# muzishen/IMAGDressing

Measured on AMD Instinct MI355X. Metric: 512x512 50-step images/sec (whole node), higher is better.
Workload: dtype bf16

## Files before the change

imagdressing_amd/_lib.py:

```python
from __future__ import annotations

import ctypes as C
import os

_HERE = os.path.dirname(os.path.abspath(__file__))
LIB_PATH = os.environ.get("IMD_LIB_PATH") or os.path.join(_HERE, "libimagdressing_hip.so")

ABI_VERSION = 9

u16p = C.POINTER(C.c_uint16)
f32p = C.POINTER(C.c_float)


class _Sized(C.Structure):

    def __init__(self, *args, **kw):
        super().__init__(*args, **kw)
        self.struct_bytes = C.sizeof(self)


class HeadsDest(C.Structure):
    _fields_ = [("ptr", C.c_void_p), ("kind", C.c_int), ("DP", C.c_int), ("L", C.c_int), ("scale", C.c_float)]


class ConvGemmParams(_Sized):
    _fields_ = [("struct_bytes", C.c_uint32), 
        ("x", C.c_void_p), ("w", C.c_void_p), ("out", C.c_void_p),
        ("M", C.c_int), ("N", C.c_int), ("K", C.c_int),
        ("Cin", C.c_int), ("taps", C.c_int), ("Hin", C.c_int), ("Win", C.c_int), ("Hout", C.c_int),
        ("Wout", C.c_int), ("stride", C.c_int), ("ups", C.c_int),
        ("x_pix_stride", C.c_int), ("out_ld", C.c_int), ("res_ld", C.c_int),
        ("bias", C.c_void_p), ("rowvec", C.c_void_p), ("rowvec_stride", C.c_int),
        ("res", C.c_void_p), ("out_scale", C.c_float), ("act", C.c_int), ("out_f32", C.c_int),
        ("mode", C.c_int), ("hC", C.c_int), ("hH", C.c_int), ("hD", C.c_int),
        ("hd", HeadsDest * 3), ("dtype", C.c_int), ("split_k", C.c_int), ("splitk_ws", C.c_void_p),
        ("x_bytes", C.c_uint32), ("w_bytes", C.c_uint32), ("flags", C.c_int),
        ("gn_a", C.c_void_p), ("gn_b", C.c_void_p), ("gn_silu", C.c_int), ("pad_br_only", C.c_int),
        ("splitk_counters", C.c_void_p),
        ("gn_stats_out", C.c_void_p), ("gn_stats_groups", C.c_int),
        ("gn_in_partial", C.c_void_p), ("gn_in_gamma", C.c_void_p), ("gn_in_beta", C.c_void_p),
        ("gn_in_nparts", C.c_int), ("gn_in_groups", C.c_int), ("gn_in_silu", C.c_int), ("gn_in_eps", C.c_float),
        ("gn_out_gamma", C.c_void_p), ("gn_out_beta", C.c_void_p), ("gn_out_eps", C.c_float), ("gn_out_silu", C.c_int), ("gn_out_groups", C.c_int), ("res_rows", C.c_int),
    ]


class FfParams(_Sized):
    _fields_ = [("struct_bytes", C.c_uint32), ("x", C.c_void_p), ("w1", C.c_void_p), ("b1", C.c_void_p), ("w2", C.c_void_p), ("b2", C.c_void_p), ("out", C.c_void_p),
                ("M", C.c_int), ("C", C.c_int), ("inner", C.c_int), ("x_ld", C.c_int), ("out_ld", C.c_int), ("ln", C.c_int),
                ("ln_eps", C.c_float), ("dtype", C.c_int)]


class XattnParams(_Sized):
    _fields_ = [("struct_bytes", C.c_uint32), ("x", C.c_void_p), ("w", C.c_void_p), ("bq", C.c_void_p), ("bo", C.c_void_p), ("kv", C.c_void_p),
                ("out", C.c_void_p), ("M", C.c_int), ("C", C.c_int), ("heads", C.c_int), ("L", C.c_int), ("rows_per_image", C.c_int),
                ("kv_bdiv", C.c_int), ("text_rows", C.c_int), ("x_ld", C.c_int), ("out_ld", C.c_int), ("q_scale", C.c_float),
                ("ln_eps", C.c_float), ("dtype", C.c_int)]


class AttnParams(_Sized):
    _fields_ = [("struct_bytes", C.c_uint32), 
        ("q", C.c_void_p), ("k1", C.c_void_p), ("v1t", C.c_void_p), ("k2", C.c_void_p), ("v2t", C.c_void_p),
        ("scale2", C.c_void_p), ("out", C.c_void_p),
        ("B", C.c_int), ("H", C.c_int), ("N", C.c_int), ("D", C.c_int),
        ("L1", C.c_int), ("L1P", C.c_int), ("kv1_bdiv", C.c_int),
        ("L2", C.c_int), ("L2P", C.c_int), ("kv2_bdiv", C.c_int),
        ("out_ld", C.c_int), ("dtype", C.c_int), ("flags", C.c_int), ("causal", C.c_int), ("k_pad_one", C.c_int),
        ("proj_w", C.c_void_p), ("proj_b", C.c_void_p), ("proj_res", C.c_void_p), ("proj_out", C.c_void_p),
        ("proj_res_ld", C.c_int), ("proj_out_ld", C.c_int), ("proj_counters", C.c_void_p),
        ("out_dup", C.c_void_p), ("phase2_out", C.c_void_p), ("phase2_rows", C.c_int),
    ]


class GroupNormParams(_Sized):
    _fields_ = [("struct_bytes", C.c_uint32), 
        ("x", C.c_void_p), ("y", C.c_void_p), ("gamma", C.c_void_p), ("beta", C.c_void_p), ("partial", C.c_void_p),
        ("B", C.c_int), ("HW", C.c_int), ("C", C.c_int), ("G", C.c_int), ("x_ld", C.c_int), ("y_ld", C.c_int),
        ("eps", C.c_float), ("silu", C.c_int), ("dtype", C.c_int), ("nparts", C.c_int),
    ]


class LayerNormParams(_Sized):
    _fields_ = [("struct_bytes", C.c_uint32), 
        ("x", C.c_void_p), ("y", C.c_void_p), ("gamma", C.c_void_p), ("beta", C.c_void_p),
        ("rows", C.c_int), ("C", C.c_int), ("x_ld", C.c_int), ("y_ld", C.c_int), ("eps", C.c_float), ("dtype", C.c_int),
    ]


class DdimParams(_Sized):
    _fields_ = [("struct_bytes", C.c_uint32), 
        ("z", C.c_void_p), ("eps", C.c_void_p), ("x_next", C.c_void_p),
        ("B", C.c_int), ("HW", C.c_int),
        ("guidance", C.c_float), ("sqrt_a_t", C.c_float), ("sqrt_1m_a_t", C.c_float),
        ("sqrt_a_prev", C.c_float), ("sqrt_1m_a_prev", C.c_float),
        ("mask", C.c_void_p), ("z_img", C.c_void_p), ("noise", C.c_void_p),
        ("sqrt_a_next", C.c_float), ("sqrt_1m_a_next", C.c_float), ("dtype", C.c_int),
        ("coefs", C.c_void_p), ("var_noise", C.c_void_p), ("sigma", C.c_float),
    ]


class SamplerParams(_Sized):
    _fields_ = [("struct_bytes", C.c_uint32),
        ("z", C.c_void_p), ("eps", C.c_void_p), ("x_next", C.c_void_p), ("hist", C.c_void_p),
        ("B", C.c_int), ("HW", C.c_int), ("K", C.c_int), ("dtype", C.c_int),
        ("guidance", C.c_float), ("guidance_rows", C.c_void_p),
        ("m_x", C.c_float), ("m_e", C.c_float), ("z_x", C.c_float), ("z_m", C.c_float),
        ("z_h", C.c_float * 4),
        ("z_n", C.c_float), ("b_img", C.c_float), ("b_noise", C.c_float), ("in_scale", C.c_float),
        ("store", C.c_int),
        ("noise", C.c_void_p), ("mask", C.c_void_p), ("z_img", C.c_void_p), ("blend_noise", C.c_void_p),
        ("coefs", C.c_void_p),
    ]


class ImageResampleParams(_Sized):
    _fields_ = [("struct_bytes", C.c_uint32),
        ("src", C.c_void_p), ("src_row_stride", C.c_int64), ("src_img_stride", C.c_int64), ("out", C.c_void_p), ("tmp", C.c_void_p),
        ("B", C.c_int), ("Hin", C.c_int), ("Win", C.c_int), ("C", C.c_int), ("Hres", C.c_int), ("Wres", C.c_int),
        ("h_xmin", C.c_void_p), ("h_count", C.c_void_p), ("h_k", C.c_void_p), ("h_kmax", C.c_int), ("h_taps", C.c_int),
        ("v_xmin", C.c_void_p), ("v_count", C.c_void_p), ("v_k", C.c_void_p), ("v_kmax", C.c_int), ("v_taps", C.c_int),
        ("v_tile_rows", C.c_int), ("top", C.c_int), ("left", C.c_int), ("crop_h", C.c_int), ("crop_w", C.c_int),
        ("kind", C.c_int), ("dtype", C.c_int), ("binarize", C.c_int), ("flags", C.c_int),
        ("a", C.c_float * 3), ("b", C.c_float * 3),
    ]


class ImagePackParams(_Sized):
    _fields_ = [("struct_bytes", C.c_uint32), ("src", C.c_void_p), ("out", C.c_void_p),
                ("B", C.c_int), ("H", C.c_int), ("W", C.c_int), ("ld", C.c_int), ("dtype", C.c_int)]


class ImageOverlayParams(_Sized):
    _fields_ = [("struct_bytes", C.c_uint32), ("orig", C.c_void_p), ("mask", C.c_void_p), ("gen", C.c_void_p), ("out", C.c_void_p),
                ("B", C.c_int), ("Bo", C.c_int), ("H0", C.c_int), ("W0", C.c_int),
                ("x1", C.c_int), ("y1", C.c_int), ("cw", C.c_int), ("ch", C.c_int)]


class ImageInpaintConditionParams(_Sized):
    _fields_ = [("struct_bytes", C.c_uint32), ("image", C.c_void_p), ("mask", C.c_void_p), ("out", C.c_void_p),
                ("B", C.c_int), ("H", C.c_int), ("W", C.c_int), ("dtype", C.c_int)]


SYMBOLS = {
    "imd_abi_version": (C.c_int, []),
    "imd_last_error": (C.c_char_p, []),
    "imd_device_check": (C.c_int, [C.c_int]),
    "imd_conv_gemm": (C.c_int, [C.POINTER(ConvGemmParams), C.c_int, C.c_void_p]),
    "imd_conv_gemm_auto_cfg": (C.c_int, [C.c_int, C.c_int]),
    "imd_conv_gemm_auto_split": (C.c_int, [C.c_int, C.c_int, C.c_int, C.c_int]),
    "imd_attention": (C.c_int, [C.POINTER(AttnParams), C.c_void_p]),
    "imd_attention_dup_supported": (C.c_int, [C.c_int, C.c_int, C.c_int]),
    "imd_attention_phase_split_supported": (C.c_int, [C.c_int]),
    "imd_attention_fp8": (C.c_int, [C.POINTER(AttnParams), C.c_int, C.c_int, C.c_int, C.c_void_p]),
    "imd_attn_quantize_fp8": (C.c_int, [C.c_void_p, C.c_void_p, C.c_int, C.c_long, C.c_int, C.c_int, C.c_float, C.c_int, C.c_void_p]),
    "imd_set_tuning": (C.c_int, [C.c_int, C.c_int]),
    "imd_get_tuning": (C.c_int, [C.c_int]),
    "imd_attn_padded_dims": (C.c_int, [C.c_int, C.POINTER(C.c_int), C.POINTER(C.c_int)]),
    "imd_groupnorm": (C.c_int, [C.POINTER(GroupNormParams), C.c_void_p]),
    "imd_groupnorm_coeffs": (C.c_int, [C.POINTER(GroupNormParams), C.c_void_p, C.c_void_p, C.c_void_p]),
    "imd_conv_patch_supported": (C.c_int, [C.POINTER(ConvGemmParams)]),
    "imd_conv_patch2_supported": (C.c_int, [C.POINTER(ConvGemmParams)]),
    "imd_conv_patch3_supported": (C.c_int, [C.POINTER(ConvGemmParams)]),
    "imd_conv_patch4_supported": (C.c_int, [C.POINTER(ConvGemmParams)]),
    "imd_conv_img_supported": (C.c_int, [C.POINTER(ConvGemmParams)]),
    "imd_conv_patch_stats_parts": (C.c_int, [C.POINTER(ConvGemmParams)]),
    "imd_conv_gemm_stats_parts": (C.c_int, [C.POINTER(ConvGemmParams), C.c_int]),
    "imd_conv_gemm_gn_out_supported": (C.c_int, [C.POINTER(ConvGemmParams)]),
    "imd_row_linear_gn_in_supported": (C.c_int, [C.POINTER(ConvGemmParams), C.c_int]),
    "imd_gemm_dma_supported": (C.c_int, [C.POINTER(ConvGemmParams)]),
    "imd_row_linear": (C.c_int, [C.POINTER(ConvGemmParams), C.c_int, C.c_float, C.c_void_p]),
    "imd_row_linear_supported": (C.c_int, [C.POINTER(ConvGemmParams)]),
    "imd_ff_geglu": (C.c_int, [C.POINTER(FfParams), C.c_void_p]),
    "imd_text_xattn320": (C.c_int, [C.POINTER(XattnParams), C.c_void_p]),
    "imd_text_xattn320_supported": (C.c_int, [C.POINTER(XattnParams)]),
    "imd_conv_ups_phase": (C.c_int, [C.POINTER(ConvGemmParams), C.c_void_p]),
    "imd_conv_ups_phase_supported": (C.c_int, [C.POINTER(ConvGemmParams)]),
    "imd_groupnorm_workspace_floats": (C.c_int, [C.c_int, C.c_int, C.c_int, C.c_int]),
    "imd_layernorm": (C.c_int, [C.POINTER(LayerNormParams), C.c_void_p]),
    "imd_softmax_rows": (C.c_int, [C.c_void_p, C.c_int, C.c_void_p, C.c_int, C.c_int, C.c_int, C.c_int, C.c_void_p]),
    "imd_ddim_cfg_step": (C.c_int, [C.POINTER(DdimParams), C.c_void_p]),
    "imd_ddim_cfg_step_rows": (C.c_int, [C.POINTER(DdimParams), C.c_void_p, C.c_void_p]),
    "imd_sampler_step": (C.c_int, [C.POINTER(SamplerParams), C.c_void_p]),
    "imd_sampler_step_rows": (C.c_int, [C.POINTER(SamplerParams), C.c_void_p, C.c_void_p]),
    "imd_image_resample": (C.c_int, [C.POINTER(ImageResampleParams), C.c_void_p]),
    "imd_image_resample_form": (C.c_int, [C.POINTER(ImageResampleParams)]),
    "imd_image_pack_u8": (C.c_int, [C.POINTER(ImagePackParams), C.c_void_p]),
    "imd_image_overlay": (C.c_int, [C.POINTER(ImageOverlayParams), C.c_void_p]),
    "imd_image_inpaint_condition": (C.c_int, [C.POINTER(ImageInpaintConditionParams), C.c_void_p]),
    "imd_timestep_embedding": (C.c_int, [C.c_void_p, C.c_void_p, C.c_int, C.c_int, C.c_void_p]),
    "imd_add": (C.c_int, [C.c_void_p, C.c_int, C.c_void_p, C.c_int, C.c_void_p, C.c_int, C.c_long, C.c_int, C.c_float, C.c_int, C.c_void_p]),
    "imd_embed_tokens": (C.c_int, [C.c_void_p, C.c_int, C.c_void_p, C.c_int, C.c_void_p, C.c_void_p, C.c_long, C.c_int, C.c_int, C.c_void_p]),
    "imd_vit_assemble": (C.c_int, [C.c_void_p, C.c_void_p, C.c_void_p, C.c_void_p, C.c_int, C.c_int, C.c_int, C.c_int, C.c_void_p]),
    "imd_lincomb": (C.c_int, [C.POINTER(C.c_void_p), C.POINTER(C.c_float), C.c_int, C.c_void_p, C.c_long, C.c_void_p]),
    "imd_copy2d": (C.c_int, [C.c_void_p, C.c_int, C.c_void_p, C.c_int, C.c_long, C.c_int, C.c_void_p]),
    "imd_concat2": (C.c_int, [C.c_void_p, C.c_int, C.c_void_p, C.c_int, C.c_void_p, C.c_void_p, C.c_long, C.c_long, C.c_int, C.c_void_p]),
    "imd_concat2_gn_stats": (C.c_int, [C.c_void_p, C.c_int, C.c_void_p, C.c_int, C.c_void_p, C.c_void_p, C.c_int, C.c_int, C.c_int, C.c_int,
                                       C.c_void_p, C.c_int, C.c_void_p]),
    "imd_groupnorm_parts": (C.c_int, [C.c_int, C.c_int, C.c_int]),
    "imd_f32_to_16": (C.c_int, [C.c_void_p, C.c_void_p, C.c_long, C.c_int, C.c_void_p]),
}

_lib = None


class ImdError(RuntimeError):
    pass


def load():
    global _lib
    if _lib is None:
        if not os.path.isfile(LIB_PATH):
            raise ImdError(
                f"{LIB_PATH} not found: build it with `python -c 'import __graft_entry__ as g; g.build()'` "
                "(or imagdressing_amd/csrc/build.sh).  imagdressing_amd has no CPU / torch fallback.")
        lib = C.CDLL(LIB_PATH)
        for name, (res, args) in SYMBOLS.items():
            fn = getattr(lib, name)
            fn.restype, fn.argtypes = res, args
        if lib.imd_abi_version() != ABI_VERSION:
            raise ImdError(f"ABI version mismatch: library reports {lib.imd_abi_version()}, binding expects {ABI_VERSION}")
        _lib = lib
    return _lib


def check(rc: int):
    if rc != 0:
        raise ImdError(load().imd_last_error().decode("utf-8", "replace"))
```

imagdressing_amd/adapter/attention_processor.py:

```python
from __future__ import annotations

import math
from typing import Dict, Optional, Tuple

import torch
import torch.nn as nn

from .. import ops

bf16 = torch.bfloat16
LOG2E = math.log2(math.e)


class LoRALinearLayer(nn.Module):

    def __init__(self, in_features, out_features, rank=4, network_alpha=None):
        super().__init__()
        self.down = nn.Linear(in_features, rank, bias=False)
        self.up = nn.Linear(rank, out_features, bias=False)
        self.network_alpha = network_alpha
        self.rank = rank
        nn.init.normal_(self.down.weight, std=1 / rank)
        nn.init.zeros_(self.up.weight)

    def delta(self) -> torch.Tensor:
        d = self.up.weight.float() @ self.down.weight.float()
        if self.network_alpha is not None:
            d = d * (self.network_alpha / self.rank)
        return d


def _version_key(*tensors) -> Tuple:
    return tuple((t.data_ptr(), t._version, t.device, t.dtype) for t in tensors)


class _TensorCache:

    def __init__(self, capacity: int = 4):
        self._entries = []
        self._cap = capacity

    def get(self, srcs, extra=()):
        key = (_version_key(*srcs), extra)
        for i, (s, k, v) in enumerate(self._entries):
            if k == key and len(s) == len(srcs) and all(a is b for a, b in zip(s, srcs)):
                if i != len(self._entries) - 1:
                    self._entries.append(self._entries.pop(i))
                return v
        return None

    def put(self, srcs, value, extra=()):
        self._entries.append((tuple(srcs), (_version_key(*srcs), extra), value))
        if len(self._entries) > self._cap:
            self._entries.pop(0)
        return value


_W_PARTS = {"qkv": ("to_q", "to_k", "to_v"), "kv": ("to_k", "to_v"), "q": ("to_q",), "o": ("to_out",), "bo": ("to_out",)}
_16BIT = (torch.bfloat16, torch.float16)


def _compute_dtype(attn, hidden_states: torch.Tensor, attention_mask=None):
    if attention_mask is not None:
        raise NotImplementedError("attention_mask is always None on the IMAGDressing path (SURVEY appendix 3); masks are not implemented")
    if getattr(attn, "spatial_norm", None) is not None or getattr(attn, "group_norm", None) is not None \
            or getattr(attn, "norm_cross", None):
        raise NotImplementedError("attn.spatial_norm / group_norm / norm_cross are None for every SD1.5 attention layer; "
                                  "modules that set them are not supported by the fused processors")
    wd = attn.to_q.weight.dtype
    if wd in _16BIT:
        return wd
    return hidden_states.dtype if hidden_states.dtype in _16BIT else torch.float16


def _layer_weights(attn, which: str, dtype, device) -> torch.Tensor:
    mods = [attn.to_out[0] if n == "to_out" else getattr(attn, n) for n in _W_PARTS[which]]
    srcs = [m.bias if which == "bo" else m.weight for m in mods]
    if srcs[0] is None:
        return None
    want = torch.float32 if which == "bo" else dtype
    if len(srcs) == 1 and srcs[0].dtype == want and srcs[0].device == device and srcs[0].is_contiguous():
        return srcs[0].detach()
    cache = attn.__dict__.setdefault("_imd_wcache", {})
    key = (_version_key(*srcs), want, str(device))
    ent = cache.get(which)
    if ent is None or ent[0] != key or not all(a is b for a, b in zip(ent[1], srcs)):
        t = torch.cat([t.detach().to(device=device, dtype=want) for t in srcs], 0).contiguous()
        ent = cache[which] = (key, tuple(srcs), t)
    return ent[2]


def _ln_folded_q(attn, gamma: torch.Tensor, beta: torch.Tensor, dtype, device, which: str = "q"):
    mods = [getattr(attn, n) for n in _W_PARTS[which]]
    srcs = tuple(m.weight for m in mods) + (gamma, beta)
    cache = attn.__dict__.setdefault("_imd_wcache", {})
    key = (_version_key(*srcs), dtype, str(device))
    ent = cache.get(which + "_ln")
    if ent is None or ent[0] != key or not all(a is b for a, b in zip(ent[1], srcs)):
        w = torch.cat([m.weight.detach().to(device=device, dtype=dtype) for m in mods], 0)
        ent = cache[which + "_ln"] = (key, srcs, ops.fold_layernorm_affine(w, None, gamma.to(device), beta.to(device)))
    return ent[2]


def _qkv_ln_ok(x: torch.Tensor) -> bool:
    return x.shape[-1] == 320 and x.shape[1] % 128 == 0 and ops.FUSED_LN


FUSED_LN_CHANNELS = (320, 640, 1280)


def _as_tokens(hidden_states: torch.Tensor, dtype):
    shape4 = None
    if hidden_states.dim() == 4:
        b, c, h, w = hidden_states.shape
        shape4 = (b, c, h, w)
        hidden_states = hidden_states.view(b, c, h * w).transpose(1, 2)
    if not hidden_states.is_cuda:
        from .._lib import ImdError
        raise ImdError("imagdressing_amd processors run on MI355X only: hidden_states is on " + str(hidden_states.device))
    return hidden_states.to(dtype).contiguous(), shape4


def _restore(out, shape4, like):
    if shape4 is not None:
        b, c, h, w = shape4
        out = out.transpose(-1, -2).reshape(b, c, h, w)
    return out


def _project_kv(tokens: torch.Tensor, wkv: torch.Tensor, heads: int):
    Bk, Lk, Kd = tokens.shape
    Cc = wkv.shape[0] // 2
    D = Cc // heads
    dpk, dpv = ops.attn_padded_dims(D)
    LP = ops.pad64(Lk)
    k = ops.k_buffer((Bk, heads, Lk, dpk), D, wkv.dtype, tokens.device)
    vt = torch.zeros(Bk, heads, dpv, LP, dtype=wkv.dtype, device=tokens.device)
    ops.conv_gemm(tokens.view(Bk * Lk, Kd), wkv, M=Bk * Lk, N=2 * Cc, Cin=Kd, Hin=Lk, Win=1, Hout=Lk, Wout=1,
                  heads=dict(C=Cc, H=heads, D=D, dests=[(k, 0, dpk, Lk, 1.0), (vt, 1, dpv, LP, 1.0)]))
    return k, vt, Lk, LP


_FP8_KV: Dict[int, tuple] = {}
ops._clear_hooks.append(_FP8_KV.clear)


def _fp8_kv(kv, cache: bool):
    k, vt = kv[0], kv[1]
    e = ops.FP8_EXPS
    if cache:
        hit = _FP8_KV.get(id(k))
        if hit is not None and hit[0] is k and hit[1] == (e["q"], e["k"], e["v"]):
            return hit[2], hit[3]
    k8 = ops.quantize_fp8_rows(k, e["k"], pad_val=float(2 ** (e["q"] + e["k"])))
    v8 = ops.quantize_fp8_vt(vt, e["v"])
    if cache:
        if len(_FP8_KV) > 64:
            _FP8_KV.clear()
        _FP8_KV[id(k)] = (k, (e["q"], e["k"], e["v"]), k8, v8)
    return k8, v8


def _fused_attention(x: torch.Tensor, heads: int, *, wq_or_qkv: torch.Tensor, self_attn: bool,
                     kv1=None, kv1_bdiv: int = 1, kv2=None, kv2_bdiv: int = 1, scale2: Optional[torch.Tensor] = None,
                     wo: torch.Tensor, bo: Optional[torch.Tensor], residual: Optional[torch.Tensor],
                     q_ln: Optional[tuple] = None, pair_half: bool = False, phase2_rows: int = 0) -> torch.Tensor:
    B, N, Cc = x.shape
    D = Cc // heads
    dpk, dpv = ops.attn_padded_dims(D)
    dev, dt = x.device, x.dtype
    qscale = D ** -0.5 * LOG2E
    if (ops.FUSED_XATTN and not self_attn and q_ln is not None and kv1 is not None and kv2 is None and not pair_half
            and ops.text_xattn_supported(Cc, heads, N, kv1[2]) and not ops.ATTN_FP8 and not ops.FUSED_OUT_PROJ
            and residual is not None and residual.data_ptr() == x.data_ptr() and residual.shape == x.shape
            and residual.dtype == dt and residual.is_contiguous()):
        return ops.text_xattn(x, ops.pack_text_xattn(q_ln[0], q_ln[1], wo, bo), ops.pack_text_kv(kv1[0], kv1[1], kv1[2]),
                              Lk=kv1[2], kv_bdiv=kv1_bdiv, ln_eps=q_ln[2], q_scale=qscale)
    q = ops.workspace("attn_q", (B, heads, N, dpk), dt, dev)
    x2 = x.view(B * N, Cc)
    if self_attn:
        LP = ops.pad64(N)
        k = ops.k_buffer((B, heads, N, dpk), D, dt, dev, tag="attn_k")
        vt = ops.workspace("attn_vt", (B, heads, dpv, LP), dt, dev)
        dests = dict(C=Cc, H=heads, D=D, dests=[(q, 0, dpk, N, qscale), (k, 0, dpk, N, 1.0), (vt, 1, dpv, LP, 1.0)])
        if q_ln is not None:
            ops.conv_gemm(x2, q_ln[0], M=B * N, N=3 * Cc, Cin=Cc, Hin=N, Win=1, Hout=N, Wout=1, bias=q_ln[1], ln_eps=q_ln[2], heads=dests)
        else:
            ops.conv_gemm(x2, wq_or_qkv, M=B * N, N=3 * Cc, Cin=Cc, Hin=N, Win=1, Hout=N, Wout=1, heads=dests)
        kv1, kv1_bdiv = (k, vt, N, LP), 1
    elif q_ln is not None:
        ops.conv_gemm(x2, q_ln[0], M=B * N, N=Cc, Cin=Cc, Hin=N, Win=1, Hout=N, Wout=1, bias=q_ln[1], ln_eps=q_ln[2],
                      heads=dict(C=Cc, H=heads, D=D, dests=[(q, 0, dpk, N, qscale)]))
    else:
        ops.conv_gemm(x2, wq_or_qkv, M=B * N, N=Cc, Cin=Cc, Hin=N, Win=1, Hout=N, Wout=1,
                      heads=dict(C=Cc, H=heads, D=D, dests=[(q, 0, dpk, N, qscale)]))
    o = torch.empty(B, N, Cc, dtype=dt, device=dev)
    if ops.ATTN_FP8 and D == 40:
        e = ops.FP8_EXPS
        q8 = ops.quantize_fp8_rows(q, e["q"])
        k18, v18 = _fp8_kv(kv1, cache=not self_attn)
        kw = {}
        if kv2 is not None and scale2 is not None:
            k28, v28 = _fp8_kv(kv2, cache=True)
            kw = dict(k2=k28, v2t=v28, L2=kv2[2], L2P=kv2[3], kv2_bdiv=kv2_bdiv, scale2=scale2)
        ops.attention_fp8(q8, k18, v18, o, B=B, H=heads, N=N, L1=kv1[2], L1P=kv1[3], kv1_bdiv=kv1_bdiv, **kw)
        res2 = None if residual is None else residual.view(B * N, Cc)
        return ops.linear(o.view(B * N, Cc), wo, bo, res=res2).view(B, N, Cc)
    kw = {}
    if kv2 is not None and scale2 is not None:
        kw = dict(k2=kv2[0], v2t=kv2[1], L2=kv2[2], L2P=kv2[3], kv2_bdiv=kv2_bdiv, scale2=scale2)
    if ops.FUSED_OUT_PROJ and ops.attention_proj_supported(heads, N, D):
        out = torch.empty(B, N, Cc, dtype=dt, device=dev)
        return ops.attention(q, kv1[0], kv1[1], o, B=B, H=heads, N=N, D=D, L1=kv1[2], L1P=kv1[3], kv1_bdiv=kv1_bdiv, k_pad_one=True,
                             proj=(wo, bo, residual, out), **kw)
    if pair_half:
        o = torch.empty(2 * B, N, Cc, dtype=dt, device=dev)
        ops.attention(q, kv1[0], kv1[1], o[:B], B=B, H=heads, N=N, D=D, L1=kv1[2], L1P=kv1[3], kv1_bdiv=kv1_bdiv, k_pad_one=True,
                      out_dup=o[B:], **kw)
        res2 = None if residual is None else residual.reshape(-1, Cc)
        return ops.linear(o.view(2 * B * N, Cc), wo, bo, res=res2).view(2 * B, N, Cc)
    ops.attention(q, kv1[0], kv1[1], o, B=B, H=heads, N=N, D=D, L1=kv1[2], L1P=kv1[3], kv1_bdiv=kv1_bdiv, k_pad_one=True, phase2_rows=phase2_rows if kw else 0, **kw)
    res2 = None if residual is None else residual.view(B * N, Cc)
    return ops.linear(o.view(B * N, Cc), wo, bo, res=res2).view(B, N, Cc)


class _FusedBase:
    fused_residual = True

    @staticmethod
    def _ehs_bdiv(B: int, ehs: torch.Tensor) -> int:
        Be = ehs.shape[0]
        if B % Be:
            raise ValueError(f"encoder_hidden_states batch {Be} does not divide hidden_states batch {B}")
        return B // Be

    @staticmethod
    def _finish(attn, out, residual_given, like, shape4, ln_fused=False):
        if getattr(attn, "residual_connection", False) and not residual_given:
            if ln_fused:
                raise NotImplementedError("attn.residual_connection together with the engine's fused LayerNorm (imd_layernorm)")
            out = ops.add(out, _as_tokens(like, out.dtype)[0])
        if getattr(attn, "rescale_output_factor", 1.0) != 1.0:
            raise NotImplementedError("rescale_output_factor != 1 is not used by SD1.5")
        out = _restore(out, shape4, like)
        return out if out.dtype == like.dtype else out.to(like.dtype)


class AttnProcessor2_0(_FusedBase):

    fused_layernorm = True

    def __init__(self, cache_entries: int = 256):
        self._text = _TensorCache(capacity=cache_entries)

    def __call__(self, attn, hidden_states, encoder_hidden_states=None, attention_mask=None, temb=None, scale=1.0,
                 imd_residual=None, imd_layernorm=None, **kwargs):
        dt = _compute_dtype(attn, hidden_states, attention_mask)
        x, shape4 = _as_tokens(hidden_states, dt)
        dev = x.device
        wo, bo = _layer_weights(attn, "o", dt, dev), _layer_weights(attn, "bo", dt, dev)
        q_ln = None
        if imd_layernorm is not None:
            g, be, eps = imd_layernorm
            if encoder_hidden_states is not None and x.shape[-1] in FUSED_LN_CHANNELS:
                q_ln = _ln_folded_q(attn, g, be, dt, dev) + (eps,)
            elif encoder_hidden_states is None and _qkv_ln_ok(x):
                q_ln = _ln_folded_q(attn, g, be, dt, dev, "qkv") + (eps,)
            else:
                x = ops.layer_norm(x, g, be, eps)
        if encoder_hidden_states is None:
            out = _fused_attention(x, attn.heads, wq_or_qkv=_layer_weights(attn, "qkv", dt, dev), self_attn=True, wo=wo, bo=bo,
                                   residual=imd_residual, q_ln=q_ln)
        else:
            srcs = (encoder_hidden_states, attn.to_k.weight, attn.to_v.weight)
            kv = self._text.get(srcs, extra=(dt,))
            if kv is None:
                e = encoder_hidden_states.to(device=dev, dtype=dt).contiguous()
                kv = self._text.put(srcs, _project_kv(e, _layer_weights(attn, "kv", dt, dev), attn.heads), extra=(dt,))
            out = _fused_attention(x, attn.heads, wq_or_qkv=_layer_weights(attn, "q", dt, dev), self_attn=False, kv1=kv,
                                   kv1_bdiv=self._ehs_bdiv(x.shape[0], encoder_hidden_states), wo=wo, bo=bo,
                                   residual=imd_residual, q_ln=q_ln)
        return self._finish(attn, out, imd_residual is not None, hidden_states, shape4, ln_fused=imd_layernorm is not None)


class CacheAttnProcessor2_0(AttnProcessor2_0):
    fused_layernorm = False

    def __init__(self):
        super().__init__()
        self.cache = {}

    def __call__(self, attn, hidden_states, encoder_hidden_states=None, attention_mask=None, temb=None, scale=1.0,
                 **kwargs):
        self.cache["hidden_states"] = hidden_states
        return super().__call__(attn, hidden_states, encoder_hidden_states=encoder_hidden_states, **kwargs)


class _RefMixin:

    def _init_ref(self, name, hidden_size, cross_attention_dim, scale):
        self.name = name
        self.hidden_size = hidden_size
        self.cross_attention_dim = cross_attention_dim
        self.to_k_ref = nn.Linear(cross_attention_dim or hidden_size, hidden_size, bias=False)
        self.to_v_ref = nn.Linear(cross_attention_dim or hidden_size, hidden_size, bias=False)
        self.scale = scale
        self._wref = _TensorCache()
        self._garment = _TensorCache()
        self._scale2 = _TensorCache()
        self._scale2_plain: Dict = {}

    def _garment_kv(self, ref: torch.Tensor, heads: int, device, dtype):
        wsrc = (self.to_k_ref.weight, self.to_v_ref.weight)
        kv = self._garment.get((ref,) + wsrc, extra=(dtype,))
        if kv is None:
            w = self._wref.get(wsrc, extra=(dtype,))
            if w is None:
                w = self._wref.put(wsrc, torch.cat([t.detach().to(device=device, dtype=dtype) for t in wsrc], 0).contiguous(),
                                   extra=(dtype,))
            r = ref.detach().to(device=device, dtype=dtype).contiguous()
            if r.dim() != 3:
                raise ValueError(f"sa_hidden_states[{self.name!r}] must be [Bg, M, C], got {tuple(ref.shape)}")
            kv = self._garment.put((ref,) + wsrc, _project_kv(r, w, heads), extra=(dtype,))
        return kv

    def _garment_bdiv(self, B: int, ref: torch.Tensor) -> int:
        Bg = ref.shape[0]
        if Bg < 1 or B % Bg:
            raise ValueError(f"sa_hidden_states[{self.name!r}] has batch {Bg}, which does not divide hidden_states batch {B}")
        return B // Bg

    def _branch_weights(self, B: int, mask: Optional[torch.Tensor], device) -> torch.Tensor:
        s = float(self.scale)
        if mask is None:
            t = self._scale2_plain.get((B, s, str(device)))
            if t is None:
                t = torch.full((B,), s, dtype=torch.float32, device=device)
                self._scale2_plain = {(B, s, str(device)): t}
            return t
        t = self._scale2.get((mask,), extra=(s,))
        if t is None:
            t = self._scale2.put((mask,), (mask.to(device=device, dtype=torch.float32) * s).contiguous(), extra=(s,))
        return t


class RefSAttnProcessor2_0(nn.Module, _FusedBase, _RefMixin):
    fused_layernorm = True
    fused_pair_half = True

    def __init__(self, name, hidden_size, cross_attention_dim=None, scale=1.0):
        super().__init__()
        self._init_ref(name, hidden_size, cross_attention_dim, scale)

    def _weights(self, attn, dt, dev):
        return _layer_weights(attn, "qkv", dt, dev), _layer_weights(attn, "o", dt, dev), _layer_weights(attn, "bo", dt, dev)

    def __call__(self, attn, hidden_states, encoder_hidden_states=None, attention_mask=None, temb=None, scale=1.0,
                 num_images_per_prompt=1, cond_hidden_states=None, sa_hidden_states=None, sa_batch_mask=None,
                 imd_residual=None, imd_layernorm=None, imd_pair_half=False, **kwargs):
        if encoder_hidden_states is not None:
            raise NotImplementedError(f"{type(self).__name__} is a self-attention (attn1) processor")
        dt = _compute_dtype(attn, hidden_states, attention_mask)
        x, shape4 = _as_tokens(hidden_states, dt)
        wqkv, wo, bo = self._weights(attn, dt, x.device)
        q_ln = None
        if imd_layernorm is not None:
            g, be, eps = imd_layernorm
            if _qkv_ln_ok(x):
                q_ln = _ln_folded_q(attn, g, be, dt, x.device, "qkv") + (eps,)
            else:
                x = ops.layer_norm(x, g, be, eps)
        kv2 = s2 = None
        bdiv2 = 1
        if sa_hidden_states is not None:
            ref = sa_hidden_states[self.name]
            kv2 = self._garment_kv(ref, attn.heads, x.device, x.dtype)
            cond_rows = x.shape[0] // 2 if (kwargs.get("sa_pair_layout") and not imd_pair_half and x.shape[0] % 2 == 0) else x.shape[0]
            bdiv2 = self._garment_bdiv(cond_rows, ref)
            s2 = self._branch_weights(x.shape[0] * (2 if imd_pair_half else 1), sa_batch_mask, x.device)
        if imd_pair_half and (kv2 is None or imd_residual is None or shape4 is not None):
            raise ValueError("imd_pair_half needs sa_hidden_states, the block residual and token-major hidden states (engine-internal)")
        pr = x.shape[0] // 2 if (kwargs.get("sa_pair_layout") and sa_batch_mask is not None and kv2 is not None and not imd_pair_half and x.shape[0] % 2 == 0) else 0
        out = _fused_attention(x, attn.heads, wq_or_qkv=wqkv, self_attn=True, kv2=kv2, kv2_bdiv=bdiv2,
                               scale2=s2, wo=wo, bo=bo, residual=imd_residual, q_ln=q_ln, pair_half=bool(imd_pair_half), phase2_rows=pr)
        return self._finish(attn, out, imd_residual is not None, hidden_states, shape4, ln_fused=imd_layernorm is not None)


class _LoraFold:

    def _init_lora(self, hidden_size, kdim, rank, network_alpha, lora_scale):
        self.rank = rank
        self.lora_scale = lora_scale
        self.to_q_lora = LoRALinearLayer(hidden_size, hidden_size, rank, network_alpha)
        self.to_k_lora = LoRALinearLayer(kdim, hidden_size, rank, network_alpha)
        self.to_v_lora = LoRALinearLayer(kdim, hidden_size, rank, network_alpha)
        self.to_out_lora = LoRALinearLayer(hidden_size, hidden_size, rank, network_alpha)
        self._folded = _TensorCache()

    def _fold(self, attn, device, dtype):
        ls = float(self.lora_scale)
        srcs = tuple(l.weight for lo in (self.to_q_lora, self.to_k_lora, self.to_v_lora, self.to_out_lora)
                     for l in (lo.down, lo.up)) + (attn.to_q.weight, attn.to_k.weight, attn.to_v.weight, attn.to_out[0].weight)
        w = self._folded.get(srcs, extra=(ls, dtype, str(device)))
        if w is None:
            def eff(base, lora):
                base = base.detach().to(device)
                if ls == 0.0:
                    return base.to(dtype).contiguous()
                return (base.float() + ls * lora.delta().to(device)).to(dtype).contiguous()
            wq, wk, wv = eff(attn.to_q.weight, self.to_q_lora), eff(attn.to_k.weight, self.to_k_lora), eff(attn.to_v.weight, self.to_v_lora)
            wo = eff(attn.to_out[0].weight, self.to_out_lora)
            w = self._folded.put(srcs, dict(q=wq, kv=torch.cat([wk, wv], 0).contiguous(),
                                            qkv=(torch.cat([wq, wk, wv], 0).contiguous() if wk.shape[1] == wq.shape[1] else None),
                                            o=wo), extra=(ls, dtype, str(device)))
        return w


class _LoraRefSBase(nn.Module, _FusedBase, _RefMixin, _LoraFold):

    def __init__(self, name, hidden_size, cross_attention_dim=None, scale=1.0, rank=128, network_alpha=None, lora_scale=1.0):
        super().__init__()
        self._init_ref(name, hidden_size, cross_attention_dim, scale)
        self._init_lora(hidden_size, cross_attention_dim or hidden_size, rank, network_alpha, lora_scale)

    def _weights(self, attn, dt, dev):
        w = self._fold(attn, dev, dt)
        return w["qkv"], w["o"], _layer_weights(attn, "bo", dt, dev)

    __call__ = RefSAttnProcessor2_0.__call__
    fused_pair_half = True


class LoraRefSAttnProcessor2_0(_LoraRefSBase):
    """attention_processor.py:391-511 (used by inference_IMAGdressing_ipa_controlnetpose.py:88-94)."""


class RefLoraSAttnProcessor2_0(_LoraRefSBase):
    """Same arithmetic under the name ``app.py:90`` uses (attention_processor.py:1006-1128).  As in the
    reference, ``pipe.set_scale`` does not match this class (it checks LoraRefSAttnProcessor2_0)."""


class CAttnProcessor2_0(nn.Module, _FusedBase):

    def __init__(self, name, hidden_size, cross_attention_dim=None):
        super().__init__()
        self.name = name
        self.hidden_size = hidden_size
        self.cross_attention_dim = cross_attention_dim
        self._plain = AttnProcessor2_0(cache_entries=4)

    fused_layernorm = True

    def __call__(self, attn, hidden_states, encoder_hidden_states=None, attention_mask=None, temb=None, scale=1.0,
                 cond_hidden_states=None, sa_hidden_states=None, imd_residual=None, imd_layernorm=None, **kwargs):
        return self._plain(attn, hidden_states, encoder_hidden_states=encoder_hidden_states, imd_residual=imd_residual,
                           imd_layernorm=imd_layernorm)


class _IPBase(nn.Module, _FusedBase, _LoraFold):

    def __init__(self, hidden_size, cross_attention_dim=None, rank=4, network_alpha=None, lora_scale=1.0, scale=1.0,
                 num_tokens=4):
        super().__init__()
        self.num_tokens = num_tokens
        self.hidden_size = hidden_size
        self.cross_attention_dim = cross_attention_dim
        self.scale = scale
        self._init_lora(hidden_size, cross_attention_dim or hidden_size, rank, network_alpha, lora_scale)
        self.to_k_ip = nn.Linear(cross_attention_dim or hidden_size, hidden_size, bias=False)
        self.to_v_ip = nn.Linear(cross_attention_dim or hidden_size, hidden_size, bias=False)
        self._kv = _TensorCache()
        self._wip = _TensorCache()
        self._s2: Dict = {}

    def _weights(self, attn, dt, dev):
        w = self._fold(attn, dev, dt)
        return w["q"], w["kv"], w["o"]

    def __call__(self, attn, hidden_states, encoder_hidden_states=None, attention_mask=None, scale=1.0, temb=None,
                 *args, imd_residual=None, **kwargs):
        if encoder_hidden_states is None:
            raise NotImplementedError(f"{type(self).__name__} is a cross-attention (attn2) processor")
        dt = _compute_dtype(attn, hidden_states, attention_mask)
        x, shape4 = _as_tokens(hidden_states, dt)
        wq, wkv, wo = self._weights(attn, dt, x.device)
        wsrc = (self.to_k_ip.weight, self.to_v_ip.weight)
        ls = float(getattr(self, "lora_scale", 0.0))
        ksrc = (encoder_hidden_states, attn.to_k.weight, attn.to_v.weight) + wsrc
        kvs = self._kv.get(ksrc, extra=(ls, x.dtype))
        if kvs is None:
            wip = self._wip.get(wsrc, extra=(x.dtype,))
            if wip is None:
                wip = self._wip.put(wsrc, torch.cat([t.detach().to(device=x.device, dtype=x.dtype) for t in wsrc], 0).contiguous(),
                                    extra=(x.dtype,))
            e = encoder_hidden_states.to(device=x.device, dtype=x.dtype)
            end = e.shape[1] - self.num_tokens
            kvs = self._kv.put(ksrc,
                               (_project_kv(e[:, :end].contiguous(), wkv, attn.heads),
                                _project_kv(e[:, end:].contiguous(), wip, attn.heads)), extra=(ls, x.dtype))
        B = x.shape[0]
        key = (B, float(self.scale), str(x.device))
        s2 = self._s2.get(key)
        if s2 is None:
            s2 = torch.full((B,), float(self.scale), dtype=torch.float32, device=x.device)
            self._s2 = {key: s2}
        bdiv = self._ehs_bdiv(B, encoder_hidden_states)
        out = _fused_attention(x, attn.heads, wq_or_qkv=wq, self_attn=False, kv1=kvs[0], kv1_bdiv=bdiv, kv2=kvs[1],
                               kv2_bdiv=bdiv, scale2=s2, wo=wo, bo=_layer_weights(attn, "bo", dt, x.device), residual=imd_residual)
        return self._finish(attn, out, imd_residual is not None, hidden_states, shape4)


class LoRAIPAttnProcessor2_0(_IPBase):
    """attention_processor.py:746-871."""


class IPAttnProcessor2_0(_IPBase):

    def __init__(self, hidden_size, cross_attention_dim=None, scale=1.0, num_tokens=4):
        nn.Module.__init__(self)
        self.num_tokens = num_tokens
        self.hidden_size = hidden_size
        self.cross_attention_dim = cross_attention_dim
        self.scale = scale
        self.to_k_ip = nn.Linear(cross_attention_dim or hidden_size, hidden_size, bias=False)
        self.to_v_ip = nn.Linear(cross_attention_dim or hidden_size, hidden_size, bias=False)
        self._kv = _TensorCache()
        self._wip = _TensorCache()
        self._s2 = {}

    def _weights(self, attn, dt, dev):
        return _layer_weights(attn, "q", dt, dev), _layer_weights(attn, "kv", dt, dev), _layer_weights(attn, "o", dt, dev)


class BaseSAttnProcessor2_0(nn.Module, _FusedBase):

    def __init__(self, name, cross_attention_dim=None):
        super().__init__()
        self.name, self.cross_attention_dim = name, cross_attention_dim
        self._plain = AttnProcessor2_0(cache_entries=4)

    def __call__(self, attn, hidden_states, encoder_hidden_states=None, attention_mask=None, temb=None, scale=1.0,
                 imd_residual=None, **kwargs):
        return self._plain(attn, hidden_states, encoder_hidden_states=encoder_hidden_states, imd_residual=imd_residual)


class SAttnProcessor2_0(nn.Module, _FusedBase):

    def __init__(self, name, hidden_size, cross_attention_dim=None):
        super().__init__()
        self.name, self.hidden_size, self.cross_attention_dim = name, hidden_size, cross_attention_dim
        self._plain = AttnProcessor2_0(cache_entries=4)
        self._garment = _TensorCache()

    def __call__(self, attn, hidden_states, encoder_hidden_states=None, attention_mask=None, temb=None, scale=1.0,
                 cond_hidden_states=None, sa_hidden_states=None, imd_residual=None, **kwargs):
        if sa_hidden_states is None or encoder_hidden_states is not None:
            return self._plain(attn, hidden_states, encoder_hidden_states=encoder_hidden_states, imd_residual=imd_residual)
        dt = _compute_dtype(attn, hidden_states, attention_mask)
        x, shape4 = _as_tokens(hidden_states, dt)
        dev, heads = x.device, attn.heads
        B, N, Cc = x.shape
        D = Cc // heads
        ref = sa_hidden_states[self.name]
        if ref.dim() != 3 or B % ref.shape[0]:
            raise ValueError(f"sa_hidden_states[{self.name!r}] must be [Bg, M, C] with Bg dividing the batch {B}, got {tuple(ref.shape)}")
        wkv = _layer_weights(attn, "kv", dt, dev)
        srcs = (ref, attn.to_k.weight, attn.to_v.weight)
        kvr = self._garment.get(srcs, extra=(dt,))
        if kvr is None:
            kvr = self._garment.put(srcs, _project_kv(ref.detach().to(device=dev, dtype=dt).contiguous(), wkv, heads), extra=(dt,))
        kx, vtx, _, _ = _project_kv(x, wkv, heads)
        M = kvr[2]
        L, LP = N + M, ops.pad64(N + M)
        dpk, dpv = ops.attn_padded_dims(D)
        k = ops.k_buffer((B, heads, L, dpk), D, dt, dev)
        vt = torch.zeros(B, heads, dpv, LP, dtype=dt, device=dev)
        rep = B // ref.shape[0]
        k[:, :, :N] = kx
        k[:, :, N:] = kvr[0].repeat_interleave(rep, 0) if rep > 1 else kvr[0]
        vt[..., :N] = vtx[..., :N]
        vt[..., N:L] = (kvr[1].repeat_interleave(rep, 0) if rep > 1 else kvr[1])[..., :M]
        out = _fused_attention(x, heads, wq_or_qkv=_layer_weights(attn, "q", dt, dev), self_attn=False, kv1=(k, vt, L, LP), kv1_bdiv=1,
                               wo=_layer_weights(attn, "o", dt, dev), bo=_layer_weights(attn, "bo", dt, dev), residual=imd_residual)
        return self._finish(attn, out, imd_residual is not None, hidden_states, shape4)


class RefCAttnProcessor2_0(nn.Module, _FusedBase, _RefMixin):

    def __init__(self, name, hidden_size, cross_attention_dim=None, scale=1.0):
        super().__init__()
        self._init_ref(name, hidden_size, None, scale)
        self.cross_attention_dim = cross_attention_dim
        self._plain = AttnProcessor2_0(cache_entries=4)
        self._text = _TensorCache()

    def __call__(self, attn, hidden_states, encoder_hidden_states=None, attention_mask=None, temb=None, scale=1.0,
                 cond_hidden_states=None, sa_hidden_states=None, sa_batch_mask=None, imd_residual=None, **kwargs):
        if sa_hidden_states is None:
            return self._plain(attn, hidden_states, encoder_hidden_states=encoder_hidden_states, imd_residual=imd_residual)
        dt = _compute_dtype(attn, hidden_states, attention_mask)
        x, shape4 = _as_tokens(hidden_states, dt)
        dev, heads = x.device, attn.heads
        ref = sa_hidden_states[self.name]
        kv2 = self._garment_kv(ref, heads, dev, dt)
        bdiv2 = self._garment_bdiv(x.shape[0], ref)
        s2 = self._branch_weights(x.shape[0], sa_batch_mask, dev)
        wo, bo = _layer_weights(attn, "o", dt, dev), _layer_weights(attn, "bo", dt, dev)
        if encoder_hidden_states is None:
            out = _fused_attention(x, heads, wq_or_qkv=_layer_weights(attn, "qkv", dt, dev), self_attn=True, kv2=kv2, kv2_bdiv=bdiv2,
                                   scale2=s2, wo=wo, bo=bo, residual=imd_residual)
        else:
            srcs = (encoder_hidden_states, attn.to_k.weight, attn.to_v.weight)
            kv = self._text.get(srcs, extra=(dt,))
            if kv is None:
                e = encoder_hidden_states.to(device=dev, dtype=dt).contiguous()
                kv = self._text.put(srcs, _project_kv(e, _layer_weights(attn, "kv", dt, dev), heads), extra=(dt,))
            out = _fused_attention(x, heads, wq_or_qkv=_layer_weights(attn, "q", dt, dev), self_attn=False, kv1=kv,
                                   kv1_bdiv=self._ehs_bdiv(x.shape[0], encoder_hidden_states), kv2=kv2, kv2_bdiv=bdiv2, scale2=s2,
                                   wo=wo, bo=bo, residual=imd_residual)
        return self._finish(attn, out, imd_residual is not None, hidden_states, shape4)
```

imagdressing_amd/csrc/capi.cpp:

```cpp
#include <atomic>
#include <mutex>
#include <stdarg.h>
#include <stdio.h>
#include <string.h>

#include "imd_kernels.h"

namespace {
thread_local char g_err[512] = "";
}

int imd_set_error(const char* fmt, ...) {
    va_list ap;
    va_start(ap, fmt);
    vsnprintf(g_err, sizeof(g_err), fmt, ap);
    va_end(ap);
    return 1;
}

int imd_check_launch(const char* what) {
    hipError_t e = hipGetLastError();
    if (e != hipSuccess) return imd_set_error("%s: launch failed: %s", what, hipGetErrorString(e));
    return 0;
}

#define IMD_REQUIRE(cond, ...) do { if (!(cond)) return imd_set_error(__VA_ARGS__); } while (0)
#define IMD_REQUIRE_SIZE(p, what) IMD_REQUIRE((p)->struct_bytes == sizeof(*(p)), \
    "%s: parameter block is %u bytes in the caller's view, this library (ABI v%d) expects %zu: the binding mirrors another version of include/imagdressing_hip.h (set struct_bytes = sizeof(struct) after zero-initialising it)", \
    what, (unsigned)(p)->struct_bytes, IMD_ABI_VERSION, sizeof(*(p)))

namespace {
struct LdsAttrEnt { const void* kern; int dev; };
constexpr int kMaxLdsAttr = 512;
LdsAttrEnt g_lds_attr[kMaxLdsAttr];
std::atomic<int> g_lds_attr_n{0};
std::mutex g_lds_attr_mu;
int g_cu8[64] = {};
}

int imd_lds_attr(const void* kern, int bytes, const char* what) {
    int dev = 0;
    if (hipGetDevice(&dev) != hipSuccess) return imd_set_error("%s: cannot identify the current device", what);
    const int n = g_lds_attr_n.load(std::memory_order_acquire);
    for (int i = 0; i < n; ++i)
        if (g_lds_attr[i].kern == kern && g_lds_attr[i].dev == dev) return 0;
    std::lock_guard<std::mutex> lock(g_lds_attr_mu);
    hipError_t e = hipFuncSetAttribute(kern, hipFuncAttributeMaxDynamicSharedMemorySize, bytes);
    if (e != hipSuccess) return imd_set_error("%s: hipFuncSetAttribute failed: %s", what, hipGetErrorString(e));
    const int m = g_lds_attr_n.load(std::memory_order_relaxed);
    if (m < kMaxLdsAttr) {
        g_lds_attr[m] = LdsAttrEnt{kern, dev};
        g_lds_attr_n.store(m + 1, std::memory_order_release);
    }
    return 0;
}

int imd_cu_count8() {
    int dev = 0;
    if (hipGetDevice(&dev) != hipSuccess || dev < 0 || dev >= 64) return -1;
    if (g_cu8[dev] == 0) {
        int cus = 0;
        if (hipDeviceGetAttribute(&cus, hipDeviceAttributeMultiprocessorCount, dev) != hipSuccess) return -1;
        g_cu8[dev] = cus / 8 * 8 < 8 ? 8 : cus / 8 * 8;
    }
    return g_cu8[dev];
}

extern "C" {

int imd_abi_version(void) { return IMD_ABI_VERSION; }
const char* imd_last_error(void) { return g_err; }

int imd_device_check(int device) {
    hipDeviceProp_t prop;
    hipError_t e = hipGetDeviceProperties(&prop, device);
    if (e != hipSuccess) return imd_set_error("device_check: hipGetDeviceProperties(%d) failed: %s", device, hipGetErrorString(e));
    if (strncmp(prop.gcnArchName, "gfx950", 6) != 0)
        return imd_set_error("device_check: device %d is %s; this library is built for gfx950 (MI355X) only", device, prop.gcnArchName);
    return 0;
}

int imd_conv_gemm(const imd_conv_gemm_params* p, int cfg, void* stream) {
    IMD_REQUIRE(p != nullptr, "conv_gemm: null params");
    IMD_REQUIRE_SIZE(p, "conv_gemm");
    IMD_REQUIRE(p->x && p->w, "conv_gemm: null input/weight pointer");
    IMD_REQUIRE(p->mode == IMD_OUT_HEADS || p->out != nullptr, "conv_gemm: null output pointer");
    IMD_REQUIRE(p->Hout > 0 && p->Wout > 0 && p->Hin > 0 && p->Win > 0, "conv_gemm: bad geometry");
    IMD_REQUIRE(p->stride == 1 || p->stride == 2, "conv_gemm: stride must be 1 or 2");
    IMD_REQUIRE(p->M % (p->Hout * p->Wout) == 0, "conv_gemm: M (%d) is not a multiple of Hout*Wout (%d)", p->M, p->Hout * p->Wout);
    if (p->mode == IMD_OUT_HEADS) {
        IMD_REQUIRE(p->hC > 0 && p->hH > 0 && p->hD > 0 && p->hC == p->hH * p->hD, "conv_gemm: bad head split C=%d H=%d D=%d", p->hC, p->hH, p->hD);
        IMD_REQUIRE(p->N % p->hC == 0 && p->N / p->hC <= 3, "conv_gemm: N (%d) must be 1..3 splits of %d channels", p->N, p->hC);
        IMD_REQUIRE(p->hD % 8 == 0, "conv_gemm: head dim must be a multiple of 8");
        IMD_REQUIRE(p->act != IMD_ACT_GEGLU && !p->out_f32, "conv_gemm: head-split output excludes GEGLU / fp32 output");
    }
    if (p->act == IMD_ACT_GEGLU) IMD_REQUIRE(!p->out_f32 && !p->res, "conv_gemm: GEGLU excludes fp32 output and residual");
    return imd_launch_conv_gemm(*p, cfg, (hipStream_t)stream);
}

int imd_conv_gemm_auto_cfg(int M, int N) { return imd_conv_gemm_choose_cfg(M, N); }
int imd_conv_gemm_auto_split(int M, int N, int K, int cfg) { return imd_conv_gemm_choose_split(M, N, K, cfg < 0 ? imd_conv_gemm_choose_cfg(M, N) : cfg); }

int imd_attention(const imd_attn_params* p, void* stream) {
    IMD_REQUIRE(p != nullptr, "attention: null params");
    IMD_REQUIRE_SIZE(p, "attention");
    IMD_REQUIRE(p->q && p->k1 && p->v1t && p->out, "attention: null q/k/v/out pointer");
    IMD_REQUIRE((p->k2 == nullptr) == (p->v2t == nullptr), "attention: k2 and v2t must be given together");
    IMD_REQUIRE(p->out_ld >= p->H * p->D && p->out_ld % 4 == 0, "attention: bad out_ld %d", p->out_ld);
    return imd_launch_attention(*p, (hipStream_t)stream);
}

int imd_attention_fp8(const imd_attn_params* p, int eq, int ek, int ev, void* stream) {
    IMD_REQUIRE(p != nullptr, "attention_fp8: null params");
    IMD_REQUIRE_SIZE(p, "attention_fp8");
    IMD_REQUIRE(p->q && p->k1 && p->v1t && p->out, "attention_fp8: null q/k/v/out pointer");
    IMD_REQUIRE((p->k2 == nullptr) == (p->v2t == nullptr), "attention_fp8: k2 and v2t must be given together");
    IMD_REQUIRE(p->out_ld >= p->H * p->D && p->out_ld % 4 == 0, "attention_fp8: bad out_ld %d", p->out_ld);
    IMD_REQUIRE(p->dtype == IMD_DTYPE_BF16 || p->dtype == IMD_DTYPE_F16, "attention_fp8: unknown output dtype %d", p->dtype);
    return imd_launch_attention_fp8(*p, eq, ek, ev, (hipStream_t)stream);
}

int imd_attn_quantize_fp8(const uint16_t* src, uint8_t* dst, int kind, long count, int LP, int exp2_scale, float pad_val, int dtype,
                          void* stream) {
    IMD_REQUIRE(src && dst && count > 0, "attn_quantize_fp8: null pointer / empty");
    IMD_REQUIRE(kind == 0 || kind == 1, "attn_quantize_fp8: kind must be 0 (Q / K rows) or 1 (V^T)");
    IMD_REQUIRE(exp2_scale >= -16 && exp2_scale <= 16, "attn_quantize_fp8: exponent out of range");
    return imd_launch_attn_quantize_fp8(src, dst, kind, count, LP, exp2_scale, pad_val, dtype, (hipStream_t)stream);
}

int imd_set_tuning(int knob, int value) {
    switch (knob) {
        case 0:
#ifdef IMD_ABLATIONS
            IMD_REQUIRE(value >= 1 && value <= 54, "set_tuning: attention variant for head dim 40 must be 1..54 (20..49: timing ablations, WRONG results; 50..54: correct but no faster)");
#else
            IMD_REQUIRE(value >= 1 && value <= 13, "set_tuning: attention variant for head dim 40 must be 1..13 (the timing ablations 20..49 and the measured no-gain variants 50..54 exist only in -DIMD_ABLATIONS builds)");
#endif
            g_attn_qw40 = value; return 0;
        case 1: g_attn_xcd = value ? 1 : 0; return 0;
        case 2:
#ifndef IMD_ABLATIONS
            IMD_REQUIRE((value & 224) == 0, "set_tuning: bits 5..7 of knob 2 are the timing ablations of gemm_dma256.hip (WRONG results); they exist only in -DIMD_ABLATIONS builds");
#endif
            IMD_REQUIRE((value & ~2047) == 0, "set_tuning: knob 2 has bits 0..10 only (got %d)", value);
            g_gemm_flags = value; return 0;
#ifdef IMD_ATTN_SWEEP
        case 3: g_attn_v80 = value; return 0;
        case 4: g_attn_v160 = value; return 0;
#endif
        default: return imd_set_error("set_tuning: unknown knob %d", knob);
    }
}

int imd_get_tuning(int knob) { return knob == 0 ? g_attn_qw40 : knob == 1 ? g_attn_xcd : knob == 2 ? g_gemm_flags : -1; }

int imd_attn_padded_dims(int D, int* dpk, int* dpv) {
    IMD_REQUIRE(D == 40 || D == 64 || D == 80 || D == 160, "attn_padded_dims: unsupported head dim %d", D);
    if (dpk) *dpk = imd_attn_dpk(D);
    if (dpv) *dpv = imd_attn_dpv(D);
    return 0;
}

int imd_groupnorm(const imd_groupnorm_params* p, void* stream) {
    IMD_REQUIRE(p != nullptr, "groupnorm: null params");
    IMD_REQUIRE_SIZE(p, "groupnorm");
    IMD_REQUIRE(p->x && p->y && p->gamma && p->beta && p->partial, "groupnorm: null pointer");
    return imd_launch_groupnorm(*p, (hipStream_t)stream);
}

int imd_groupnorm_coeffs(const imd_groupnorm_params* p, float* coef_a, float* coef_b, void* stream) {
    IMD_REQUIRE(p != nullptr, "groupnorm_coeffs: null params");
    IMD_REQUIRE_SIZE(p, "groupnorm_coeffs");
    IMD_REQUIRE(p->x && p->gamma && p->beta && p->partial && coef_a && coef_b, "groupnorm_coeffs: null pointer");
    return imd_launch_groupnorm_coeffs(*p, coef_a, coef_b, (hipStream_t)stream);
}

static bool sized(const imd_conv_gemm_params* p) { return p && p->struct_bytes == sizeof(*p); }
static int query(const imd_conv_gemm_params* p, bool (*pred)(const imd_conv_gemm_params&)) {
    if (!sized(p)) return 0;
    imd_conv_gemm_params q = *p;
    if (!imd_conv_gemm_fill_extents(q)) return 0;
    return pred(q) ? 1 : 0;
}
int imd_conv_patch_supported(const imd_conv_gemm_params* p) { return query(p, static_cast<bool (*)(const imd_conv_gemm_params&)>(imd_conv_patch_supported)); }
int imd_conv_patch2_supported(const imd_conv_gemm_params* p) { return query(p, static_cast<bool (*)(const imd_conv_gemm_params&)>(imd_conv_patch2_supported)); }
int imd_conv_patch3_supported(const imd_conv_gemm_params* p) { return query(p, static_cast<bool (*)(const imd_conv_gemm_params&)>(imd_conv_patch3_supported)); }
int imd_conv_patch4_supported(const imd_conv_gemm_params* p) { return query(p, static_cast<bool (*)(const imd_conv_gemm_params&)>(imd_conv_patch4_supported)); }
int imd_conv_img_supported(const imd_conv_gemm_params* p) { return query(p, static_cast<bool (*)(const imd_conv_gemm_params&)>(imd_conv_img_supported)); }
int imd_conv_patch_stats_parts(const imd_conv_gemm_params* p) { return sized(p) ? imd_conv_patch_stats_parts_of(*p) : 0; }
int imd_conv_gemm_stats_parts(const imd_conv_gemm_params* p, int cfg) { return sized(p) ? imd_conv_gemm_stats_parts_of(*p, cfg) : 0; }
int imd_row_linear_gn_in_supported(const imd_conv_gemm_params* p, int cfg) { return (sized(p) && p->gn_in_partial != nullptr && imd_row_linear_gn_in_supported_of(*p, cfg)) ? 1 : 0; }
int imd_conv_gemm_gn_out_supported(const imd_conv_gemm_params* p) { return (sized(p) && imd_conv_gemm_gn_out_supported_of(*p, -1)) ? 1 : 0; }
int imd_gemm_dma_supported(const imd_conv_gemm_params* p) { return query(p, static_cast<bool (*)(const imd_conv_gemm_params&)>(imd_gemm_dma_supported)); }

int imd_row_linear_supported(const imd_conv_gemm_params* p) { return (sized(p) && (imd_row_linear_supported(*p) || imd_row_linear_k640_supported(*p) || imd_row_linear_k1280_supported(*p) || imd_row_qkv_supported(*p))) ? 1 : 0; }

int imd_row_linear(const imd_conv_gemm_params* p, int ln, float ln_eps, void* stream) {
    IMD_REQUIRE(p != nullptr, "row_linear: null params");
    IMD_REQUIRE_SIZE(p, "row_linear");
    IMD_REQUIRE(p->x && p->w, "row_linear: null input/weight pointer");
    IMD_REQUIRE(p->mode == IMD_OUT_HEADS || p->out != nullptr, "row_linear: null output pointer");
    IMD_REQUIRE(p->Hout > 0 && p->Wout > 0 && p->M > 0 && p->M % (p->Hout * p->Wout) == 0, "row_linear: bad geometry");
    if (p->mode == IMD_OUT_HEADS) {
        IMD_REQUIRE(p->hC > 0 && p->hH > 0 && p->hD > 0 && p->hC == p->hH * p->hD && p->N % p->hC == 0 && p->N / p->hC <= 3 && p->hD % 8 == 0,
                    "row_linear: bad head split C=%d H=%d D=%d", p->hC, p->hH, p->hD);
        IMD_REQUIRE(!p->out_f32, "row_linear: head-split output excludes fp32 output");
    }
    IMD_REQUIRE(!ln || ln_eps > 0.f, "row_linear: LayerNorm needs eps > 0");
    if (p->K == 320 && p->N == 960 && p->mode == IMD_OUT_HEADS) {
        IMD_REQUIRE(p->gn_in_partial == nullptr, "row_linear: the fused q / k / v projection has no GroupNorm prologue (gn_in_*)");
        return imd_launch_row_qkv(*p, ln, ln_eps, (hipStream_t)stream);
    }
    if (p->K == 640) return imd_launch_row_linear_k640(*p, ln, ln_eps, (hipStream_t)stream);
    if (p->K == 1280) return imd_launch_row_linear_k1280(*p, ln, ln_eps, (hipStream_t)stream);
    return imd_launch_row_linear(*p, ln, ln_eps, (hipStream_t)stream);
}

int imd_ff_geglu(const imd_ff_params* p, void* stream) {
    IMD_REQUIRE(p != nullptr, "ff_geglu: null params");
    IMD_REQUIRE_SIZE(p, "ff_geglu");
    IMD_REQUIRE(p->x && p->w1 && p->b1 && p->w2 && p->b2 && p->out, "ff_geglu: null pointer");
    IMD_REQUIRE(!p->ln || p->ln_eps > 0.f, "ff_geglu: LayerNorm needs eps > 0");
    return imd_launch_ff_geglu(*p, (hipStream_t)stream);
}

int imd_text_xattn320_supported(const imd_xattn_params* p) {
    return (p && p->struct_bytes == sizeof(*p) && imd_text_xattn320_supported_of(*p)) ? 1 : 0;
}

int imd_text_xattn320(const imd_xattn_params* p, void* stream) {
    IMD_REQUIRE(p != nullptr, "text_xattn320: null params");
    IMD_REQUIRE_SIZE(p, "text_xattn320");
    IMD_REQUIRE(p->x && p->w && p->bq && p->bo && p->kv && p->out, "text_xattn320: null pointer");
    return imd_launch_text_xattn320(*p, (hipStream_t)stream);
}

int imd_conv_ups_phase_supported(const imd_conv_gemm_params* p) { return (sized(p) && imd_conv_ups_phase_supported_of(*p)) ? 1 : 0; }

int imd_conv_ups_phase(const imd_conv_gemm_params* p, void* stream) {
    IMD_REQUIRE(p != nullptr, "conv_ups_phase: null params");
    IMD_REQUIRE_SIZE(p, "conv_ups_phase");
    IMD_REQUIRE(p->x && p->w && p->out, "conv_ups_phase: null input / weight / output pointer");
    return imd_launch_conv_ups_phase(*p, (hipStream_t)stream);
}

int imd_layernorm(const imd_layernorm_params* p, void* stream) {
    IMD_REQUIRE(p != nullptr, "layernorm: null params");
    IMD_REQUIRE_SIZE(p, "layernorm");
    IMD_REQUIRE(p->x && p->y && p->gamma && p->beta, "layernorm: null pointer");
    return imd_launch_layernorm(*p, (hipStream_t)stream);
}

int imd_embed_tokens(const uint16_t* table, int vocab, const uint16_t* pos, int T, const int64_t* ids, uint16_t* out, long rows, int C,
                     int dtype, void* stream) {
    IMD_REQUIRE(table && pos && ids && out, "embed_tokens: null pointer");
    return imd_launch_embed_tokens(table, vocab, pos, T, ids, out, rows, C, dtype, (hipStream_t)stream);
}

int imd_vit_assemble(const uint16_t* patches, const uint16_t* cls, const uint16_t* pos, uint16_t* out, int B, int P, int C, int dtype,
                     void* stream) {
    IMD_REQUIRE(patches && cls && pos && out, "vit_assemble: null pointer");
    return imd_launch_vit_assemble(patches, cls, pos, out, B, P, C, dtype, (hipStream_t)stream);
}

int imd_lincomb(const float* const* xs, const float* coefs, int n, float* out, long numel, void* stream) {
    IMD_REQUIRE(xs && coefs && out, "lincomb: null pointer");
    return imd_launch_lincomb(xs, coefs, n, out, numel, (hipStream_t)stream);
}

int imd_softmax_rows(const float* s, int s_ld, uint16_t* p, int p_ld, int rows, int cols, int dtype, void* stream) {
    IMD_REQUIRE(s && p, "softmax_rows: null pointer");
    return imd_launch_softmax_rows(s, s_ld, p, p_ld, rows, cols, dtype, (hipStream_t)stream);
}

int imd_ddim_cfg_step(const imd_ddim_params* p, void* stream) {
    IMD_REQUIRE(p != nullptr, "ddim_cfg_step: null params");
    IMD_REQUIRE_SIZE(p, "ddim_cfg_step");
    IMD_REQUIRE(p->z && p->eps, "ddim_cfg_step: null pointer");
    IMD_REQUIRE(p->coefs != nullptr || p->sqrt_a_t > 0.f, "ddim_cfg_step: sqrt(alpha_t) must be positive");
    return imd_launch_ddim_cfg_step(*p, (hipStream_t)stream);
}

int imd_sampler_step(const imd_sampler_params* p, void* stream) {
    IMD_REQUIRE(p != nullptr, "sampler_step: null params");
    IMD_REQUIRE_SIZE(p, "sampler_step");
    IMD_REQUIRE(p->z && p->eps, "sampler_step: null pointer");
    return imd_launch_sampler_step(*p, (hipStream_t)stream);
}

int imd_sampler_step_rows(const imd_sampler_params* p, const float* coef_rows, void* stream) {
    IMD_REQUIRE(p != nullptr, "sampler_step_rows: null params");
    IMD_REQUIRE_SIZE(p, "sampler_step_rows");
    IMD_REQUIRE(p->z && p->eps, "sampler_step_rows: null pointer");
    return imd_launch_sampler_step_rows(*p, coef_rows, (hipStream_t)stream);
}

int imd_image_resample(const imd_image_resample_params* p, void* stream) {
    IMD_REQUIRE(p != nullptr, "image_resample: null params");
    IMD_REQUIRE_SIZE(p, "image_resample");
    return imd_launch_image_resample(*p, (hipStream_t)stream);
}

int imd_image_resample_form(const imd_image_resample_params* p) {
    if (!p || p->struct_bytes != sizeof(*p)) return 0;
    return imd_image_resample_form_of(*p);
}

int imd_image_pack_u8(const imd_image_pack_params* p, void* stream) {
    IMD_REQUIRE(p != nullptr, "image_pack_u8: null params");
    IMD_REQUIRE_SIZE(p, "image_pack_u8");
    return imd_launch_image_pack_u8(*p, (hipStream_t)stream);
}

int imd_image_overlay(const imd_image_overlay_params* p, void* stream) {
    IMD_REQUIRE(p != nullptr, "image_overlay: null params");
    IMD_REQUIRE_SIZE(p, "image_overlay");
    return imd_launch_image_overlay(*p, (hipStream_t)stream);
}

int imd_image_inpaint_condition(const imd_image_inpaint_condition_params* p, void* stream) {
    IMD_REQUIRE(p != nullptr, "image_inpaint_condition: null params");
    IMD_REQUIRE_SIZE(p, "image_inpaint_condition");
    return imd_launch_image_inpaint_condition(*p, (hipStream_t)stream);
}

int imd_ddim_cfg_step_rows(const imd_ddim_params* p, const float* guidance, void* stream) {
    IMD_REQUIRE(p != nullptr, "ddim_cfg_step_rows: null params");
    IMD_REQUIRE_SIZE(p, "ddim_cfg_step_rows");
    IMD_REQUIRE(p->z && p->eps && guidance, "ddim_cfg_step_rows: null pointer");
    IMD_REQUIRE(p->coefs != nullptr || p->sqrt_a_t > 0.f, "ddim_cfg_step_rows: sqrt(alpha_t) must be positive");
    return imd_launch_ddim_cfg_step_rows(*p, guidance, (hipStream_t)stream);
}

int imd_timestep_embedding(const float* t, float* out, int B, int dim, void* stream) {
    IMD_REQUIRE(t && out, "timestep_embedding: null pointer");
    return imd_launch_timestep_embedding(t, out, B, dim, (hipStream_t)stream);
}

int imd_add(const uint16_t* a, int a_ld, const uint16_t* b, int b_ld, uint16_t* out, int out_ld, long rows, int C, float b_scale, int dtype, void* stream) {
    IMD_REQUIRE(a && b && out, "add: null pointer");
    return imd_launch_add(a, a_ld, b, b_ld, out, out_ld, rows, C, b_scale, dtype, (hipStream_t)stream);
}

int imd_copy2d(const uint16_t* a, int a_ld, uint16_t* out, int out_ld, long rows, int C, void* stream) {
    IMD_REQUIRE(a && out, "copy2d: null pointer");
    return imd_launch_copy2d(a, a_ld, out, out_ld, rows, C, (hipStream_t)stream);
}

int imd_concat2(const uint16_t* a, int Ca, const uint16_t* b, int Cb, const uint16_t* b_add, uint16_t* out, long rows, long b_rows, int dtype, void* stream) {
    IMD_REQUIRE(a && b && out, "concat2: null pointer");
    return imd_launch_concat2(a, Ca, b, Cb, b_add, out, rows, b_rows, dtype, (hipStream_t)stream);
}

int imd_groupnorm_parts(int B, int HW, int C) { return imd_groupnorm_parts_of(B, HW, C); }

int imd_concat2_gn_stats(const uint16_t* a, int Ca, const uint16_t* b, int Cb, const uint16_t* b_add, uint16_t* out, int B, int HW, int b_B, int G,
                         float* partial, int dtype, void* stream) {
    IMD_REQUIRE(a && b && out && partial, "concat2 + statistics: null pointer");
    return imd_launch_concat2_gn_stats(a, Ca, b, Cb, b_add, out, B, HW, b_B, G, partial, dtype, (hipStream_t)stream);
}

int imd_f32_to_16(const float* a, uint16_t* out, long n, int dtype, void* stream) {
    IMD_REQUIRE(a && out, "f32_to_16: null pointer");
    return imd_launch_f32_to_16(a, out, n, dtype, (hipStream_t)stream);
}

}
```

imagdressing_amd/csrc/imd_kernels.h:

```cpp
#pragma once
#include <hip/hip_runtime.h>
#include <stdint.h>

#include "../../include/imagdressing_hip.h"

typedef uint16_t bf16_t;
typedef imd_heads_dest HeadsDest;
typedef imd_conv_gemm_params ConvGemmParams;
typedef imd_attn_params AttnParams;
typedef imd_groupnorm_params GroupNormParams;
typedef imd_layernorm_params LayerNormParams;
typedef imd_ddim_params DdimParams;
typedef imd_sampler_params SamplerParams;
typedef imd_image_resample_params ImageResampleParams;
typedef imd_image_pack_params ImagePackParams;
typedef imd_image_overlay_params ImageOverlayParams;
typedef imd_image_inpaint_condition_params ImageInpaintConditionParams;

enum { ACT_NONE = IMD_ACT_NONE, ACT_SILU = IMD_ACT_SILU, ACT_GEGLU = IMD_ACT_GEGLU, ACT_GELU = IMD_ACT_GELU, ACT_QUICK_GELU = IMD_ACT_QUICK_GELU };
enum { OUT_ROWMAJOR = IMD_OUT_ROWMAJOR, OUT_HEADS = IMD_OUT_HEADS };

int imd_set_error(const char* fmt, ...);
int imd_check_launch(const char* what);
int imd_lds_attr(const void* kern, int bytes, const char* what);
int imd_cu_count8();

int imd_conv_gemm_choose_cfg(int M, int N);
int imd_conv_gemm_choose_split(int M, int N, int K, int cfg);
int imd_launch_conv_gemm(const ConvGemmParams& p, int cfg, hipStream_t s);
bool imd_conv_gemm_fill_extents(ConvGemmParams& p);
bool imd_conv_patch_supported(const ConvGemmParams& p);
bool imd_conv_patch2_supported(const ConvGemmParams& p);
int imd_launch_conv_patch2(const ConvGemmParams& p, hipStream_t s);
bool imd_conv_patch3_supported(const ConvGemmParams& p);
int imd_launch_conv_patch3(const ConvGemmParams& p, hipStream_t s);
bool imd_conv_patch4_supported(const ConvGemmParams& p);
int imd_launch_conv_patch4(const ConvGemmParams& p, hipStream_t s);
int imd_conv_patch3_stats_parts_of(const ConvGemmParams& p, int nw);
bool imd_conv_patch64_supported(const ConvGemmParams& p);
int imd_launch_conv_patch64(const ConvGemmParams& p, hipStream_t s);
bool imd_conv_ups_phase_supported_of(const ConvGemmParams& p);
int imd_launch_conv_ups_phase(const ConvGemmParams& p, hipStream_t s);
bool imd_conv_img_supported(const ConvGemmParams& p);
int imd_launch_conv_img(const ConvGemmParams& p, hipStream_t s);
int imd_conv_patch_stats_parts_of(const ConvGemmParams& p);
int imd_conv_gemm_stats_parts_of(const ConvGemmParams& p, int cfg);
bool imd_conv_gemm_gn_out_supported_of(const ConvGemmParams& p, int cfg);
bool imd_row_linear_gn_in_supported_of(const ConvGemmParams& p, int cfg);
int imd_launch_conv_patch(const ConvGemmParams& p, hipStream_t s);
bool imd_row_linear_supported(const ConvGemmParams& p);
int imd_launch_row_linear(const ConvGemmParams& p, int ln, float ln_eps, hipStream_t s);
bool imd_row_linear_k640_supported(const ConvGemmParams& p);
int imd_launch_row_linear_k640(const ConvGemmParams& p, int ln, float ln_eps, hipStream_t s);
bool imd_row_linear_k1280_supported(const ConvGemmParams& p);
int imd_launch_row_linear_k1280(const ConvGemmParams& p, int ln, float ln_eps, hipStream_t s);
bool imd_row_qkv_supported(const ConvGemmParams& p);
int imd_launch_row_qkv(const ConvGemmParams& p, int ln, float ln_eps, hipStream_t s);
bool imd_gemm_dma_supported(const ConvGemmParams& p);
int imd_launch_gemm_dma(const ConvGemmParams& p, hipStream_t s);
int imd_launch_gemm_dma128(const ConvGemmParams& p, int stages, int bk, hipStream_t s);
int imd_launch_gemm_dma256(const ConvGemmParams& p, int form, hipStream_t s);
bool imd_conv_dma_supported(const ConvGemmParams& p);
int imd_launch_ff_geglu(const imd_ff_params& p, hipStream_t s);
bool imd_text_xattn320_supported_of(const imd_xattn_params& p);
int imd_launch_text_xattn320(const imd_xattn_params& p, hipStream_t s);
int imd_launch_attention(const AttnParams& p, hipStream_t s);
int imd_launch_attention_d40(const AttnParams& p, int variant, hipStream_t s);
int imd_launch_attention_fp8(const AttnParams& p, int eq, int ek, int ev, hipStream_t s);
int imd_launch_attn_quantize_fp8(const bf16_t* src, unsigned char* dst, int kind, long rows_or_groups, int LP, int exp2_scale,
                                 float pad_val, int dtype, hipStream_t s);
extern int g_attn_qw40;
extern int g_attn_xcd;
#ifdef IMD_ATTN_SWEEP
extern int g_attn_v80, g_attn_v160;
#endif
extern int g_gemm_flags;
int imd_attn_dpk(int D);
int imd_attn_dpv(int D);
int imd_launch_groupnorm(const GroupNormParams& p, hipStream_t s);
int imd_launch_groupnorm_coeffs(const GroupNormParams& p, float* ca, float* cb, hipStream_t s);
int imd_groupnorm_parts_of(int B, int HW, int C);
int imd_launch_concat2_gn_stats(const bf16_t* a, int Ca, const bf16_t* b, int Cb, const bf16_t* b_add, bf16_t* out, int B, int HW, int b_B, int G,
                                float* partial, int dtype, hipStream_t s);
int imd_launch_layernorm(const LayerNormParams& p, hipStream_t s);
int imd_launch_softmax_rows(const float* s_in, int s_ld, bf16_t* p_out, int p_ld, int rows, int cols, int dtype, hipStream_t s);
int imd_launch_ddim_cfg_step(const DdimParams& p, hipStream_t s);
int imd_launch_ddim_cfg_step_rows(const DdimParams& p, const float* guidance, hipStream_t s);
int imd_launch_sampler_step(const SamplerParams& p, hipStream_t s);
int imd_launch_sampler_step_rows(const SamplerParams& p, const float* coef_rows, hipStream_t s);
int imd_launch_image_resample(const ImageResampleParams& p, hipStream_t s);
int imd_image_resample_form_of(const ImageResampleParams& p);
int imd_launch_image_pack_u8(const ImagePackParams& p, hipStream_t s);
int imd_launch_image_overlay(const ImageOverlayParams& p, hipStream_t s);
int imd_launch_image_inpaint_condition(const ImageInpaintConditionParams& p, hipStream_t s);
int imd_launch_timestep_embedding(const float* t, float* out, int B, int dim, hipStream_t s);
int imd_launch_add(const bf16_t* a, int a_ld, const bf16_t* b, int b_ld, bf16_t* out, int out_ld, long rows, int C, float b_scale, int dtype, hipStream_t s);
int imd_launch_embed_tokens(const bf16_t* table, int vocab, const bf16_t* pos, int T, const int64_t* ids, bf16_t* out, long rows, int C, int dtype, hipStream_t s);
int imd_launch_vit_assemble(const bf16_t* patches, const bf16_t* cls, const bf16_t* pos, bf16_t* out, int B, int P, int C, int dtype, hipStream_t s);
int imd_launch_lincomb(const float* const* xs, const float* coefs, int n, float* out, long numel, hipStream_t s);
int imd_launch_copy2d(const bf16_t* a, int a_ld, bf16_t* out, int out_ld, long rows, int C, hipStream_t s);
int imd_launch_concat2(const bf16_t* a, int Ca, const bf16_t* b, int Cb, const bf16_t* b_add, bf16_t* out, long rows, long b_rows, int dtype, hipStream_t s);
int imd_launch_f32_to_16(const float* a, bf16_t* out, long n, int dtype, hipStream_t s);
```

imagdressing_amd/csrc/row_xattn.hip:

```cpp
#include "row_common.h"

namespace {

constexpr int XA_C = 320;
constexpr int XA_STEPS = XA_C / 16;
constexpr int XA_ROWB = XA_C * 2;
constexpr int XA_CHUNK = 64 * XA_ROWB;
constexpr int XA_PIECES = ROW_PIECES;
constexpr int XA_RING = ROW_RING;
constexpr int XA_BM = 128;
constexpr int XA_NQ = 6, XA_NKV = 4, XA_NO = 5;
constexpr int XA_NCHUNK = XA_NQ + XA_NKV + XA_NO;
constexpr int XA_LMAX = 96;
constexpr int XA_KROW = 96;
constexpr int XA_VROW = 208;
constexpr int XA_KBYTES = XA_LMAX * XA_KROW;
constexpr int XA_HEADB = XA_KBYTES + 48 * XA_VROW;
constexpr int XA_XB = 8 * 5 * 512;
constexpr int XA_OFF_X = XA_RING * XA_CHUNK;
constexpr int XA_LDS = XA_OFF_X + 2 * XA_XB;
static_assert(XA_CHUNK == ROW_CHUNK, "the ring of the family: 40 KB chunks in five pieces per wave");
static_assert(2 * XA_HEADB <= XA_CHUNK && XA_LDS <= 160 * 1024, "LDS budget");
static_assert(64 * XA_NQ * 4 <= XA_XB && XA_C * 4 <= XA_XB, "bias tables live in the exchange area");

template <bool F16>
__global__ __launch_bounds__(512, 1) void text_xattn320_kernel(const imd_xattn_params p) {
    using E = El<F16>;
    extern __shared__ __attribute__((aligned(16))) char smem[];
    const int tid = threadIdx.x;
    const int lane = tid & 63;
    const int wave = __builtin_amdgcn_readfirstlane(tid >> 6);
    const int hi = lane >> 5, col = lane & 31;
    const int rb = wave & 3;
    const int chh = wave >> 2;
    const int m0 = blockIdx.x * XA_BM;

    const uint32_t x_bytes = (uint32_t)(((size_t)(p.M - 1) * p.x_ld + XA_C) * 2);
    const __amdgpu_buffer_rsrc_t rs_x = __builtin_amdgcn_make_buffer_rsrc(const_cast<uint16_t*>(p.x), 0, x_bytes, 0x00020000);
    const int m = m0 + rb * 32 + col;
    const uint32_t xoff = (uint32_t)m * (uint32_t)(p.x_ld * 2) + hi * 16;
    uint4 xf[XA_STEPS];
    load_rows(xf, rs_x, m < p.M, xoff, 32);
    float bq_v = 0.f, bo_v = 0.f;
    if (tid < 64 * XA_NQ) bq_v = p.bq[tid];
    if (tid < XA_C) bo_v = p.bo[tid];

    const int tb = (m0 / p.rows_per_image) / p.kv_bdiv;
    const v4i_t ds_w = raw_rsrc(p.w, (uint32_t)((XA_NQ + XA_NO) * XA_CHUNK));
    const v4i_t ds_kv = raw_rsrc(reinterpret_cast<const char*>(p.kv) + (size_t)tb * XA_NKV * XA_CHUNK, (uint32_t)(XA_NKV * XA_CHUNK));
    const uint32_t loff = (uint32_t)wave * 1024u + (uint32_t)lane * 16u;
    const uint32_t lds0 = (uint32_t)(uintptr_t)smem;
    auto stage = [&](int c) {
        const uint32_t base = lds0 + (uint32_t)((c % XA_RING) * XA_CHUNK) + (uint32_t)wave * 1024u;
        const bool kvc = c >= XA_NQ && c < XA_NQ + XA_NKV;
        const uint32_t src = loff + (uint32_t)((kvc ? c - XA_NQ : c < XA_NQ ? c : c - XA_NKV) * XA_CHUNK);
#pragma unroll
        for (int j = 0; j < XA_PIECES; ++j) dma16(kvc ? ds_kv : ds_w, base + j * 8192u, src + j * 8192u);
    };
    stage(0);
    stage(1);
    pin_rows(xf);
    float* bias_s = reinterpret_cast<float*>(smem + XA_OFF_X);
    if (tid < 64 * XA_NQ) bias_s[tid] = bq_v;

    ln_rows_inplace<F16, XA_C>(xf, p.ln_eps);

    const f32x16 zero16 = {0.f, 0.f, 0.f, 0.f, 0.f, 0.f, 0.f, 0.f, 0.f, 0.f, 0.f, 0.f, 0.f, 0.f, 0.f, 0.f};
    const int wrow = chh * 32 + col;
    const uint32_t a16 = (uint32_t)((hi ^ ((wrow >> 1) & 7)) << 4);
    const char* wlane = smem + wrow * XA_ROWB;

    uint4 qf[2 * XA_NQ];
#pragma unroll
    for (int c = 0; c < XA_NQ; ++c) {
        dma_wait_keep_n<XA_PIECES>();
        __syncthreads();
        stage(c + 2);
        const char* Ws = wlane + (c % XA_RING) * XA_CHUNK;
        f32x16 acc = zero16;
#pragma unroll
        for (int s = 0; s < XA_STEPS; ++s) {
            const uint4 wf = *reinterpret_cast<const uint4*>(Ws + ((uint32_t)(s * 32) ^ a16));
            acc = E::mfma(wf, xf[s], acc);
        }
        v2u pk[4];
#pragma unroll
        for (int j = 0; j < 4; ++j) {
            const float4 bb = *reinterpret_cast<const float4*>(bias_s + c * 64 + chh * 32 + 8 * j + 4 * hi);
            pk[j] = v2u{E::pack2((acc[4 * j] + bb.x) * p.q_scale, (acc[4 * j + 1] + bb.y) * p.q_scale),
                        E::pack2((acc[4 * j + 2] + bb.z) * p.q_scale, (acc[4 * j + 3] + bb.w) * p.q_scale)};
        }
#pragma unroll
        for (int t = 0; t < 2; ++t) {
            const v4u w = quads_to_wide(pk[2 * t], pk[2 * t + 1]);
            qf[2 * c + t] = make_uint4(w[0], w[1], w[2], w[3]);
        }
    }
    {
        const uint32_t one = (uint32_t)E::fromf(1.0f);
#pragma unroll
        for (int hl = 0; hl < 4; ++hl)
            if (hi == 1) qf[3 * hl + 2].x = (qf[3 * hl + 2].x & 0xffff0000u) | one;
    }

    uint2 og[4][5], pg[4][5];
    const int krot = 3 * ((col >> 3) & 1);
    const char* xown = smem + XA_OFF_X + wave * (5 * 512) + lane * 8;
    const char* xpar = smem + XA_OFF_X + (wave ^ 4) * (5 * 512) + lane * 8;
#pragma unroll
    for (int hl = 0; hl < XA_NKV; ++hl) {
        const int c = XA_NQ + hl;
        dma_wait_keep_n<XA_PIECES>();
        __syncthreads();
        stage(c + 2);
        if (hl > 0) {
#pragma unroll
            for (int j = 0; j < 5; ++j) pg[hl - 1][j] = *reinterpret_cast<const uint2*>(xpar + ((hl - 1) & 1) * XA_XB + j * 512);
        }
        const char* Ks = smem + (c % XA_RING) * XA_CHUNK + chh * XA_HEADB;
        const char* Vs = Ks + XA_KBYTES;
        f32x16 sc[3];
#pragma unroll
        for (int kb = 0; kb < 3; ++kb) {
            sc[kb] = zero16;
#pragma unroll
            for (int t = 0; t < 3; ++t) {
                const uint4 kf = *reinterpret_cast<const uint4*>(Ks + (kb * 32 + col) * XA_KROW + ((2 * t + hi + krot) % 6) * 16);
                sc[kb] = E::mfma(kf, qf[3 * hl + t], sc[kb]);
            }
        }
        float mx = sc[0][0];
#pragma unroll
        for (int kb = 0; kb < 3; ++kb)
#pragma unroll
            for (int r = 0; r < 16; ++r) mx = fmaxf(mx, sc[kb][r]);
        mx = fmaxf(mx, __shfl_xor(mx, 32));
        f32x16 o0 = zero16, o1 = zero16;
#pragma unroll
        for (int kb = 0; kb < 3; ++kb)
#pragma unroll
            for (int g = 0; g < 2; ++g) {
                uint4 pf;
                pf.x = E::pack2(__builtin_amdgcn_exp2f(sc[kb][8 * g + 0] - mx), __builtin_amdgcn_exp2f(sc[kb][8 * g + 1] - mx));
                pf.y = E::pack2(__builtin_amdgcn_exp2f(sc[kb][8 * g + 2] - mx), __builtin_amdgcn_exp2f(sc[kb][8 * g + 3] - mx));
                pf.z = E::pack2(__builtin_amdgcn_exp2f(sc[kb][8 * g + 4] - mx), __builtin_amdgcn_exp2f(sc[kb][8 * g + 5] - mx));
                pf.w = E::pack2(__builtin_amdgcn_exp2f(sc[kb][8 * g + 6] - mx), __builtin_amdgcn_exp2f(sc[kb][8 * g + 7] - mx));
                const int pc = (2 * (2 * kb + g) + hi) * 16;
                const uint4 v0 = *reinterpret_cast<const uint4*>(Vs + col * XA_VROW + pc);
                const uint4 v1 = *reinterpret_cast<const uint4*>(Vs + (32 + (col & 15)) * XA_VROW + pc);
                o0 = E::mfma(v0, pf, o0);
                o1 = E::mfma(v1, pf, o1);
            }
        const float inv = 1.0f / __shfl(o1[4], col);
#pragma unroll
        for (int j = 0; j < 4; ++j)
            og[hl][j] = make_uint2(E::pack2(o0[4 * j] * inv, o0[4 * j + 1] * inv), E::pack2(o0[4 * j + 2] * inv, o0[4 * j + 3] * inv));
        og[hl][4] = make_uint2(E::pack2(o1[0] * inv, o1[1] * inv), E::pack2(o1[2] * inv, o1[3] * inv));
#pragma unroll
        for (int j = 0; j < 5; ++j) *reinterpret_cast<uint2*>(const_cast<char*>(xown) + (hl & 1) * XA_XB + j * 512) = og[hl][j];
    }

    const __amdgpu_buffer_rsrc_t rs_o = __builtin_amdgcn_make_buffer_rsrc(p.out, 0, 0x80000000u, 0x00020000);
    const uint32_t obase = m < p.M ? (uint32_t)m * (uint32_t)(p.out_ld * 2) : OOB;
    const uint32_t roff = (uint32_t)m * (uint32_t)(p.x_ld * 2) + (uint32_t)(chh * 64);
    uint4 rraw[2][2];
    auto load_res = [&](int c) {
#pragma unroll
        for (int t = 0; t < 2; ++t) rraw[c & 1][t] = buf_load16(rs_x, m < p.M ? roff + (uint32_t)(c * 128 + t * 32 + hi * 16) : OOB);
    };
    f32x16 acc[XA_NO];
    auto emit = [&](int c) {
        uint2 rres[4];
#pragma unroll
        for (int t = 0; t < 2; ++t) {
            const uint4 r = wide_to_quads(rraw[c & 1][t]);
            rres[2 * t] = make_uint2(r.x, r.y); rres[2 * t + 1] = make_uint2(r.z, r.w);
        }
        v2u pk[4];
#pragma unroll
        for (int j = 0; j < 4; ++j) {
            const float4 bb = *reinterpret_cast<const float4*>(bias_s + c * 64 + chh * 32 + 8 * j + 4 * hi);
            const float v0 = acc[c][4 * j] + bb.x + E::lo(rres[j].x), v1 = acc[c][4 * j + 1] + bb.y + E::hi(rres[j].x);
            const float v2 = acc[c][4 * j + 2] + bb.z + E::lo(rres[j].y), v3 = acc[c][4 * j + 3] + bb.w + E::hi(rres[j].y);
            pk[j] = v2u{E::pack2(v0, v1), E::pack2(v2, v3)};
        }
#pragma unroll
        for (int t = 0; t < 2; ++t) {
            const v4u w = quads_to_wide(pk[2 * t], pk[2 * t + 1]);
            const uint32_t off = (uint32_t)((c * 64 + chh * 32 + 16 * t + 8 * hi) * 2);
            __builtin_amdgcn_raw_buffer_store_b128(w, rs_o, (int)(obase == OOB ? OOB : obase + off), 0, 0);
        }
    };
    uint4 of[XA_STEPS];
#pragma unroll
    for (int co = 0; co < XA_NO; ++co) {
        const int c = XA_NQ + XA_NKV + co;
        dma_wait();
        __syncthreads();
        if (co == 0) {
#pragma unroll
            for (int j = 0; j < 5; ++j) pg[3][j] = *reinterpret_cast<const uint2*>(xpar + XA_XB + j * 512);
            if (tid < XA_C) bias_s[tid] = bo_v;
#pragma unroll
            for (int s = 0; s < XA_STEPS; ++s) {
                uint2 g2[2];
#pragma unroll
                for (int e = 0; e < 2; ++e) {
                    const int G = 2 * s + e, h = G / 5, j = G % 5;
                    const uint2 mine = og[h & 3][j], theirs = pg[h & 3][j];
                    const bool own = (h >> 2) == chh;
                    g2[e] = make_uint2(own ? mine.x : theirs.x, own ? mine.y : theirs.y);
                }
                of[s] = make_uint4(g2[0].x, g2[0].y, g2[1].x, g2[1].y);
            }
        }
        if (co > 0) emit(co - 1);
        if (c + 2 < XA_NCHUNK) stage(c + 2);
        load_res(co);
        const char* Ws = wlane + (c % XA_RING) * XA_CHUNK;
        acc[co] = zero16;
#pragma unroll
        for (int s = 0; s < XA_STEPS; ++s) {
            const uint4 wf = *reinterpret_cast<const uint4*>(Ws + ((uint32_t)(s * 32) ^ a16));
            acc[co] = E::mfma(wf, of[s], acc[co]);
        }
    }
    emit(XA_NO - 1);
}

}

bool imd_text_xattn320_supported_of(const imd_xattn_params& p) {
    return p.C == XA_C && p.heads == 8 && p.L >= 1 && p.L <= XA_LMAX && p.M > 0 && p.rows_per_image > 0 && (p.rows_per_image % XA_BM) == 0 &&
           (p.M % p.rows_per_image) == 0 && p.kv_bdiv >= 1 && p.text_rows >= 1 && (p.M / p.rows_per_image) == p.text_rows * p.kv_bdiv &&
           p.x_ld >= XA_C && (p.x_ld % 8) == 0 && p.out_ld >= XA_C && (p.out_ld % 8) == 0 &&
           (p.dtype == IMD_DTYPE_BF16 || p.dtype == IMD_DTYPE_F16);
}

int imd_launch_text_xattn320(const imd_xattn_params& p, hipStream_t s) {
    if (!imd_text_xattn320_supported_of(p))
        return imd_set_error("text_xattn320: needs C = 320, 8 heads, 1..96 text keys, rows per image a multiple of 128 and M / rows_per_image == text_rows * kv_bdiv "
                             "(got C=%d heads=%d L=%d M=%d rows_per_image=%d text_rows=%d kv_bdiv=%d x_ld=%d out_ld=%d dtype=%d)",
                             p.C, p.heads, p.L, p.M, p.rows_per_image, p.text_rows, p.kv_bdiv, p.x_ld, p.out_ld, p.dtype);
    if (((size_t)(p.M - 1) * p.x_ld + XA_C) * 2 >= 0x80000000ull || ((size_t)(p.M - 1) * p.out_ld + XA_C) * 2 >= 0x80000000ull)
        return imd_set_error("text_xattn320: operand larger than 2 GiB");
    if (!(p.ln_eps > 0.f)) return imd_set_error("text_xattn320: LayerNorm needs eps > 0");
    const bool h = p.dtype == IMD_DTYPE_F16;
    const void* kern = h ? reinterpret_cast<const void*>(text_xattn320_kernel<true>) : reinterpret_cast<const void*>(text_xattn320_kernel<false>);
    if (int rc_attr = imd_lds_attr(kern, XA_LDS, "text_xattn320")) return rc_attr;
    const dim3 grid((unsigned)(p.M / XA_BM));
    if (h) hipLaunchKernelGGL(text_xattn320_kernel<true>, grid, dim3(512), XA_LDS, s, p);
    else hipLaunchKernelGGL(text_xattn320_kernel<false>, grid, dim3(512), XA_LDS, s, p);
    return imd_check_launch("text_xattn320");
}
```

imagdressing_amd/ops.py:

```python
from __future__ import annotations

import functools
import ctypes as C
from typing import Dict, Optional, Sequence, Tuple

import torch

from . import _lib as L

ACT_NONE, ACT_SILU, ACT_GEGLU, ACT_GELU, ACT_QUICK_GELU = 0, 1, 2, 3, 4
bf16 = torch.bfloat16
f16 = torch.float16
DTYPE_CODE = {torch.bfloat16: 0, torch.float16: 1}


def _code(t: torch.Tensor, name: str = "tensor") -> int:
    try:
        return DTYPE_CODE[t.dtype]
    except KeyError:
        raise L.ImdError(f"{name}: expected a bfloat16 or float16 tensor, got {t.dtype}") from None


try:
    _raw_stream, _cur_dev = torch._C._cuda_getCurrentRawStream, torch._C._cuda_getDevice
# ... 285 lines not shown
    gamma, beta, eps, silu, groups = gn_out
    if not (p.split_k > 1 and p.mode == 0 and not p.out_f32 and p.act == ACT_NONE and not p.res and out_scale == 1.0):
        return False
    p.gn_out_gamma, p.gn_out_beta = _dev(gamma, torch.float32, "gn_out gamma"), _dev(beta, torch.float32, "gn_out beta")
    p.gn_out_eps, p.gn_out_silu, p.gn_out_groups = float(eps), int(bool(silu)), int(groups)
    if lib.imd_conv_gemm_gn_out_supported(C.byref(p)):
        p.splitk_counters = None
        return True
    p.gn_out_gamma, p.gn_out_beta, p.gn_out_groups = None, None, 0
    return False


def _attach_stats(p, lib, cfg: int, split_k: int, groups: int, images: int, device):
    if not (cfg in STATS_EPILOGUE_CFGS or split_k > 1 or (GENERIC_GN_STATS and cfg in TILE_STATS_CFGS)):
        return None
    p.gn_stats_groups = groups
    nparts = lib.imd_conv_gemm_stats_parts(C.byref(p), cfg)
    if nparts <= 0:
        p.gn_stats_groups = 0
        return None
    part = torch.empty((images, nparts, groups, 2), dtype=torch.float32, device=device)
    p.gn_stats_out = part.data_ptr()
    return part, nparts, groups


def conv_gemm(
    x: torch.Tensor, w: torch.Tensor, *, M: int, N: int, Cin: int, taps: int = 1,
    Hin: int = 1, Win: int = 1, Hout: int = 1, Wout: int = 1, stride: int = 1, ups: bool = False,
    x_pix_stride: Optional[int] = None, out: Optional[torch.Tensor] = None, out_ld: Optional[int] = None,
    bias: Optional[torch.Tensor] = None, rowvec: Optional[torch.Tensor] = None, rowvec_stride: int = 0,
    rowvec_off: int = 0, res: Optional[torch.Tensor] = None, res_ld: Optional[int] = None, out_scale: float = 1.0,
    act: int = ACT_NONE, out_f32: bool = False, heads: Optional[dict] = None, cfg: int = -1, split_k: int = 0,
    gn: Optional[tuple] = None, pad_br_only: bool = False, ln_eps: Optional[float] = None, gn_stats_groups: int = 0,
    gn_out: Optional[tuple] = None, gn_in: Optional[tuple] = None,
) -> Optional[torch.Tensor]:
    ensure_device(x.device)
    K = taps * Cin
    p, out, res_rows = _marshal(x, w, M, N, K, Cin, taps, Hin, Win, Hout, Wout, stride, ups, x_pix_stride, out, out_ld, bias, rowvec, rowvec_stride, rowvec_off,
                                res, res_ld, out_scale, act, out_f32, heads, pad_br_only)
    _count("gemm_conv", 2.0 * M * N * K)
    lib = L.load()
    if gn is not None:
        p.gn_a, p.gn_b, p.gn_silu = _dev(gn[0], torch.float32, "gn_a"), _dev(gn[1], torch.float32, "gn_b"), int(gn[2])
        if cfg == -1:
            cfg = PATCH_CFG
    if ln_eps is not None:
        if res_rows:
            res = _periodic_residual(p, res, res_rows, K == 320)
        p.split_k = 1
        L.check(lib.imd_row_linear(C.byref(p), 1, float(ln_eps), _stream()))
        return out
    splittable = heads is None and act != ACT_GEGLU
    if GEMM_TRACE is not None:
        GEMM_TRACE.append(dict(M=M, N=N, K=K, Cin=Cin, taps=taps, Hin=Hin, Win=Win, Hout=Hout, Wout=Wout, stride=stride, ups=int(ups), splittable=splittable, dtype=str(x.dtype),
                               bias=bias is not None, rowvec=rowvec is not None, rowvec_stride=rowvec_stride, res=res is not None, res_rows=res_rows, act=act, out_f32=bool(out_f32),
                               heads=None if heads is None else dict(C=heads["C"], H=heads["H"], D=heads["D"],
                                                                     dests=[(t is not None, kind, DP, Ltok, scale) for t, kind, DP, Ltok, scale in heads["dests"]]),
                               gn_stats_groups=gn_stats_groups, x_pix_stride=p.x_pix_stride, out_scale=out_scale, pad_br_only=bool(pad_br_only),
                               out_ld=p.out_ld, res_ld=p.res_ld, gn=gn is not None, gn_in=gn_in is not None, gn_out=gn_out is not None))
    dkey = hit = None
    if cfg == -1 and split_k == 0 and GEMM_TRACE is None:
        hk = None if heads is None else (heads["C"], heads["H"], heads["D"], tuple((t is None, kind, DP, Ltok) for t, kind, DP, Ltok, _ in heads["dests"]))
        dkey = (M, N, K, Cin, taps, stride, int(ups), Hin, Win, Hout, Wout, p.x_pix_stride, p.res_ld, p.out_ld, act, int(out_f32), int(pad_br_only), p.dtype,
                rowvec is None, res is None, bias is None, hk, PATCH_CONV, id(_GEMM_TABLE))
        hit = _CFG_DECISIONS.get(dkey)
    cfg, split_k = hit or _choose_tile(p, lib, cfg, split_k, splittable)
    if hit is None and dkey is not None and len(_CFG_DECISIONS) < 4096:
        _CFG_DECISIONS[dkey] = (cfg, split_k)
    if res_rows:
        res = _periodic_residual(p, res, res_rows, cfg in PERIODIC_RES_CFGS)
    p.split_k = split_k
    xn = None if gn_in is None else _fuse_gn_in(p, lib, x, gn_in, cfg, M, Hout * Wout)
    if split_k > 1:
        p.splitk_ws = splitk_workspace(split_k * M * N, x.device).data_ptr()
        if SPLITK_IN_KERNEL:
            p.splitk_counters = splitk_counters(x.device).data_ptr()
    if gn_out is not None and FUSED_GN_FINISH and _fuse_gn_out(p, lib, gn_out, out_scale):
        L.check(lib.imd_conv_gemm(C.byref(p), cfg, _stream()))
        out._imd_gn_applied = True
        return out
    stats = None
    if gn_stats_groups and FUSED_GN_STATS and heads is None and not out_f32 and act != ACT_GEGLU:
        stats = _attach_stats(p, lib, cfg, split_k, gn_stats_groups, M // (Hout * Wout), x.device)
    if GEMM_EVENT_HOOK is not None:
        e0, e1 = torch.cuda.Event(enable_timing=True), torch.cuda.Event(enable_timing=True)
        e0.record()
        L.check(lib.imd_conv_gemm(C.byref(p), cfg, _stream()))
        e1.record()
        GEMM_EVENT_HOOK.setdefault((f"{M},{N},{K},{taps},{stride},{int(ups)}|{Hout}x{Wout}", cfg, split_k), []).append((e0, e1))
    else:
        L.check(lib.imd_conv_gemm(C.byref(p), cfg, _stream()))
    if stats is not None:
        out._imd_gn_stats = stats
    return out


_splitk_ws: Dict[Tuple, torch.Tensor] = {}
_splitk_cnt: Dict[Tuple, torch.Tensor] = {}


def splitk_counters(device) -> torch.Tensor:
    key = (str(device), _stream())
    t = _splitk_cnt.get(key)
    if t is None:
        t = torch.zeros(16384, dtype=torch.int32, device=device)
        _splitk_cnt[key] = t
    return t


def splitk_workspace(nfloats: int, device) -> torch.Tensor:
    key = (str(device), _stream())
    t = _splitk_ws.get(key)
    if t is None or t.numel() < nfloats:
        t = torch.empty(max(nfloats, 1 << 22), dtype=torch.float32, device=device)
        _splitk_ws[key] = t
    return t


def linear(x2d: torch.Tensor, w: torch.Tensor, bias=None, *, res=None, act=ACT_NONE, out_f32=False, out=None,
           out_ld=None, res_ld=None, cfg=-1, split_k=0, ln_eps=None) -> torch.Tensor:
    M, K = x2d.shape
    N = w.shape[0]
    return conv_gemm(x2d, w, M=M, N=N, Cin=K, bias=bias, res=res, act=act, out_f32=out_f32, out=out,
                     out_ld=out_ld, res_ld=res_ld, cfg=cfg, split_k=split_k, ln_eps=ln_eps)


def fold_layernorm_affine(w: torch.Tensor, bias: Optional[torch.Tensor], gamma: torch.Tensor, beta: torch.Tensor):
    wf = w.float()
    w2 = (wf * gamma.float()[None, :]).to(w.dtype).contiguous()
    b2 = wf @ beta.float()
    if bias is not None:
        b2 = b2 + bias.float()
    return w2, b2.contiguous()


def pack_ff_fused(w1: torch.Tensor, b1: torch.Tensor, w2: torch.Tensor, b2: torch.Tensor, gamma: Optional[torch.Tensor] = None,
                  beta: Optional[torch.Tensor] = None, dtype=None):
    dtype = dtype or w1.dtype
    inner, C = w2.shape[1], w2.shape[0]
    w1f, b1f = w1.float(), b1.float()
    if gamma is not None:
        b1f = b1f + w1f @ beta.float()
        w1f = w1f * gamma.float()[None, :]
    dev = w1.device
    i = torch.arange(32, device=dev)
    jj = (i & 7) + 8 * (i >> 4)
    gate = ((i >> 3) & 1).bool()
    blk = torch.arange(inner // 16, device=dev)
    src = 16 * blk[:, None] + jj[None, :] + torch.where(gate, inner, 0)[None, :]
    w1p = w1f[src.reshape(-1)].to(dtype).contiguous()
    b1p = b1f[src.reshape(-1)].contiguous()
    ks = torch.arange(16, device=dev)
    jk = torch.where(ks < 4, ks, torch.where(ks < 8, ks + 4, torch.where(ks < 12, ks - 4, ks)))
    cols = (16 * torch.arange(inner // 16, device=dev)[:, None] + jk[None, :]).reshape(inner // 32, 32)
    w2p = w2.float()[:, cols].permute(1, 0, 2).to(dtype).contiguous()
    return dict(w1=w1p, b1=b1p, w2=w2p, b2=b2.float().contiguous(), ln=gamma is not None, C=C, inner=inner)


def ff_geglu_fused(x2d: torch.Tensor, packed: dict, ln_eps: float = 1e-5, out: Optional[torch.Tensor] = None) -> torch.Tensor:
    ensure_device(x2d.device)
    M, C_ = x2d.shape
    dt = x2d.dtype
    if out is None:
        out = torch.empty((M, C_), dtype=dt, device=x2d.device)
    p = L.FfParams()
    p.x, p.w1, p.b1 = _dev(x2d, dt, "x"), _dev(packed["w1"], dt, "w1"), _dev(packed["b1"], torch.float32, "b1")
    p.w2, p.b2, p.out = _dev(packed["w2"], dt, "w2"), _dev(packed["b2"], torch.float32, "b2"), _dev(out, dt, "out")
    p.M, p.C, p.inner, p.x_ld, p.out_ld = M, packed["C"], packed["inner"], x2d.stride(0), out.stride(0)
    p.ln, p.ln_eps, p.dtype = int(packed["ln"]), float(ln_eps), _code(x2d, "x")
    _count("gemm_conv", 2.0 * M * packed["C"] * 2 * packed["inner"] + 2.0 * M * packed["inner"] * packed["C"])
    L.check(L.load().imd_ff_geglu(C.byref(p), _stream()))
    return out


FUSED_XATTN = _os.environ.get("IMD_FUSED_XATTN", "1") != "0"
XATTN_C, XATTN_HEADS, XATTN_D, XATTN_DP, XATTN_LMAX = 320, 8, 40, 48, 96
XATTN_CHUNK = 64 * 320
XATTN_VROW = 104
XATTN_HEAD = XATTN_LMAX * XATTN_DP + XATTN_DP * XATTN_VROW
XATTN_PAD_KEY = -30000.0
_XATTN_W: Dict[Tuple, tuple] = {}
_XATTN_KV: Dict[int, tuple] = {}
_clear_hooks.append(_XATTN_W.clear)
_clear_hooks.append(_XATTN_KV.clear)


def xattn_q_rows(device=None):
    i = torch.arange(6 * 64, device=device)
    r = i % 64
    R = 32 * (i // 64) + r % 32
    head, dim = 4 * (r // 32) + R // 48, R % 48
    return head * XATTN_D + dim.clamp(max=XATTN_D - 1), dim < XATTN_D


def xattn_o_cols(device=None):
    k = torch.arange(XATTN_C, device=device)
    s, hi, e = k // 16, (k % 16) // 8, k % 8
    G = 2 * s + e // 4
    return (G // 5) * XATTN_D + 8 * (G % 5) + 4 * hi + e % 4


def xattn_swizzle_rows(w2d: torch.Tensor) -> torch.Tensor:
    R = w2d.shape[0]
    r = torch.arange(R, device=w2d.device) % 64
    pos = torch.arange(40, device=w2d.device)[None, :] ^ ((r >> 1) & 7)[:, None]
    return w2d.reshape(R, 40, 8).gather(1, pos[:, :, None].expand(R, 40, 8)).reshape(R, XATTN_C).contiguous()


def xattn_key_cols(device=None):
    c = torch.arange(XATTN_LMAX, device=device)
    c16 = c % 16
    return (c // 16) * 16 + (c16 & 3) + 8 * ((c16 >> 2) & 1) + 4 * (c16 >> 3)


def xattn_k_pieces(device=None):
    r = torch.arange(XATTN_LMAX, device=device)
    return (torch.arange(6, device=device)[None, :] - 3 * ((r >> 3) & 1)[:, None]) % 6


def _pack_text_xattn(wq, bq, wo, bo):
    dev, dt = wq.device, wq.dtype
    src, valid = xattn_q_rows(dev)
    wq_p = torch.where(valid[:, None], wq[src], torch.zeros((), dtype=dt, device=dev))
    bq_p = torch.where(valid, bq.float()[src], torch.zeros((), dtype=torch.float32, device=dev)).contiguous()
    wo_p = wo[:, xattn_o_cols(dev)]
    w = torch.cat([xattn_swizzle_rows(wq_p), xattn_swizzle_rows(wo_p)], 0).contiguous()
    bo_p = torch.zeros(XATTN_C, dtype=torch.float32, device=dev) if bo is None else bo.float().contiguous()
    return dict(w=w, bq=bq_p, bo=bo_p)


def pack_text_xattn(wq: torch.Tensor, bq: torch.Tensor, wo: torch.Tensor, bo: Optional[torch.Tensor]):
    if tuple(wq.shape) != (XATTN_C, XATTN_C) or tuple(wo.shape) != (XATTN_C, XATTN_C) or wq.dtype != wo.dtype:
        raise L.ImdError(f"pack_text_xattn: expected two [320, 320] matrices of one dtype, got {tuple(wq.shape)} {wq.dtype}, {tuple(wo.shape)} {wo.dtype}")
    srcs = (wq, bq, wo, bo)
    key = tuple(None if t is None else (t.data_ptr(), t._version, t.dtype, str(t.device)) for t in srcs)
    ent = _XATTN_W.get(key)
    if ent is None:
        if len(_XATTN_W) > 64:
            _XATTN_W.clear()
        ent = _XATTN_W[key] = (srcs, _pack_text_xattn(wq, bq, wo, bo))
    return ent[1]


def _pack_text_kv(k, vt, Lk):
    Bt, dev, dt = k.shape[0], k.device, k.dtype
    H, D, DP, LM = XATTN_HEADS, XATTN_D, XATTN_DP, XATTN_LMAX
    kf = torch.zeros(Bt, H, LM, DP, dtype=dt, device=dev)
    kf[:, :, :Lk, :D] = k[:, :, :Lk, :D]
    kf[:, :, Lk:, D] = XATTN_PAD_KEY
    kimg = kf.view(Bt, H, LM, 6, 8).gather(3, xattn_k_pieces(dev)[None, None, :, :, None].expand(Bt, H, LM, 6, 8))
    vf = torch.zeros(Bt, H, DP, LM, dtype=dt, device=dev)
    vf[:, :, :D, :Lk] = vt[:, :, :D, :Lk]
    vf[:, :, D, :] = 1.0
    vimg = torch.zeros(Bt, H, DP, XATTN_VROW, dtype=dt, device=dev)
    vimg[..., :LM] = vf[..., xattn_key_cols(dev)]
    head = torch.cat([kimg.reshape(Bt, H, LM * DP), vimg.reshape(Bt, H, DP * XATTN_VROW)], -1)
    img = torch.zeros(Bt, 4, XATTN_CHUNK, dtype=dt, device=dev)
    img[:, :, :XATTN_HEAD] = head[:, :4]
    img[:, :, XATTN_HEAD:2 * XATTN_HEAD] = head[:, 4:]
    return img


def pack_text_kv(k: torch.Tensor, vt: torch.Tensor, Lk: int) -> torch.Tensor:
    if k.dim() != 4 or k.shape[1] != XATTN_HEADS or k.shape[3] != XATTN_DP or not (1 <= Lk <= XATTN_LMAX) or k.shape[2] < Lk \
            or vt.shape[:2] != k.shape[:2] or vt.shape[2] < XATTN_D or vt.shape[3] < Lk:
        raise L.ImdError(f"pack_text_kv: expected K [Bt, 8, L, 48] / V^T [Bt, 8, >= 40, >= L] with L <= 96, got {tuple(k.shape)} / {tuple(vt.shape)}, L = {Lk}")
    hit = _XATTN_KV.get(id(k))
    if hit is not None and hit[0] is k and hit[1] is vt and hit[2] == Lk:
        return hit[3]
    if len(_XATTN_KV) > 64:
        _XATTN_KV.clear()
    img = _pack_text_kv(k, vt, Lk)
    _XATTN_KV[id(k)] = (k, vt, Lk, img)
    return img


def text_xattn_supported(C_: int, heads: int, N: int, Lk: int) -> bool:
    return C_ == XATTN_C and heads == XATTN_HEADS and N % 128 == 0 and 1 <= Lk <= XATTN_LMAX


def text_xattn(x: torch.Tensor, packed: dict, kv_img: torch.Tensor, *, Lk: int, kv_bdiv: int = 1, ln_eps: float = 1e-5,
               q_scale: Optional[float] = None, out: Optional[torch.Tensor] = None) -> torch.Tensor:
    ensure_device(x.device)
    B, N, C_ = x.shape
    dt = x.dtype
    if out is None:
        out = torch.empty((B, N, C_), dtype=dt, device=x.device)
    if kv_img.dim() != 3 or tuple(kv_img.shape[1:]) != (4, XATTN_CHUNK):
        raise L.ImdError(f"text_xattn: kv_img must be [Bt, 4, {XATTN_CHUNK}], got {tuple(kv_img.shape)}")
    p = L.XattnParams()
    p.x, p.w, p.out = _dev(x, dt, "x"), _dev(packed["w"], dt, "w"), _dev(out, dt, "out")
    p.bq, p.bo, p.kv = _dev(packed["bq"], torch.float32, "bq"), _dev(packed["bo"], torch.float32, "bo"), _dev(kv_img, dt, "kv_img")
    p.M, p.C, p.heads, p.L = B * N, C_, XATTN_HEADS, int(Lk)
    p.rows_per_image, p.kv_bdiv, p.text_rows = N, int(kv_bdiv), kv_img.shape[0]
    p.x_ld = p.out_ld = C_
    p.q_scale = float(XATTN_D ** -0.5 * 1.4426950408889634 if q_scale is None else q_scale)
    p.ln_eps, p.dtype = float(ln_eps), _code(x, "x")
    _count("gemm_conv", 2 * 2.0 * B * N * C_ * C_)
    _count("attention", 4.0 * XATTN_HEADS * N * XATTN_D * B * Lk)
    L.check(L.load().imd_text_xattn320(C.byref(p), _stream()))
    return out


def conv2d_nhwc(x: torch.Tensor, w: torch.Tensor, bias=None, *, taps=9, stride=1, ups=False, rowvec=None,
                rowvec_stride=0, rowvec_off=0, res=None, out_scale=1.0, act=ACT_NONE, out_f32=False, cfg=-1, split_k=0, gn=None,
                pad_br_only=False, gn_stats_groups=0, gn_out=None, gn_in=None) -> torch.Tensor:
    B, H, W, Cin = x.shape
    Cout = w.shape[0]
    Hl, Wl = (2 * H, 2 * W) if ups else (H, W)
    Ho, Wo = ((Hl + stride - 1) // stride, (Wl + stride - 1) // stride)
    M = B * Ho * Wo
    out = conv_gemm(x, w, M=M, N=Cout, Cin=Cin, taps=taps, Hin=H, Win=W, Hout=Ho, Wout=Wo, stride=stride, ups=ups,
                    bias=bias, rowvec=rowvec, rowvec_stride=rowvec_stride, rowvec_off=rowvec_off, res=res, out_scale=out_scale, act=act,
                    out_f32=out_f32, cfg=cfg, split_k=split_k, gn=gn, pad_br_only=pad_br_only, gn_stats_groups=gn_stats_groups, gn_out=gn_out, gn_in=gn_in)
    r = out.view(B, Ho, Wo, -1)
    if getattr(out, "_imd_gn_applied", False):
        r._imd_gn_applied = True
    st = getattr(out, "_imd_gn_stats", None)
    if st is not None:
        r._imd_gn_stats = st
    return r


UPS_PHASE = _os.environ.get("IMD_UPS_PHASE", "1") != "0"
UPS_PHASE_TAPS = (((0,), (1, 2)), ((0, 1), (2,)))
UPS_PHASE_CFG = "ups_phase"
_UPS_W: Dict[Tuple, tuple] = {}
_UPS_OK: Dict[Tuple, bool] = {}
_clear_hooks.append(_UPS_W.clear)
_clear_hooks.append(_UPS_OK.clear)


def _pack_upsample_phase(w: torch.Tensor, dtype=None) -> torch.Tensor:
    N, Cp = w.shape[0], w.shape[1] // 9
    acc_dt = torch.float32 if w.dtype in DTYPE_CODE else w.dtype
    w9 = w.to(acc_dt).view(N, 3, 3, Cp)
    out = torch.zeros(4, N, 4, Cp, dtype=acc_dt, device=w.device)
    for py in range(2):
        for px in range(2):
            for dy in range(2):
                for dx in range(2):
                    for ky in UPS_PHASE_TAPS[py][dy]:
                        for kx in UPS_PHASE_TAPS[px][dx]:
                            out[2 * py + px, :, 2 * dy + dx] += w9[:, ky, kx]
    return out.to(w.dtype if dtype is None else dtype).contiguous()


def pack_upsample_phase(w: torch.Tensor, dtype=None) -> torch.Tensor:
    if w.dim() != 2 or w.shape[1] % 9:
        raise L.ImdError(f"pack_upsample_phase: expected a packed 3x3 weight [Cout, 9 * Cin], got {tuple(w.shape)}")
    key = (w.data_ptr(), w._version, w.dtype, str(w.device), tuple(w.shape), dtype)
    ent = _UPS_W.get(key)
    if ent is None:
        if len(_UPS_W) > 64:
            _UPS_W.clear()
        ent = _UPS_W[key] = (w, _pack_upsample_phase(w, dtype))
    return ent[1]


def _ups_phase_block(shape, N: int, dtype):
    B, H, W, Cin = shape
    p = L.ConvGemmParams()
    p.flags = _gemm_call_flags()
    p.dtype, p.M, p.N, p.K, p.Cin, p.taps = DTYPE_CODE[dtype], 4 * B * H * W, N, 9 * Cin, Cin, 9
    p.Hin, p.Win, p.Hout, p.Wout, p.stride, p.ups = H, W, 2 * H, 2 * W, 1, 1
    p.x_pix_stride, p.out_ld, p.res_ld, p.out_scale, p.split_k = Cin, N, N, 1.0, 1
    return p


def conv_ups_phase_supported(x: torch.Tensor, w: torch.Tensor, bias=None) -> bool:
    if x.dim() != 4 or w.dim() != 2 or w.shape[1] != 9 * x.shape[3] or x.dtype not in DTYPE_CODE or w.dtype != x.dtype or not x.is_contiguous():
        return False
    key = (tuple(x.shape), w.shape[0], x.dtype)
    ok = _UPS_OK.get(key)
    if ok is None:
        ok = bool(L.load().imd_conv_ups_phase_supported(C.byref(_ups_phase_block(x.shape, w.shape[0], x.dtype))))
        if len(_UPS_OK) < 4096:
            _UPS_OK[key] = ok
    return ok


def conv_ups_phase(x: torch.Tensor, w: torch.Tensor, bias=None, *, out: Optional[torch.Tensor] = None,
                   phase_weights: Optional[torch.Tensor] = None) -> torch.Tensor:
    ensure_device(x.device)
    B, H, W, Cin = x.shape
    N = w.shape[0]
    M, K = 4 * B * H * W, 9 * Cin
    dt = x.dtype
    if w.dim() != 2 or tuple(w.shape) != (N, K) or w.dtype != dt:
        raise L.ImdError(f"conv_ups_phase: expected a packed 3x3 weight [{N}, {K}] of {dt}, got {tuple(w.shape)} {w.dtype}")
    wp = pack_upsample_phase(w) if phase_weights is None else phase_weights
    if tuple(wp.shape) != (4, N, 4, Cin):
        raise L.ImdError(f"conv_ups_phase: phase weights must be [4, {N}, 4, {Cin}], got {tuple(wp.shape)}")
    if out is None:
        out = torch.empty((B, 2 * H, 2 * W, N), dtype=dt, device=x.device)
    elif out.numel() != M * N:
        raise L.ImdError(f"conv_ups_phase: out has {out.numel()} elements, expected {M * N}")
    p = _ups_phase_block(x.shape, N, dt)
    p.x, p.w, p.out = _dev(x, dt, "x"), _dev(wp, dt, "phase weights"), _dev(out, dt, "out")
    p.bias = None if bias is None else _dev(bias, torch.float32, "bias")
    _count("gemm_conv", 2.0 * M * N * K)
    if GEMM_TRACE is not None:
        GEMM_TRACE.append(dict(M=M, N=N, K=K, Cin=Cin, taps=9, Hin=H, Win=W, Hout=2 * H, Wout=2 * W, stride=1, ups=1, splittable=True, dtype=str(x.dtype),
                               bias=bias is not None, rowvec=False, rowvec_stride=0, res=False, res_rows=0, act=ACT_NONE, out_f32=False, heads=None,
                               gn_stats_groups=0, x_pix_stride=Cin, out_scale=1.0, pad_br_only=False, out_ld=N, res_ld=N, gn=False, gn_in=False, gn_out=False,
                               ups_phase=True))
    lib = L.load()
    if GEMM_EVENT_HOOK is not None:
        e0, e1 = torch.cuda.Event(enable_timing=True), torch.cuda.Event(enable_timing=True)
        e0.record()
        L.check(lib.imd_conv_ups_phase(C.byref(p), _stream()))
        e1.record()
        GEMM_EVENT_HOOK.setdefault((f"{M},{N},{K},9,1,1|{2 * H}x{2 * W}", UPS_PHASE_CFG, 1), []).append((e0, e1))
    else:
        L.check(lib.imd_conv_ups_phase(C.byref(p), _stream()))
    return out.view(B, 2 * H, 2 * W, N)


ATTN_EVENT_HOOK = None


FUSED_OUT_PROJ = _os.environ.get("IMD_FUSED_OUT_PROJ", "0") == "1"


def attention_proj_supported(H: int, N: int, D: int) -> bool:
    return D == 40 and H * D == 320 and N >= 512


_proj_cnt: Dict[Tuple, torch.Tensor] = {}


def proj_counters(n: int, device) -> torch.Tensor:
    key = (str(device), _stream())
    t = _proj_cnt.get(key)
    if t is None or t.numel() < n:
        t = torch.zeros(max(n, 4096), dtype=torch.int32, device=device)
        _proj_cnt[key] = t
    return t


def attention_dup_supported(H: int, N: int, D: int) -> bool:
    return bool(L.load().imd_attention_dup_supported(H, N, D))


ATTN_PHASE_SPLIT = _os.environ.get("IMD_ATTN_PHASE_SPLIT", "1") != "0"
ATTN_PHASE_SPLIT_MAX_N = int(_os.environ.get("IMD_ATTN_PHASE_SPLIT_MAX_N", "512"))


@functools.lru_cache(maxsize=None)
def attention_phase_split_supported(D: int) -> bool:
    return bool(L.load().imd_attention_phase_split_supported(D))


def attention(q, k1, v1t, out, *, B, H, N, D, L1, L1P, kv1_bdiv=1, k2=None, v2t=None, scale2=None,
              L2=0, L2P=0, kv2_bdiv=1, out_ld=None, causal=False, k_pad_one=False, proj=None, out_dup=None, phase2_rows=0):
    ensure_device(q.device)
    p = L.AttnParams()
    dt = q.dtype
    p.dtype = _code(q, "q")
    p.q, p.k1, p.v1t = _dev(q, dt, "q"), _dev(k1, dt, "k1"), _dev(v1t, dt, "v1t")
    p.k2, p.v2t = _opt(k2, dt, "k2"), _opt(v2t, dt, "v2t")
    p.scale2 = _opt(scale2, torch.float32, "scale2")
    p.out = _dev(out, dt, "out")
    p.B, p.H, p.N, p.D = B, H, N, D
    p.L1, p.L1P, p.kv1_bdiv = L1, L1P, kv1_bdiv
    p.L2, p.L2P, p.kv2_bdiv = L2, L2P, kv2_bdiv
    p.out_ld = H * D if out_ld is None else out_ld
    p.causal = int(causal)
    p.k_pad_one = int(bool(k_pad_one))
    p.flags = _attn_call_flags()
    if out_dup is not None:
        if out_dup.numel() != out.numel():
            raise L.ImdError("attention: out_dup must have the shape of out")
        p.out_dup = _dev(out_dup, dt, "out_dup")
    if phase2_rows and ATTN_PHASE_SPLIT and k2 is not None and scale2 is not None and proj is None and out_dup is None and not causal \
            and 0 < phase2_rows <= B and attention_phase_split_supported(D) and N <= ATTN_PHASE_SPLIT_MAX_N:
        p.phase2_rows = int(phase2_rows)
        p.phase2_out = workspace("attn_phase2", (phase2_rows * N * H * D,), torch.float32, q.device).data_ptr()
    ret = out
    if proj is not None:
        pw, pb, pres, pout = proj
        Cc = H * D
        if pw.numel() != Cc * Cc or pout.numel() != B * N * Cc or (pres is not None and pres.numel() != B * N * Cc):
            raise L.ImdError(f"attention: fused out-projection operands do not match B={B} N={N} C={Cc}")
        p.proj_w, p.proj_b = _dev(pw, dt, "proj_w"), _opt(pb, torch.float32, "proj_b")
        p.proj_res, p.proj_out = _opt(pres, dt, "proj_res"), _dev(pout, dt, "proj_out")
        p.proj_res_ld = p.proj_out_ld = Cc
        p.proj_counters = proj_counters(B * ((N + 255) // 256), q.device).data_ptr()
        ret = pout
        _count("gemm", 2.0 * B * N * Cc * Cc)
    if FLOP_COUNTER is not None:
        rows2 = 0 if (k2 is None or scale2 is None) else int((scale2 != 0).sum().item())
        _count("attention", 4.0 * H * N * D * (B * L1 * (0.5 if causal else 1.0) + rows2 * L2))
    hook = ATTN_EVENT_HOOK
    if hook is not None and hook["match"](B=B, H=H, N=N, D=D, L1=L1, L2=L2 if k2 is not None else 0):
        e0, e1 = torch.cuda.Event(enable_timing=True), torch.cuda.Event(enable_timing=True)
        e0.record()
        L.check(L.load().imd_attention(C.byref(p), _stream()))
        e1.record()
        hook["events"].append((e0, e1))
        return ret
    L.check(L.load().imd_attention(C.byref(p), _stream()))
    return ret


ATTN_FP8 = False
FP8_EXPS = dict(q=4, k=2, v=3)


def quantize_fp8_rows(x: torch.Tensor, exp: int, pad_val: float = 0.0) -> torch.Tensor:
    ensure_device(x.device)
    if x.shape[-1] != 48:
        raise L.ImdError(f"quantize_fp8_rows: expected head-dim-40 rows padded to 48, got {tuple(x.shape)}")
    rows = x.numel() // 48
    out = torch.empty(x.shape[:-1] + (64,), dtype=torch.uint8, device=x.device)
    L.check(L.load().imd_attn_quantize_fp8(_dev(x, x.dtype, "x"), out.data_ptr(), 0, rows, 0, exp, float(pad_val), _code(x, "x"), _stream()))
    return out


def quantize_fp8_vt(vt: torch.Tensor, exp: int) -> torch.Tensor:
    ensure_device(vt.device)
    if vt.shape[-2] != 64 or vt.shape[-1] % 64:
        raise L.ImdError(f"quantize_fp8_vt: expected [.., 64, LP] with LP % 64 == 0, got {tuple(vt.shape)}")
    LP = vt.shape[-1]
    groups = vt.numel() // (64 * LP)
    out = torch.zeros(vt.shape, dtype=torch.uint8, device=vt.device)
    L.check(L.load().imd_attn_quantize_fp8(_dev(vt, vt.dtype, "vt"), out.data_ptr(), 1, groups, LP, exp, 0.0, _code(vt, "vt"), _stream()))
    return out


def attention_fp8(q8, k1, v1t, out, *, B, H, N, L1, L1P, kv1_bdiv=1, k2=None, v2t=None, scale2=None, L2=0, L2P=0, kv2_bdiv=1,
                  out_ld=None, exps=None):
    ensure_device(out.device)
    e = dict(FP8_EXPS, **(exps or {}))
    u8 = torch.uint8
    p = L.AttnParams()
    p.dtype = _code(out, "out")
    p.q, p.k1, p.v1t = _dev(q8, u8, "q8"), _dev(k1, u8, "k1"), _dev(v1t, u8, "v1t")
    p.k2, p.v2t = _opt(k2, u8, "k2"), _opt(v2t, u8, "v2t")
    p.scale2 = _opt(scale2, torch.float32, "scale2")
    p.out = _dev(out, out.dtype, "out")
    p.B, p.H, p.N, p.D = B, H, N, 40
    p.L1, p.L1P, p.kv1_bdiv = L1, L1P, kv1_bdiv
    p.L2, p.L2P, p.kv2_bdiv = L2, L2P, kv2_bdiv
    p.out_ld = H * 40 if out_ld is None else out_ld
    L.check(L.load().imd_attention_fp8(C.byref(p), e["q"], e["k"], e["v"], _stream()))
    return out


def group_norm(x: torch.Tensor, gamma, beta, *, groups=32, eps=1e-5, silu=False, out=None) -> torch.Tensor:
    ensure_device(x.device)
    B, Cc = x.shape[0], x.shape[-1]
    HW = x.numel() // (B * Cc)
    if out is None:
        out = torch.empty_like(x)
    lib = L.load()
    nws = lib.imd_groupnorm_workspace_floats(B, HW, Cc, groups)
    part = workspace("gn_partial", (max(nws, 1),), torch.float32, x.device)
    p = L.GroupNormParams()
    p.dtype = _code(x, "x")
    p.x, p.y = _dev(x, x.dtype, "x"), _dev(out, x.dtype, "out")
    p.gamma, p.beta = _dev(gamma, torch.float32, "gamma"), _dev(beta, torch.float32, "beta")
    p.partial = part.data_ptr()
    p.B, p.HW, p.C, p.G, p.x_ld, p.y_ld = B, HW, Cc, groups, Cc, Cc
    p.eps, p.silu = eps, int(silu)
    st = getattr(x, "_imd_gn_stats", None)
    if st is not None and st[2] == groups and st[0].shape[0] == B and FUSED_GN_STATS:
        p.partial, p.nparts = st[0].data_ptr(), st[1]
    L.check(lib.imd_groupnorm(C.byref(p), _stream()))
    return out


def group_norm_coeffs(x: torch.Tensor, gamma, beta, *, groups=32, eps=1e-5):
    ensure_device(x.device)
    B, Cc = x.shape[0], x.shape[-1]
    HW = x.numel() // (B * Cc)
    lib = L.load()
    nws = lib.imd_groupnorm_workspace_floats(B, HW, Cc, groups)
    part = workspace("gn_partial", (max(nws, 1),), torch.float32, x.device)
    ab = torch.empty((2, B, Cc), dtype=torch.float32, device=x.device)
    p = L.GroupNormParams()
    p.dtype = _code(x, "x")
    p.x, p.y = _dev(x, x.dtype, "x"), None
    p.gamma, p.beta = _dev(gamma, torch.float32, "gamma"), _dev(beta, torch.float32, "beta")
    p.partial = part.data_ptr()
    p.B, p.HW, p.C, p.G, p.x_ld, p.y_ld = B, HW, Cc, groups, Cc, Cc
    p.eps, p.silu = eps, 0
    st = getattr(x, "_imd_gn_stats", None)
    if st is not None and st[2] == groups and st[0].shape[0] == B and FUSED_GN_STATS:
        p.partial, p.nparts = st[0].data_ptr(), st[1]
    L.check(lib.imd_groupnorm_coeffs(C.byref(p), ab[0].data_ptr(), ab[1].data_ptr(), _stream()))
    return ab[0], ab[1]


def lincomb(terms, out: Optional[torch.Tensor] = None) -> torch.Tensor:
    xs = [t for _, t in terms]
    ensure_device(xs[0].device)
    n, numel = len(terms), xs[0].numel()
    for t in xs:
        if t.numel() != numel:
            raise L.ImdError("lincomb: all tensors must have the same number of elements")
    if out is None:
        out = torch.empty_like(xs[0])
    ptrs = (C.c_void_p * n)(*[_dev(t, torch.float32, "lincomb input") for t in xs])
    coefs = (C.c_float * n)(*[float(c) for c, _ in terms])
    L.check(L.load().imd_lincomb(ptrs, coefs, n, _dev(out, torch.float32, "out"), numel, _stream()))
# ... 402 lines not shown
```

imagdressing_amd/unet.py:

```python
from __future__ import annotations

import math
from types import SimpleNamespace
from typing import Dict, List, Optional

import torch

from . import ops
from .hub import PretrainedMixin

FUSED_LN_CHANNELS = (320, 640, 1280)

bf16 = torch.bfloat16

SD15_CONFIG = dict(
    in_channels=4, out_channels=4, block_out_channels=(320, 640, 1280, 1280), layers_per_block=2,
    attention_head_dim=8, cross_attention_dim=768, norm_num_groups=32, sample_size=64,
    down_attn=(True, True, True, False), time_cond_proj_dim=None,
)


def _resnet_shapes(p, cin, cout, temb):
    s = {f"{p}.norm1.weight": (cin,), f"{p}.norm1.bias": (cin,),
         f"{p}.conv1.weight": (cout, cin, 3, 3), f"{p}.conv1.bias": (cout,),
         f"{p}.time_emb_proj.weight": (cout, temb), f"{p}.time_emb_proj.bias": (cout,),
         f"{p}.norm2.weight": (cout,), f"{p}.norm2.bias": (cout,),
         f"{p}.conv2.weight": (cout, cout, 3, 3), f"{p}.conv2.bias": (cout,)}
    if cin != cout:
        s[f"{p}.conv_shortcut.weight"] = (cout, cin, 1, 1)
        s[f"{p}.conv_shortcut.bias"] = (cout,)
    return s


def _transformer_shapes(p, ch, cross):
    s = {f"{p}.norm.weight": (ch,), f"{p}.norm.bias": (ch,),
         f"{p}.proj_in.weight": (ch, ch, 1, 1), f"{p}.proj_in.bias": (ch,),
         f"{p}.proj_out.weight": (ch, ch, 1, 1), f"{p}.proj_out.bias": (ch,)}
    b = f"{p}.transformer_blocks.0"
    for n in ("norm1", "norm2", "norm3"):
        s[f"{b}.{n}.weight"] = (ch,); s[f"{b}.{n}.bias"] = (ch,)
    for a, kd in (("attn1", ch), ("attn2", cross)):
        s[f"{b}.{a}.to_q.weight"] = (ch, ch)
        s[f"{b}.{a}.to_k.weight"] = (ch, kd)
        s[f"{b}.{a}.to_v.weight"] = (ch, kd)
        s[f"{b}.{a}.to_out.0.weight"] = (ch, ch); s[f"{b}.{a}.to_out.0.bias"] = (ch,)
    s[f"{b}.ff.net.0.proj.weight"] = (8 * ch, ch); s[f"{b}.ff.net.0.proj.bias"] = (8 * ch,)
    s[f"{b}.ff.net.2.weight"] = (ch, 4 * ch); s[f"{b}.ff.net.2.bias"] = (ch,)
    return s


def _encoder_shapes(cfg):
    boc = cfg["block_out_channels"]
    temb, cross = boc[0] * 4, cfg["cross_attention_dim"]
    s = {"conv_in.weight": (boc[0], cfg["in_channels"], 3, 3), "conv_in.bias": (boc[0],),
         "time_embedding.linear_1.weight": (temb, boc[0]), "time_embedding.linear_1.bias": (temb,),
         "time_embedding.linear_2.weight": (temb, temb), "time_embedding.linear_2.bias": (temb,)}
    out = boc[0]
    for i, ch in enumerate(boc):
        cin, out = out, ch
        for j in range(2):
            s.update(_resnet_shapes(f"down_blocks.{i}.resnets.{j}", cin if j == 0 else out, out, temb))
            if cfg["down_attn"][i]:
                s.update(_transformer_shapes(f"down_blocks.{i}.attentions.{j}", out, cross))
        if i != len(boc) - 1:
            s[f"down_blocks.{i}.downsamplers.0.conv.weight"] = (out, out, 3, 3)
            s[f"down_blocks.{i}.downsamplers.0.conv.bias"] = (out,)
    s.update(_resnet_shapes("mid_block.resnets.0", boc[-1], boc[-1], temb))
    s.update(_resnet_shapes("mid_block.resnets.1", boc[-1], boc[-1], temb))
    s.update(_transformer_shapes("mid_block.attentions.0", boc[-1], cross))
    return s


def unet_param_shapes(cfg=None) -> Dict[str, tuple]:
    cfg = dict(SD15_CONFIG, **(cfg or {}))
    boc = cfg["block_out_channels"]
    temb, cross = boc[0] * 4, cfg["cross_attention_dim"]
    s = _encoder_shapes(cfg)
    rev = list(reversed(boc))
    up_attn = list(reversed(cfg["down_attn"]))
    out = rev[0]
    for i, ch in enumerate(rev):
        prev, out = out, ch
        inp = rev[min(i + 1, len(boc) - 1)]
        for j in range(3):
            skip = inp if j == 2 else out
            rin = prev if j == 0 else out
            s.update(_resnet_shapes(f"up_blocks.{i}.resnets.{j}", rin + skip, out, temb))
            if up_attn[i]:
                s.update(_transformer_shapes(f"up_blocks.{i}.attentions.{j}", out, cross))
        if i != len(boc) - 1:
            s[f"up_blocks.{i}.upsamplers.0.conv.weight"] = (out, out, 3, 3)
            s[f"up_blocks.{i}.upsamplers.0.conv.bias"] = (out,)
    s["conv_norm_out.weight"] = (boc[0],); s["conv_norm_out.bias"] = (boc[0],)
    s["conv_out.weight"] = (cfg["out_channels"], boc[0], 3, 3); s["conv_out.bias"] = (cfg["out_channels"],)
    return s


def controlnet_param_shapes(cfg=None, cond_channels=3, embed_channels=(16, 32, 96, 256)) -> Dict[str, tuple]:
    cfg = dict(SD15_CONFIG, **(cfg or {}))
    boc = cfg["block_out_channels"]
    s = _encoder_shapes(cfg)
    e = "controlnet_cond_embedding"
    s[f"{e}.conv_in.weight"] = (embed_channels[0], cond_channels, 3, 3); s[f"{e}.conv_in.bias"] = (embed_channels[0],)
    for i in range(len(embed_channels) - 1):
        a, b = embed_channels[i], embed_channels[i + 1]
        s[f"{e}.blocks.{2 * i}.weight"] = (a, a, 3, 3); s[f"{e}.blocks.{2 * i}.bias"] = (a,)
        s[f"{e}.blocks.{2 * i + 1}.weight"] = (b, a, 3, 3); s[f"{e}.blocks.{2 * i + 1}.bias"] = (b,)
    s[f"{e}.conv_out.weight"] = (boc[0], embed_channels[-1], 3, 3); s[f"{e}.conv_out.bias"] = (boc[0],)
    chans = [boc[0]]
    for i, ch in enumerate(boc):
        chans += [ch, ch] + ([ch] if i != len(boc) - 1 else [])
    for i, ch in enumerate(chans):
        s[f"controlnet_down_blocks.{i}.weight"] = (ch, ch, 1, 1); s[f"controlnet_down_blocks.{i}.bias"] = (ch,)
    s["controlnet_mid_block.weight"] = (boc[-1], boc[-1], 1, 1); s["controlnet_mid_block.bias"] = (boc[-1],)
    return s


def random_state_dict(shapes: Dict[str, tuple], seed: int, device="cpu", dtype=torch.float32, zero_convs=False):
    device = torch.device(device)
    g = torch.Generator(device=device).manual_seed(seed)

    def randn(shape):
        return torch.randn(shape, generator=g, device=device)
    sd = {}
    for name, shape in shapes.items():
        if name.endswith(".bias"):
            t = randn(shape) * 0.02
        elif ".norm" in name or name.startswith("conv_norm_out"):
            t = 1.0 + randn(shape) * 0.05
        else:
            fan_in = 1
            for d in shape[1:]:
                fan_in *= d
            t = randn(shape) * (1.0 / math.sqrt(fan_in))
            if zero_convs and name.startswith(("controlnet_down_blocks", "controlnet_mid_block")):
                t = t * 0.1
        sd[name] = t.to(dtype=dtype)
    return sd


def _f32(t, device):
    return t.detach().to(device=device, dtype=torch.float32).contiguous()


class LinearOp:

    def __init__(self, weight: torch.Tensor, bias: Optional[torch.Tensor], device, dtype=bf16):
        self.weight = weight.detach().to(device=device, dtype=dtype).contiguous()
        self.bias = None if bias is None else _f32(bias, device)
        self.out_features, self.in_features = self.weight.shape

    def __call__(self, x: torch.Tensor, **kw) -> torch.Tensor:
        x2 = x.to(self.weight.dtype).contiguous().view(-1, self.in_features)
        return ops.linear(x2, self.weight, self.bias, **kw).view(*x.shape[:-1], self.out_features)


class ConvOp:

    def __init__(self, weight: torch.Tensor, bias: Optional[torch.Tensor], device, dtype=bf16):
        cout, cin, kh, kw = weight.shape
        assert (kh, kw) in ((1, 1), (3, 3))
        cin_p = (cin + 7) // 8 * 8
        w = weight.detach().to(device=device, dtype=torch.float32).permute(0, 2, 3, 1)
        if cin_p != cin:
            w = torch.nn.functional.pad(w, (0, cin_p - cin))
        cout_p = (cout + 3) // 4 * 4
        self.weight = w.reshape(cout, kh * kw * cin_p).to(dtype).contiguous()
        self.bias = None if bias is None else _f32(bias, device)
        self.cin, self.cin_p, self.cout, self.taps = cin, cin_p, cout, kh * kw
        assert cout_p == cout, "output channels must be a multiple of 4"

    def __call__(self, x, **kw):
        if ops.UPS_PHASE and self.taps == 9 and kw == {"ups": True} and ops.conv_ups_phase_supported(x, self.weight, self.bias):
            return ops.conv_ups_phase(x, self.weight, self.bias)
        return ops.conv2d_nhwc(x, self.weight, self.bias, taps=self.taps, **kw)


class NormParams:
    def __init__(self, sd, prefix, device):
        self.weight = _f32(sd[prefix + ".weight"], device)
        self.bias = _f32(sd[prefix + ".bias"], device)


class _Identity:
    def __call__(self, x):
        return x


class Attention:

    def __init__(self, sd, prefix, heads, device, dtype=bf16):
        self.heads = heads
        self.dtype = dtype
        self.to_q = LinearOp(sd[f"{prefix}.to_q.weight"], None, device, dtype)
        self.to_k = LinearOp(sd[f"{prefix}.to_k.weight"], None, device, dtype)
        self.to_v = LinearOp(sd[f"{prefix}.to_v.weight"], None, device, dtype)
        self.to_out = [LinearOp(sd[f"{prefix}.to_out.0.weight"], sd[f"{prefix}.to_out.0.bias"], device, dtype), _Identity()]
        self.query_dim = self.to_q.out_features
        self.is_cross = self.to_k.in_features != self.query_dim
        self.spatial_norm = None
        self.group_norm = None
        self.norm_cross = None
        self.residual_connection = False
        self.rescale_output_factor = 1.0
        self.processor = None

    def prepare_attention_mask(self, mask, *a, **k):
        return mask

    def set_processor(self, p):
        self.processor = p

    def __call__(self, hidden_states, encoder_hidden_states=None, residual=None, layernorm=None, **cross_attention_kwargs):
        proc = self.processor
        if layernorm is not None:
            nrm, eps = layernorm
            if (getattr(proc, "fused_layernorm", False) and getattr(proc, "fused_residual", False) and ops.FUSED_LN
                    and (hidden_states.shape[-1] in FUSED_LN_CHANNELS if encoder_hidden_states is not None
                         else hidden_states.shape[-1] == 320)):
                cross_attention_kwargs = dict(cross_attention_kwargs, imd_layernorm=(nrm.weight, nrm.bias, eps))
            else:
                hidden_states = ops.layer_norm(hidden_states, nrm.weight, nrm.bias, eps)
        if getattr(proc, "fused_residual", False):
            return proc(self, hidden_states, encoder_hidden_states=encoder_hidden_states, attention_mask=None,
                        imd_residual=residual, **cross_attention_kwargs)
        out = proc(self, hidden_states, encoder_hidden_states=encoder_hidden_states, attention_mask=None,
                   **cross_attention_kwargs)
        out = out.to(self.dtype).contiguous()
        return out if residual is None else ops.add(out, residual)


class TransformerBlock:
    def __init__(self, sd, p, ch, heads, device, dtype=bf16):
        self.norm1 = NormParams(sd, f"{p}.norm1", device)
        self.norm2 = NormParams(sd, f"{p}.norm2", device)
        self.norm3 = NormParams(sd, f"{p}.norm3", device)
        self.attn1 = Attention(sd, f"{p}.attn1", heads, device, dtype)
        self.attn2 = Attention(sd, f"{p}.attn2", heads, device, dtype)
        w, b = sd[f"{p}.ff.net.0.proj.weight"], sd[f"{p}.ff.net.0.proj.bias"]
        inner = w.shape[0] // 2
        wi = torch.stack([w[:inner], w[inner:]], dim=1).reshape(2 * inner, w.shape[1])
        bi = torch.stack([b[:inner], b[inner:]], dim=1).reshape(2 * inner)
        self.ff_in = LinearOp(wi, bi, device, dtype)
        self.ff_out = LinearOp(sd[f"{p}.ff.net.2.weight"], sd[f"{p}.ff.net.2.bias"], device, dtype)
        self.ff_fused = None
        if ch == 320 and inner == 4 * ch:
            self.ff_fused = ops.pack_ff_fused(w.to(device), b.to(device), sd[f"{p}.ff.net.2.weight"].to(device),
                                              sd[f"{p}.ff.net.2.bias"].to(device), self.norm3.weight, self.norm3.bias, dtype=dtype)

    def __call__(self, h, ehs, cak):
        h = self.attn1(h, encoder_hidden_states=None, residual=h, layernorm=(self.norm1, 1e-5), **cak)
        return self.after_attn1(h, ehs, cak)

    def after_attn1(self, h, ehs, cak):
        h = self.attn2(h, encoder_hidden_states=ehs, residual=h, layernorm=(self.norm2, 1e-5), **cak)
        B, L, Cc = h.shape
        if self.ff_fused is not None and ops.FUSED_FF and B * L >= ops.FUSED_FF_MIN_ROWS:
            return ops.ff_geglu_fused(h.view(B * L, Cc), self.ff_fused, 1e-5).view(B, L, Cc)
        n = ops.layer_norm(h, self.norm3.weight, self.norm3.bias)
        g = ops.linear(n.view(B * L, Cc), self.ff_in.weight, self.ff_in.bias, act=ops.ACT_GEGLU)
        return ops.linear(g, self.ff_out.weight, self.ff_out.bias, res=h.view(B * L, Cc)).view(B, L, Cc)


class Transformer2D:
    def __init__(self, sd, p, ch, heads, groups, device, dtype=bf16):
        self.norm = NormParams(sd, f"{p}.norm", device)
        self.proj_in = ConvOp(sd[f"{p}.proj_in.weight"], sd[f"{p}.proj_in.bias"], device, dtype)
        self.proj_out = ConvOp(sd[f"{p}.proj_out.weight"], sd[f"{p}.proj_out.bias"], device, dtype)
        self.transformer_blocks = [TransformerBlock(sd, f"{p}.transformer_blocks.0", ch, heads, device, dtype)]
        self.groups = groups

    def __call__(self, x, ehs, cak):
        B, H, W, Cc = x.shape
        h = self.proj_in(x, gn_in=(self.norm.weight, self.norm.bias, 1e-6, False, self.groups)).view(B, H * W, Cc)
        for blk in self.transformer_blocks:
            h = blk(h, ehs, cak)
        return self.proj_out(h.view(B, H, W, Cc), res=x, gn_stats_groups=self.groups)

    def pair_half_ok(self, x_half, cak) -> bool:
        blk = self.transformer_blocks[0]
        proc = blk.attn1.processor
        sa = cak.get("sa_hidden_states")
        Bh, H, W, Cc = x_half.shape
        return bool(cak.get("sa_pair_layout") and cak.get("sa_batch_mask") is not None and sa is not None
                    and getattr(proc, "fused_pair_half", False) and getattr(proc, "fused_residual", False)
                    and getattr(proc, "name", None) in sa and not ops.ATTN_FP8 and not ops.FUSED_OUT_PROJ
                    and ops.attention_dup_supported(blk.attn1.heads, H * W, Cc // blk.attn1.heads))

    def call_pair_half(self, x_half, ehs, cak):
        Bh, H, W, Cc = x_half.shape
        blk = self.transformer_blocks[0]
        h = self.proj_in(x_half, gn_in=(self.norm.weight, self.norm.bias, 1e-6, False, self.groups)).view(Bh, H * W, Cc)
        r = h
        h = blk.attn1(h, encoder_hidden_states=None, residual=r, layernorm=(blk.norm1, 1e-5), imd_pair_half=True, **cak)
        h = blk.after_attn1(h, ehs, cak)
        return self.proj_out(h.view(2 * Bh, H, W, Cc), res=x_half)


def _temb_stride(temb_all):
    return temb_all.shape[1] if temb_all.shape[0] > 1 else 0


class ResnetBlock:
    def __init__(self, sd, p, groups, device, temb_slices: list, dtype=bf16):
        self.norm1 = NormParams(sd, f"{p}.norm1", device)
        self.norm2 = NormParams(sd, f"{p}.norm2", device)
        self.conv1 = ConvOp(sd[f"{p}.conv1.weight"], sd[f"{p}.conv1.bias"], device, dtype)
        self.conv2 = ConvOp(sd[f"{p}.conv2.weight"], sd[f"{p}.conv2.bias"], device, dtype)
        self.shortcut = None
        if f"{p}.conv_shortcut.weight" in sd:
            self.shortcut = ConvOp(sd[f"{p}.conv_shortcut.weight"], sd[f"{p}.conv_shortcut.bias"], device, dtype)
        self.groups = groups
        self.temb_off = sum(w.shape[0] for w, _ in temb_slices)
        temb_slices.append((sd[f"{p}.time_emb_proj.weight"], sd[f"{p}.time_emb_proj.bias"]))

    def __call__(self, x, temb_all):
        if ops.FUSED_GN_CONV and x.shape[2] >= 32 and x.shape[1] >= 8:
            a, b = ops.group_norm_coeffs(x, self.norm1.weight, self.norm1.bias, groups=self.groups, eps=1e-5)
            h = self.conv1(x, rowvec=temb_all, rowvec_stride=_temb_stride(temb_all), rowvec_off=self.temb_off, gn_stats_groups=self.groups, gn=(a, b, True))
            a, b = ops.group_norm_coeffs(h, self.norm2.weight, self.norm2.bias, groups=self.groups, eps=1e-5)
            sc = x if self.shortcut is None else self.shortcut(x)
            return self.conv2(h, res=sc, gn_stats_groups=self.groups, gn=(a, b, True))
        h = ops.group_norm(x, self.norm1.weight, self.norm1.bias, groups=self.groups, eps=1e-5, silu=True)
        h = self.conv1(h, rowvec=temb_all, rowvec_stride=_temb_stride(temb_all), rowvec_off=self.temb_off, gn_stats_groups=self.groups,
                       gn_out=(self.norm2.weight, self.norm2.bias, 1e-5, True, self.groups))
        if not getattr(h, "_imd_gn_applied", False):
            h = ops.group_norm(h, self.norm2.weight, self.norm2.bias, groups=self.groups, eps=1e-5, silu=True)
        sc = x if self.shortcut is None else self.shortcut(x)
        return self.conv2(h, res=sc, gn_stats_groups=self.groups)


class DeepCache:

    def __init__(self, depth: int = 1):
        self.depth = int(depth)
        self.full = True
        self._feat: Optional[torch.Tensor] = None
        self._sig = None
        self._ctrl_sig = None

    def check_depth(self, layers_per_block: int):
        if not 1 <= self.depth <= layers_per_block + 1:
            raise ValueError(f"deepcache depth must be in 1 .. {layers_per_block + 1} (layers_per_block + 1), got {self.depth}")

    @staticmethod
    def _signature(x, depth):
        return (x.shape[0], x.shape[1], x.shape[2], x.dtype, depth)

    def store(self, h: torch.Tensor, x: torch.Tensor):
        if self._feat is None or self._feat.shape != h.shape or self._feat.dtype != h.dtype or self._feat.device != h.device:
            self._feat = torch.empty(h.shape, dtype=h.dtype, device=h.device)
        ops.copy_into(self._feat, h)
        self._sig = self._signature(x, self.depth)

    def load(self, x: torch.Tensor) -> torch.Tensor:
        self._match(self._sig, x, "UNet")
        return self._feat

    def note_controlnet(self, x: torch.Tensor):
        self._ctrl_sig = self._signature(x, self.depth)

    def check_controlnet(self, x: torch.Tensor):
        self._match(self._ctrl_sig, x, "ControlNet")

    def _match(self, sig, x, who):
        if sig is None:
            raise ValueError(f"deepcache: shallow {who} forward before any full one (the first call of a loop must be full)")
        want = self._signature(x, self.depth)
        if sig != want:
            raise ValueError(f"deepcache: the cache holds (batch, height, width, dtype, depth) = {sig} and this {who} forward has {want}")

    def clear(self):
        self._feat = self._sig = self._ctrl_sig = None


class _Encoder(PretrainedMixin):
    _config_keys = ("in_channels", "out_channels", "block_out_channels", "layers_per_block", "attention_head_dim",
                    "cross_attention_dim", "norm_num_groups", "sample_size")

    def _build_encoder(self, sd, cfg, device):
        boc = cfg["block_out_channels"]
        g, heads = cfg["norm_num_groups"], cfg["attention_head_dim"]
        self._temb_slices: list = []
        self.conv_in = ConvOp(sd["conv_in.weight"], sd["conv_in.bias"], device, self.dtype)
        self.time_lin1 = LinearOp(sd["time_embedding.linear_1.weight"], sd["time_embedding.linear_1.bias"], device, self.dtype)
        self.time_lin2 = LinearOp(sd["time_embedding.linear_2.weight"], sd["time_embedding.linear_2.bias"], device, self.dtype)
        self.down_blocks = []
        self._attn: Dict[str, Attention] = {}
        for i, ch in enumerate(boc):
            blk = SimpleNamespace(resnets=[], attentions=[], downsampler=None)
            for j in range(2):
                blk.resnets.append(ResnetBlock(sd, f"down_blocks.{i}.resnets.{j}", g, device, self._temb_slices, self.dtype))
                if cfg["down_attn"][i]:
                    blk.attentions.append(self._transformer(sd, f"down_blocks.{i}.attentions.{j}", ch, heads, g, device))
            if i != len(boc) - 1:
                blk.downsampler = ConvOp(sd[f"down_blocks.{i}.downsamplers.0.conv.weight"],
                                         sd[f"down_blocks.{i}.downsamplers.0.conv.bias"], device, self.dtype)
            self.down_blocks.append(blk)

    def _build_mid(self, sd, cfg, device):
        boc = cfg["block_out_channels"]
        g, heads = cfg["norm_num_groups"], cfg["attention_head_dim"]
        self.mid_block = SimpleNamespace(
            resnets=[ResnetBlock(sd, "mid_block.resnets.0", g, device, self._temb_slices, self.dtype)],
            attentions=[self._transformer(sd, "mid_block.attentions.0", boc[-1], heads, g, device)])
        self.mid_block.resnets.append(ResnetBlock(sd, "mid_block.resnets.1", g, device, self._temb_slices, self.dtype))

    def _transformer(self, sd, p, ch, heads, groups, device):
        t = Transformer2D(sd, p, ch, heads, groups, device, self.dtype)
        b = t.transformer_blocks[0]
        self._attn[f"{p}.transformer_blocks.0.attn1.processor"] = b.attn1
        self._attn[f"{p}.transformer_blocks.0.attn2.processor"] = b.attn2
        return t

    def _finish_temb(self, device):
        w = torch.cat([w for w, _ in self._temb_slices], dim=0)
        b = torch.cat([b for _, b in self._temb_slices], dim=0)
        self.temb_proj = LinearOp(w, b, device, self.dtype)
        del self._temb_slices

    @property
    def attn_processors(self) -> Dict[str, object]:
        return {name: a.processor for name, a in self._attn.items()}

    def set_attn_processor(self, processor):
        if isinstance(processor, dict):
            missing = set(self._attn) - set(processor)
            if missing:
                raise ValueError(f"set_attn_processor: {len(missing)} processor names missing, e.g. {sorted(missing)[0]}")
            for name, a in self._attn.items():
                a.set_processor(processor[name])
        else:
            for a in self._attn.values():
                a.set_processor(processor)

    def _time_embed(self, timestep, B, device):
        fixed = self.__dict__.get("_temb_fixed")
        if fixed is not None:
            return fixed
        tab = self.__dict__.get("_temb_table")
        if tab is not None and not torch.is_tensor(timestep):
            i = tab[1].get(float(timestep))
            if i is not None:
                return tab[0][i:i + 1]
        if not torch.is_tensor(timestep):
            t = torch.full((B,), float(timestep), dtype=torch.float32, device=device)
        else:
            t = timestep.to(device=device, dtype=torch.float32).reshape(-1).expand(B).contiguous()
        return self._time_embed_rows(t)

    def _time_embed_rows(self, t):
        e = ops.f32_to_16(ops.timestep_embedding(t, self.time_lin1.in_features), self.dtype)
        e = ops.linear(e, self.time_lin1.weight, self.time_lin1.bias, act=ops.ACT_SILU)
        e = ops.linear(e, self.time_lin2.weight, self.time_lin2.bias, act=ops.ACT_SILU)
        return ops.linear(e, self.temb_proj.weight, self.temb_proj.bias, out_f32=True)

    def precompute_time_embeddings(self, timesteps, device):
        ts = [float(t) for t in timesteps]
        table = self._time_embed_rows(torch.tensor(ts, dtype=torch.float32).to(device))
        self._temb_table = (table, {k: i for i, k in enumerate(ts)})
        return table

    def use_time_embedding(self, row):
        self._temb_fixed = row

    def clear_time_embeddings(self):
        self._temb_table = None
        self._temb_fixed = None

    def _run_down(self, x, temb_all, ehs, cak, pair_skip=None, pair_attn_done=False, layers: Optional[int] = None):
        skips = [x if pair_skip is None else pair_skip]
        first = pair_skip is not None
        if layers == 0:
            return x, skips
        for blk in self.down_blocks:
            for j, r in enumerate(blk.resnets):
                if first:
                    first = False
                    if blk.attentions and not pair_attn_done:
                        x = blk.attentions[j](x, ehs, cak)
                else:
                    x = r(x, temb_all)
                    if blk.attentions:
                        x = blk.attentions[j](x, ehs, cak)
                skips.append(x)
                if layers is not None and len(skips) > layers:
                    return x, skips
            if blk.downsampler is not None:
                x = blk.downsampler(x, stride=2, gn_stats_groups=self.cfg["norm_num_groups"])
                skips.append(x)
        return x, skips

    def _run_mid(self, x, temb_all, ehs, cak):
        x = self.mid_block.resnets[0](x, temb_all)
        x = self.mid_block.attentions[0](x, ehs, cak)
        return self.mid_block.resnets[1](x, temb_all)


def _default_processor():
    from .adapter.attention_processor import AttnProcessor2_0
    return AttnProcessor2_0()


def nchw_to_nhwc8(x: torch.Tensor, dtype=bf16) -> torch.Tensor:
    B, Cc, H, W = x.shape
    out = torch.zeros(B, H, W, (Cc + 7) // 8 * 8, dtype=dtype, device=x.device)
    out[..., :Cc] = x.permute(0, 2, 3, 1)
    return out


class UNet2DConditionModel(_Encoder):
    def __init__(self, state_dict: Dict[str, torch.Tensor], config: Optional[dict] = None, device="cuda", dtype=bf16):
        cfg = dict(SD15_CONFIG, **(config or {}))
        if dtype not in ops.DTYPE_CODE:
            raise ValueError(f"dtype must be torch.bfloat16 or torch.float16, got {dtype}")
        want = unet_param_shapes(cfg)
        missing = [k for k in want if k not in state_dict]
        if missing:
            raise KeyError(f"UNet state dict is missing {len(missing)} keys, e.g. {missing[0]}")
        for k, shp in want.items():
            if tuple(state_dict[k].shape) != shp:
                raise ValueError(f"{k}: shape {tuple(state_dict[k].shape)} != expected {shp}")
        self.cfg = cfg
        self._ctor_config = config
        self.config = SimpleNamespace(**cfg)
        self.device = torch.device(device)
        self.dtype = dtype
        sd, dev = state_dict, self.device
        boc = cfg["block_out_channels"]
        g, heads = cfg["norm_num_groups"], cfg["attention_head_dim"]
        self._build_encoder(sd, cfg, dev)
        enc_attn = self._attn
        self._attn = {}
        self.up_blocks = []
        rev = list(reversed(boc))
        up_attn = list(reversed(cfg["down_attn"]))
        self._build_mid(sd, cfg, dev)
        mid_attn = self._attn
        self._attn = {}
        for i, ch in enumerate(rev):
            blk = SimpleNamespace(resnets=[], attentions=[], upsampler=None)
            for j in range(3):
                blk.resnets.append(ResnetBlock(sd, f"up_blocks.{i}.resnets.{j}", g, dev, self._temb_slices, self.dtype))
                if up_attn[i]:
                    blk.attentions.append(self._transformer(sd, f"up_blocks.{i}.attentions.{j}", ch, heads, g, dev))
            if i != len(boc) - 1:
                blk.upsampler = ConvOp(sd[f"up_blocks.{i}.upsamplers.0.conv.weight"],
                                       sd[f"up_blocks.{i}.upsamplers.0.conv.bias"], dev, self.dtype)
            self.up_blocks.append(blk)
        up_attn_map = self._attn
        self._attn = {**enc_attn, **up_attn_map, **mid_attn}
        self._finish_temb(dev)
        self.conv_norm_out = NormParams(sd, "conv_norm_out", dev)
        self.conv_out = ConvOp(sd["conv_out.weight"], sd["conv_out.bias"], dev, self.dtype)
        self.set_attn_processor(_default_processor())

    @classmethod
    def random_init(cls, seed: int = 0, config: Optional[dict] = None, device="cuda", dtype=bf16):
        cfg = dict(SD15_CONFIG, **(config or {}))
        return cls(random_state_dict(unet_param_shapes(cfg), seed, device=device), cfg, device, dtype)

    def forward_nhwc(self, x: torch.Tensor, timestep, encoder_hidden_states: torch.Tensor,
                     cross_attention_kwargs: Optional[dict] = None,
                     down_block_additional_residuals: Optional[List[torch.Tensor]] = None,
                     mid_block_additional_residual: Optional[torch.Tensor] = None, cfg_pair: bool = False,
                     deepcache: Optional[DeepCache] = None) -> torch.Tensor:
        cak = dict(cross_attention_kwargs or {})
        B, H, W, _ = x.shape
        ehs = encoder_hidden_states
        shallow = None
        if deepcache is not None:
            deepcache.check_depth(len(self.down_blocks[0].resnets))
            if not deepcache.full:
                feat = deepcache.load(x)
                shallow = deepcache.depth - 1
        temb_all = self._time_embed(timestep, B, x.device)
        if shallow == 0:
            dedup = cfg_pair and B % 2 == 0 and ops.CFG_PAIR_DEDUP
            h, skips = None, [self.conv_in(x[:B // 2] if dedup else x, gn_stats_groups=self.cfg["norm_num_groups"])]
        elif cfg_pair and B % 2 == 0 and ops.CFG_PAIR_DEDUP:
            h0 = self.conv_in(x[:B // 2], gn_stats_groups=self.cfg["norm_num_groups"])
            blk0 = self.down_blocks[0]
            r0 = blk0.resnets[0](h0, temb_all)
            if ops.CFG_PAIR_ATTN and blk0.attentions and blk0.attentions[0].pair_half_ok(r0, cak):
                h = blk0.attentions[0].call_pair_half(r0, ehs, cak)
                h, skips = self._run_down(h, temb_all, ehs, cak, pair_skip=h0, pair_attn_done=True, layers=shallow)
            else:
                h, skips = self._run_down(ops.repeat_batch(r0), temb_all, ehs, cak, pair_skip=h0, layers=shallow)
        else:
            h = self.conv_in(x, gn_stats_groups=self.cfg["norm_num_groups"])
            h, skips = self._run_down(h, temb_all, ehs, cak, layers=shallow)
        ctrl = down_block_additional_residuals
        cut = None if deepcache is None else len(self.up_blocks[-1].resnets) - deepcache.depth
        if shallow is None:
            h = self._run_mid(h, temb_all, ehs, cak)
            if mid_block_additional_residual is not None:
                h = ops.add(h, mid_block_additional_residual)
# ... 134 lines not shown
```

include/imagdressing_hip.h:

```cpp
#ifndef IMAGDRESSING_HIP_H
#define IMAGDRESSING_HIP_H

#include <stdint.h>

#ifdef __cplusplus
extern "C" {
#endif

#define IMD_ABI_VERSION 9

enum { IMD_ACT_NONE = 0, IMD_ACT_SILU = 1, IMD_ACT_GEGLU = 2, IMD_ACT_GELU = 3, IMD_ACT_QUICK_GELU = 4  };
enum { IMD_OUT_ROWMAJOR = 0, IMD_OUT_HEADS = 1 };
enum { IMD_DTYPE_BF16 = 0, IMD_DTYPE_F16 = 1 };

typedef struct imd_heads_dest {
    uint16_t* ptr;
    int kind;
    int DP;
    int L;
    float scale;
} imd_heads_dest;

#define IMD_TUNING_PER_CALL 0x5A000000
#define IMD_TUNING_TAG_MASK 0xFF000000u

typedef struct imd_conv_gemm_params {
    uint32_t struct_bytes;
    const uint16_t* x;
    const uint16_t* w;
    void* out;
    int M, N, K;
    int Cin, taps, Hin, Win, Hout, Wout, stride, ups;
    int x_pix_stride;
    int out_ld, res_ld;
    const float* bias;
    const float* rowvec;
    int rowvec_stride;
    const uint16_t* res;
    float out_scale;
    int act;
    int out_f32;
    int mode;
    int hC, hH, hD;
    imd_heads_dest hd[3];
    int dtype;
    int split_k;
    float* splitk_ws;
    uint32_t x_bytes, w_bytes;
    int flags;
    const float* gn_a;
    const float* gn_b;
    int gn_silu;
    int pad_br_only;
    int* splitk_counters;
    float* gn_stats_out;
    int gn_stats_groups;
    const float* gn_in_partial;
    const float* gn_in_gamma;
    const float* gn_in_beta;
    int gn_in_nparts, gn_in_groups, gn_in_silu;
    float gn_in_eps;
    const float* gn_out_gamma;
    const float* gn_out_beta;
    float gn_out_eps;
    int gn_out_silu;
    int gn_out_groups;
    int res_rows;
} imd_conv_gemm_params;
#define IMD_SPLITK_COUNTERS 16384

typedef struct imd_attn_params {
    uint32_t struct_bytes;
    const uint16_t* q;
    const uint16_t* k1;
    const uint16_t* v1t;
    const uint16_t* k2;
    const uint16_t* v2t;
    const float* scale2;
    uint16_t* out;
    int B, H, N, D;
    int L1, L1P, kv1_bdiv;
    int L2, L2P, kv2_bdiv;
    int out_ld;
    int dtype;
    int flags;
    int causal;
    int k_pad_one;
    const uint16_t* proj_w;
    const float* proj_b;
    const uint16_t* proj_res;
    uint16_t* proj_out;
    int proj_res_ld, proj_out_ld;
    int* proj_counters;
    uint16_t* out_dup;
    float* phase2_out;
    int phase2_rows;
} imd_attn_params;

typedef struct imd_ff_params {
    uint32_t struct_bytes;
    const uint16_t* x;
    const uint16_t* w1;
    const float* b1;
    const uint16_t* w2;
    const float* b2;
    uint16_t* out;
    int M, C, inner;
    int x_ld, out_ld;
    int ln;
    float ln_eps;
    int dtype;
} imd_ff_params;

typedef struct imd_xattn_params {
    uint32_t struct_bytes;
    const uint16_t* x;
    const uint16_t* w;
    const float* bq;
    const float* bo;
    const uint16_t* kv;
    uint16_t* out;
    int M, C, heads, L;
    int rows_per_image;
    int kv_bdiv, text_rows;
    int x_ld, out_ld;
    float q_scale;
    float ln_eps;
    int dtype;
} imd_xattn_params;

typedef struct imd_groupnorm_params {
    uint32_t struct_bytes;
    const uint16_t* x; uint16_t* y; const float* gamma; const float* beta;
    float* partial;
    int B, HW, C, G, x_ld, y_ld;
    float eps;
    int silu;
    int dtype;
    int nparts;
} imd_groupnorm_params;

typedef struct imd_layernorm_params {
    uint32_t struct_bytes;
    const uint16_t* x; uint16_t* y; const float* gamma; const float* beta;
    int rows, C, x_ld, y_ld;
    float eps;
    int dtype;
} imd_layernorm_params;

typedef struct imd_ddim_params {
    uint32_t struct_bytes;
    float* z;
    const float* eps;
    uint16_t* x_next;
    int B, HW;
    float guidance, sqrt_a_t, sqrt_1m_a_t, sqrt_a_prev, sqrt_1m_a_prev;
    const float* mask;
    const float* z_img;
    const float* noise;
    float sqrt_a_next, sqrt_1m_a_next;
    int dtype;
    const float* coefs;
    const float* var_noise;
    float sigma;
} imd_ddim_params;

#define IMD_SAMPLER_MAX_HISTORY 4
#define IMD_SAMPLER_COEFS 13
typedef struct imd_sampler_params {
    uint32_t struct_bytes;
    float* z;
    const float* eps;
    uint16_t* x_next;
    float* hist;
    int B, HW, K;
    int dtype;
    float guidance;
    const float* guidance_rows;
    float m_x, m_e, z_x, z_m;
    float z_h[4];
    float z_n, b_img, b_noise, in_scale;
    int store;
    const float* noise;
    const float* mask;
    const float* z_img;
    const float* blend_noise;
    const float* coefs;
} imd_sampler_params;

enum { IMD_IMG_U8 = 0, IMD_IMG_F32_NCHW = 1, IMD_IMG_16_NHWC8 = 2 };
#define IMD_IMG_FORCE_TWO_PASS 1
#define IMD_IMG_TILE_W 32
#define IMD_IMG_TILE_H 8
#define IMD_IMG_LDS_BYTES 32768
typedef struct imd_image_resample_params {
    uint32_t struct_bytes;
    const uint8_t* src;
    int64_t src_row_stride, src_img_stride;
    void* out;
    uint8_t* tmp;
    int B, Hin, Win, C;
    int Hres, Wres;
    const int32_t* h_xmin;
    const int32_t* h_count;
    const int32_t* h_k;
    int h_kmax, h_taps;
    const int32_t* v_xmin;
    const int32_t* v_count;
    const int32_t* v_k;
    int v_kmax, v_taps;
    int v_tile_rows;
    int top, left, crop_h, crop_w;
    int kind;
    int dtype;
    int binarize;
    int flags;
    float a[3], b[3];
} imd_image_resample_params;

typedef struct imd_image_pack_params {
    uint32_t struct_bytes;
    const uint16_t* src;
    uint8_t* out;
    int B, H, W, ld;
    int dtype;
} imd_image_pack_params;

typedef struct imd_image_overlay_params {
    uint32_t struct_bytes;
    const uint8_t* orig;
    const uint8_t* mask;
    const uint8_t* gen;
    uint8_t* out;
    int B, Bo;
    int H0, W0;
    int x1, y1, cw, ch;
} imd_image_overlay_params;

typedef struct imd_image_inpaint_condition_params {
    uint32_t struct_bytes;
    const uint8_t* image;
    const uint8_t* mask;
    void* out;
    int B, H, W;
    int dtype;
} imd_image_inpaint_condition_params;

int imd_abi_version(void);
const char* imd_last_error(void);
int imd_device_check(int device);

int imd_conv_gemm(const imd_conv_gemm_params* p, int cfg, void* stream);
int imd_conv_gemm_auto_cfg(int M, int N);
int imd_conv_gemm_auto_split(int M, int N, int K, int cfg);

int imd_attention(const imd_attn_params* p, void* stream);
int imd_attention_fp8(const imd_attn_params* p, int eq, int ek, int ev, void* stream);
int imd_attn_quantize_fp8(const uint16_t* src, uint8_t* dst, int kind, long count, int LP, int exp2_scale, float pad_val, int dtype,
                          void* stream);
int imd_row_linear_gn_in_supported(const imd_conv_gemm_params* p, int cfg);
int imd_conv_gemm_gn_out_supported(const imd_conv_gemm_params* p);
int imd_attention_dup_supported(int H, int N, int D);
int imd_attention_phase_split_supported(int D);
int imd_attn_padded_dims(int D, int* dpk, int* dpv);
int imd_set_tuning(int knob, int value);
int imd_get_tuning(int knob);

int imd_groupnorm(const imd_groupnorm_params* p, void* stream);
int imd_groupnorm_workspace_floats(int B, int HW, int C, int G);
int imd_groupnorm_coeffs(const imd_groupnorm_params* p, float* coef_a, float* coef_b, void* stream);
int imd_conv_patch_supported(const imd_conv_gemm_params* p);
int imd_conv_patch2_supported(const imd_conv_gemm_params* p);
int imd_conv_patch3_supported(const imd_conv_gemm_params* p);
int imd_conv_patch4_supported(const imd_conv_gemm_params* p);
int imd_conv_img_supported(const imd_conv_gemm_params* p);
int imd_conv_patch_stats_parts(const imd_conv_gemm_params* p);
int imd_conv_gemm_stats_parts(const imd_conv_gemm_params* p, int cfg);
int imd_gemm_dma_supported(const imd_conv_gemm_params* p);

int imd_row_linear(const imd_conv_gemm_params* p, int ln, float ln_eps, void* stream);
int imd_row_linear_supported(const imd_conv_gemm_params* p);

int imd_ff_geglu(const imd_ff_params* p, void* stream);

int imd_text_xattn320(const imd_xattn_params* p, void* stream);
int imd_text_xattn320_supported(const imd_xattn_params* p);

int imd_conv_ups_phase(const imd_conv_gemm_params* p, void* stream);
int imd_conv_ups_phase_supported(const imd_conv_gemm_params* p);

int imd_layernorm(const imd_layernorm_params* p, void* stream);
int imd_softmax_rows(const float* s, int s_ld, uint16_t* p, int p_ld, int rows, int cols, int dtype, void* stream);

int imd_ddim_cfg_step(const imd_ddim_params* p, void* stream);
int imd_ddim_cfg_step_rows(const imd_ddim_params* p, const float* guidance, void* stream);
int imd_sampler_step(const imd_sampler_params* p, void* stream);
#define IMD_SAMPLER_ROW_FLOATS 16
int imd_sampler_step_rows(const imd_sampler_params* p, const float* coef_rows , void* stream);

int imd_image_resample(const imd_image_resample_params* p, void* stream);
int imd_image_resample_form(const imd_image_resample_params* p);
int imd_image_pack_u8(const imd_image_pack_params* p, void* stream);
int imd_image_overlay(const imd_image_overlay_params* p, void* stream);
int imd_image_inpaint_condition(const imd_image_inpaint_condition_params* p, void* stream);

int imd_timestep_embedding(const float* t, float* out, int B, int dim, void* stream);

int imd_add(const uint16_t* a, int a_ld, const uint16_t* b, int b_ld, uint16_t* out, int out_ld, long rows, int C, float b_scale, int dtype, void* stream);
int imd_embed_tokens(const uint16_t* table, int vocab, const uint16_t* pos, int T, const int64_t* ids, uint16_t* out, long rows, int C,
                     int dtype, void* stream);
int imd_vit_assemble(const uint16_t* patches, const uint16_t* cls, const uint16_t* pos, uint16_t* out, int B, int P, int C, int dtype,
                     void* stream);
int imd_lincomb(const float* const* xs, const float* coefs, int n, float* out, long numel, void* stream);
int imd_copy2d(const uint16_t* a, int a_ld, uint16_t* out, int out_ld, long rows, int C, void* stream);
int imd_concat2(const uint16_t* a, int Ca, const uint16_t* b, int Cb, const uint16_t* b_add, uint16_t* out, long rows, long b_rows, int dtype, void* stream);
int imd_concat2_gn_stats(const uint16_t* a, int Ca, const uint16_t* b, int Cb, const uint16_t* b_add, uint16_t* out, int B, int HW, int b_B, int G,
                         float* partial, int dtype, void* stream);
int imd_groupnorm_parts(int B, int HW, int C);
int imd_f32_to_16(const float* a, uint16_t* out, long n, int dtype, void* stream);

#ifdef __cplusplus
}
#endif
#endif
```

Measured before the change: 7.096.

## Fuse self-attention out-projection into the text cross-attention row kernel

Self-attention at C=320 now returns a deferred out-projection object instead of running the output linear right away. The following cross-attention block picks it up and a new HIP kernel runs the attn1 out-projection plus bias and residual, LayerNorm, the Q projection, text attention and the attn2 out-projection in one pass over each row tile. This removes one GEMM launch and a full write and read of the intermediate hidden states per transformer block. It adds a large specialized kernel with a deferred-object protocol across processors, falling back to materializing the linear when the conditions do not hold.

Result: no change. 7.135 (median of 6 runs) (+0.6%).

```diff
diff --git a/imagdressing_amd/_lib.py b/imagdressing_amd/_lib.py
--- a/imagdressing_amd/_lib.py
+++ b/imagdressing_amd/_lib.py
@@ -55,6 +55,14 @@
                 ("out", C.c_void_p), ("M", C.c_int), ("C", C.c_int), ("heads", C.c_int), ("L", C.c_int), ("rows_per_image", C.c_int),
                 ("kv_bdiv", C.c_int), ("text_rows", C.c_int), ("x_ld", C.c_int), ("out_ld", C.c_int), ("q_scale", C.c_float),
                 ("ln_eps", C.c_float), ("dtype", C.c_int)]
+
+
+class AttnOutXattnParams(_Sized):
+    _fields_ = [("struct_bytes", C.c_uint32), ("o", C.c_void_p), ("w_o1", C.c_void_p), ("b_o1", C.c_void_p), ("res", C.c_void_p),
+                ("w", C.c_void_p), ("bq", C.c_void_p), ("bo", C.c_void_p), ("kv", C.c_void_p), ("out", C.c_void_p),
+                ("M", C.c_int), ("C", C.c_int), ("heads", C.c_int), ("L", C.c_int), ("rows_per_image", C.c_int),
+                ("kv_bdiv", C.c_int), ("text_rows", C.c_int), ("o_ld", C.c_int), ("res_ld", C.c_int), ("res_rows", C.c_int),
+                ("out_ld", C.c_int), ("q_scale", C.c_float), ("ln_eps", C.c_float), ("dtype", C.c_int)]
 
 
 class AttnParams(_Sized):
@@ -172,6 +180,8 @@
     "imd_ff_geglu": (C.c_int, [C.POINTER(FfParams), C.c_void_p]),
     "imd_text_xattn320": (C.c_int, [C.POINTER(XattnParams), C.c_void_p]),
     "imd_text_xattn320_supported": (C.c_int, [C.POINTER(XattnParams)]),
+    "imd_attn_out_text_xattn320": (C.c_int, [C.POINTER(AttnOutXattnParams), C.c_void_p]),
+    "imd_attn_out_text_xattn320_supported": (C.c_int, [C.POINTER(AttnOutXattnParams)]),
     "imd_conv_ups_phase": (C.c_int, [C.POINTER(ConvGemmParams), C.c_void_p]),
     "imd_conv_ups_phase_supported": (C.c_int, [C.POINTER(ConvGemmParams)]),
     "imd_groupnorm_workspace_floats": (C.c_int, [C.c_int, C.c_int, C.c_int, C.c_int]),
diff --git a/imagdressing_amd/adapter/attention_processor.py b/imagdressing_amd/adapter/attention_processor.py
--- a/imagdressing_amd/adapter/attention_processor.py
+++ b/imagdressing_amd/adapter/attention_processor.py
@@ -164,12 +164,21 @@
 def _fused_attention(x: torch.Tensor, heads: int, *, wq_or_qkv: torch.Tensor, self_attn: bool,
                      kv1=None, kv1_bdiv: int = 1, kv2=None, kv2_bdiv: int = 1, scale2: Optional[torch.Tensor] = None,
                      wo: torch.Tensor, bo: Optional[torch.Tensor], residual: Optional[torch.Tensor],
-                     q_ln: Optional[tuple] = None, pair_half: bool = False, phase2_rows: int = 0) -> torch.Tensor:
+                     q_ln: Optional[tuple] = None, pair_half: bool = False, phase2_rows: int = 0, defer_out: bool = False,
+                     attn_out: Optional["ops.DeferredOutProj"] = None) -> torch.Tensor:
     B, N, Cc = x.shape
     D = Cc // heads
     dpk, dpv = ops.attn_padded_dims(D)
     dev, dt = x.device, x.dtype
     qscale = D ** -0.5 * LOG2E
+    if attn_out is not None:
+        if (ops.FUSED_ROWCHAIN and ops.FUSED_XATTN and not self_attn and q_ln is not None and kv1 is not None and kv2 is None and not pair_half
+                and ops.text_xattn_supported(Cc, heads, N, kv1[2]) and not ops.ATTN_FP8 and not ops.FUSED_OUT_PROJ
+                and attn_out.o.dtype == dt and attn_out.res.dtype == dt and attn_out.wo.dtype == dt and attn_out.res.is_contiguous()):
+            return ops.attn_out_text_xattn(attn_out.o, attn_out.res, ops.pack_attn_out(attn_out.wo, attn_out.bo),
+                                           ops.pack_text_xattn(q_ln[0], q_ln[1], wo, bo), ops.pack_text_kv(kv1[0], kv1[1], kv1[2]),
+                                           Lk=kv1[2], kv_bdiv=kv1_bdiv, ln_eps=q_ln[2], q_scale=qscale)
+        x = residual = attn_out.materialize()
     if (ops.FUSED_XATTN and not self_attn and q_ln is not None and kv1 is not None and kv2 is None and not pair_half
             and ops.text_xattn_supported(Cc, heads, N, kv1[2]) and not ops.ATTN_FP8 and not ops.FUSED_OUT_PROJ
             and residual is not None and residual.data_ptr() == x.data_ptr() and residual.shape == x.shape
@@ -217,9 +226,13 @@
         o = torch.empty(2 * B, N, Cc, dtype=dt, device=dev)
         ops.attention(q, kv1[0], kv1[1], o[:B], B=B, H=heads, N=N, D=D, L1=kv1[2], L1P=kv1[3], kv1_bdiv=kv1_bdiv, k_pad_one=True,
                       out_dup=o[B:], **kw)
+        if defer_out and residual is not None:
+            return ops.DeferredOutProj(o, wo, bo, residual)
         res2 = None if residual is None else residual.reshape(-1, Cc)
         return ops.linear(o.view(2 * B * N, Cc), wo, bo, res=res2).view(2 * B, N, Cc)
     ops.attention(q, kv1[0], kv1[1], o, B=B, H=heads, N=N, D=D, L1=kv1[2], L1P=kv1[3], kv1_bdiv=kv1_bdiv, k_pad_one=True, phase2_rows=phase2_rows if kw else 0, **kw)
+    if defer_out and residual is not None:
+        return ops.DeferredOutProj(o, wo, bo, residual)
     res2 = None if residual is None else residual.view(B * N, Cc)
     return ops.linear(o.view(B * N, Cc), wo, bo, res=res2).view(B, N, Cc)
 
@@ -249,12 +262,16 @@
 class AttnProcessor2_0(_FusedBase):
 
     fused_layernorm = True
+    fused_rowchain = True
 
     def __init__(self, cache_entries: int = 256):
         self._text = _TensorCache(capacity=cache_entries)
 
     def __call__(self, attn, hidden_states, encoder_hidden_states=None, attention_mask=None, temb=None, scale=1.0,
-                 imd_residual=None, imd_layernorm=None, **kwargs):
+                 imd_residual=None, imd_layernorm=None, imd_defer_out=False, imd_attn_out=None, **kwargs):
+        if imd_attn_out is not None and not (encoder_hidden_states is not None and imd_layernorm is not None and imd_attn_out.o.shape[-1] == ops.XATTN_C):
+            hidden_states = imd_residual = imd_attn_out.materialize()
+            imd_attn_out = None
         dt = _compute_dtype(attn, hidden_states, attention_mask)
         x, shape4 = _as_tokens(hidden_states, dt)
         dev = x.device
@@ -270,7 +287,9 @@
                 x = ops.layer_norm(x, g, be, eps)
         if encoder_hidden_states is None:
             out = _fused_attention(x, attn.heads, wq_or_qkv=_layer_weights(attn, "qkv", dt, dev), self_attn=True, wo=wo, bo=bo,
-                                   residual=imd_residual, q_ln=q_ln)
+                                   residual=imd_residual, q_ln=q_ln, defer_out=bool(imd_defer_out) and shape4 is None)
+            if isinstance(out, ops.DeferredOutProj):
+                return out
         else:
             srcs = (encoder_hidden_states, attn.to_k.weight, attn.to_v.weight)
             kv = self._text.get(srcs, extra=(dt,))
@@ -279,8 +298,8 @@
                 kv = self._text.put(srcs, _project_kv(e, _layer_weights(attn, "kv", dt, dev), attn.heads), extra=(dt,))
             out = _fused_attention(x, attn.heads, wq_or_qkv=_layer_weights(attn, "q", dt, dev), self_attn=False, kv1=kv,
                                    kv1_bdiv=self._ehs_bdiv(x.shape[0], encoder_hidden_states), wo=wo, bo=bo,
-                                   residual=imd_residual, q_ln=q_ln)
-        return self._finish(attn, out, imd_residual is not None, hidden_states, shape4, ln_fused=imd_layernorm is not None)
+                                   residual=imd_residual, q_ln=q_ln, attn_out=imd_attn_out)
+        return self._finish(attn, out, imd_residual is not None or imd_attn_out is not None, hidden_states, shape4, ln_fused=imd_layernorm is not None)
 
 
 class CacheAttnProcessor2_0(AttnProcessor2_0):
@@ -347,6 +366,7 @@
 class RefSAttnProcessor2_0(nn.Module, _FusedBase, _RefMixin):
     fused_layernorm = True
     fused_pair_half = True
+    fused_rowchain = True
 
     def __init__(self, name, hidden_size, cross_attention_dim=None, scale=1.0):
         super().__init__()
@@ -357,7 +377,7 @@
 
     def __call__(self, attn, hidden_states, encoder_hidden_states=None, attention_mask=None, temb=None, scale=1.0,
                  num_images_per_prompt=1, cond_hidden_states=None, sa_hidden_states=None, sa_batch_mask=None,
-                 imd_residual=None, imd_layernorm=None, imd_pair_half=False, **kwargs):
+                 imd_residual=None, imd_layernorm=None, imd_pair_half=False, imd_defer_out=False, **kwargs):
         if encoder_hidden_states is not None:
             raise NotImplementedError(f"{type(self).__name__} is a self-attention (attn1) processor")
         dt = _compute_dtype(attn, hidden_states, attention_mask)
@@ -382,7 +402,10 @@
             raise ValueError("imd_pair_half needs sa_hidden_states, the block residual and token-major hidden states (engine-internal)")
         pr = x.shape[0] // 2 if (kwargs.get("sa_pair_layout") and sa_batch_mask is not None and kv2 is not None and not imd_pair_half and x.shape[0] % 2 == 0) else 0
         out = _fused_attention(x, attn.heads, wq_or_qkv=wqkv, self_attn=True, kv2=kv2, kv2_bdiv=bdiv2,
-                               scale2=s2, wo=wo, bo=bo, residual=imd_residual, q_ln=q_ln, pair_half=bool(imd_pair_half), phase2_rows=pr)
+                               scale2=s2, wo=wo, bo=bo, residual=imd_residual, q_ln=q_ln, pair_half=bool(imd_pair_half), phase2_rows=pr,
+                               defer_out=bool(imd_defer_out) and shape4 is None)
+        if isinstance(out, ops.DeferredOutProj):
+            return out
         return self._finish(attn, out, imd_residual is not None, hidden_states, shape4, ln_fused=imd_layernorm is not None)
 
 
@@ -428,6 +451,7 @@
         return w["qkv"], w["o"], _layer_weights(attn, "bo", dt, dev)
 
     __call__ = RefSAttnProcessor2_0.__call__
+    fused_rowchain = True
     fused_pair_half = True
 
 
@@ -450,11 +474,12 @@
         self._plain = AttnProcessor2_0(cache_entries=4)
 
     fused_layernorm = True
+    fused_rowchain = True
 
     def __call__(self, attn, hidden_states, encoder_hidden_states=None, attention_mask=None, temb=None, scale=1.0,
-                 cond_hidden_states=None, sa_hidden_states=None, imd_residual=None, imd_layernorm=None, **kwargs):
+                 cond_hidden_states=None, sa_hidden_states=None, imd_residual=None, imd_layernorm=None, imd_attn_out=None, **kwargs):
         return self._plain(attn, hidden_states, encoder_hidden_states=encoder_hidden_states, imd_residual=imd_residual,
-                           imd_layernorm=imd_layernorm)
+                           imd_layernorm=imd_layernorm, imd_attn_out=imd_attn_out)
 
 
 class _IPBase(nn.Module, _FusedBase, _LoraFold):
diff --git a/imagdressing_amd/csrc/capi.cpp b/imagdressing_amd/csrc/capi.cpp
--- a/imagdressing_amd/csrc/capi.cpp
+++ b/imagdressing_amd/csrc/capi.cpp
@@ -235,6 +235,17 @@
     return imd_launch_text_xattn320(*p, (hipStream_t)stream);
 }
 
+int imd_attn_out_text_xattn320_supported(const imd_attn_out_xattn_params* p) {
+    return (p && p->struct_bytes == sizeof(*p) && imd_attn_out_text_xattn320_supported_of(*p)) ? 1 : 0;
+}
+
+int imd_attn_out_text_xattn320(const imd_attn_out_xattn_params* p, void* stream) {
+    IMD_REQUIRE(p != nullptr, "attn_out_text_xattn320: null params");
+    IMD_REQUIRE_SIZE(p, "attn_out_text_xattn320");
+    IMD_REQUIRE(p->o && p->w_o1 && p->b_o1 && p->res && p->w && p->bq && p->bo && p->kv && p->out, "attn_out_text_xattn320: null pointer");
+    return imd_launch_attn_out_text_xattn320(*p, (hipStream_t)stream);
+}
+
 int imd_conv_ups_phase_supported(const imd_conv_gemm_params* p) { return (sized(p) && imd_conv_ups_phase_supported_of(*p)) ? 1 : 0; }
 
 int imd_conv_ups_phase(const imd_conv_gemm_params* p, void* stream) {
diff --git a/imagdressing_amd/csrc/imd_kernels.h b/imagdressing_amd/csrc/imd_kernels.h
--- a/imagdressing_amd/csrc/imd_kernels.h
+++ b/imagdressing_amd/csrc/imd_kernels.h
@@ -64,6 +64,8 @@
 int imd_launch_ff_geglu(const imd_ff_params& p, hipStream_t s);
 bool imd_text_xattn320_supported_of(const imd_xattn_params& p);
 int imd_launch_text_xattn320(const imd_xattn_params& p, hipStream_t s);
+bool imd_attn_out_text_xattn320_supported_of(const imd_attn_out_xattn_params& p);
+int imd_launch_attn_out_text_xattn320(const imd_attn_out_xattn_params& p, hipStream_t s);
 int imd_launch_attention(const AttnParams& p, hipStream_t s);
 int imd_launch_attention_d40(const AttnParams& p, int variant, hipStream_t s);
 int imd_launch_attention_fp8(const AttnParams& p, int eq, int ek, int ev, hipStream_t s);
diff --git a/imagdressing_amd/csrc/row_xattn.hip b/imagdressing_amd/csrc/row_xattn.hip
--- a/imagdressing_amd/csrc/row_xattn.hip
+++ b/imagdressing_amd/csrc/row_xattn.hip
@@ -228,6 +228,287 @@
     emit(XA_NO - 1);
 }
 
+constexpr int XA_NO1 = 5;
+constexpr int XA_X1B = 8 * 2048;
+constexpr int XA_OFF_B1 = 2 * XA_X1B, XA_OFF_BQ = XA_OFF_B1 + XA_C * 4;
+static_assert(XA_OFF_BQ + 64 * XA_NQ * 4 <= 2 * XA_XB, "x1 exchange + both bias tables fit the exchange area");
+
+template <bool F16>
+__global__ __launch_bounds__(512, 1) void attn_out_text_xattn320_kernel(const imd_attn_out_xattn_params p) {
+    using E = El<F16>;
+    extern __shared__ __attribute__((aligned(16))) char smem[];
+    const int tid = threadIdx.x;
+    const int lane = tid & 63;
+    const int wave = __builtin_amdgcn_readfirstlane(tid >> 6);
+    const int hi = lane >> 5, col = lane & 31;
+    const int rb = wave & 3;
+    const int chh = wave >> 2;
+    const int m0 = blockIdx.x * XA_BM;
+
+    const __amdgpu_buffer_rsrc_t rs_a = __builtin_amdgcn_make_buffer_rsrc(const_cast<uint16_t*>(p.o), 0, (uint32_t)(((size_t)(p.M - 1) * p.o_ld + XA_C) * 2), 0x00020000);
+    const int m = m0 + rb * 32 + col;
+    uint4 xf[XA_STEPS], af[XA_STEPS];
+    load_rows(af, rs_a, true, (uint32_t)m * (uint32_t)(p.o_ld * 2) + hi * 16, 32);
+    float b1_v = 0.f, bq_v = 0.f, bo_v = 0.f;
+    if (tid < XA_C) b1_v = p.b_o1[tid];
+    if (tid < 64 * XA_NQ) bq_v = p.bq[tid];
+    if (tid < XA_C) bo_v = p.bo[tid];
+
+    const int tb = (m0 / p.rows_per_image) / p.kv_bdiv;
+    const v4i_t ds_w = raw_rsrc(p.w, (uint32_t)((XA_NQ + XA_NO) * XA_CHUNK));
+    const v4i_t ds_kv = raw_rsrc(reinterpret_cast<const char*>(p.kv) + (size_t)tb * XA_NKV * XA_CHUNK, (uint32_t)(XA_NKV * XA_CHUNK));
+    const uint32_t loff = (uint32_t)wave * 1024u + (uint32_t)lane * 16u;
+    const uint32_t lds0 = (uint32_t)(uintptr_t)smem;
+    constexpr int C0 = XA_NO1;
+    const v4i_t ds_w1 = raw_rsrc(p.w_o1, (uint32_t)(XA_NO1 * XA_CHUNK));
+    auto stage0 = [&](int c) {
+        const uint32_t base = lds0 + (uint32_t)((c % XA_RING) * XA_CHUNK) + (uint32_t)wave * 1024u;
+#pragma unroll
+        for (int j = 0; j < XA_PIECES; ++j) dma16(ds_w1, base + j * 8192u, loff + (uint32_t)(c * XA_CHUNK) + j * 8192u);
+    };
+    auto stage = [&](int c) {
+        const uint32_t base = lds0 + (uint32_t)(((C0 + c) % XA_RING) * XA_CHUNK) + (uint32_t)wave * 1024u;
+        const bool kvc = c >= XA_NQ && c < XA_NQ + XA_NKV;
+        const uint32_t src = loff + (uint32_t)((kvc ? c - XA_NQ : c < XA_NQ ? c : c - XA_NKV) * XA_CHUNK);
+#pragma unroll
+        for (int j = 0; j < XA_PIECES; ++j) dma16(kvc ? ds_kv : ds_w, base + j * 8192u, src + j * 8192u);
+    };
+    stage0(0);
+    stage0(1);
+    pin_rows(af);
+    float* bias_s = reinterpret_cast<float*>(smem + XA_OFF_X);
+    float* bq_s = reinterpret_cast<float*>(smem + XA_OFF_X + XA_OFF_BQ);
+    if (tid < 64 * XA_NQ) bq_s[tid] = bq_v;
+    if (tid < XA_C) reinterpret_cast<float*>(smem + XA_OFF_X + XA_OFF_B1)[tid] = b1_v;
+
+    const f32x16 zero16 = {0.f, 0.f, 0.f, 0.f, 0.f, 0.f, 0.f, 0.f, 0.f, 0.f, 0.f, 0.f, 0.f, 0.f, 0.f, 0.f};
+    const int wrow = chh * 32 + col;
+    const uint32_t a16 = (uint32_t)((hi ^ ((wrow >> 1) & 7)) << 4);
+    const char* wlane = smem + wrow * XA_ROWB;
+
+    uint4 x1own[XA_NO1][2], x1par[XA_NO1][2];
+    const char* xr = smem + XA_OFF_X + (wave ^ 4) * 2048 + lane * 16;
+    auto take_x1 = [&](int c) {
+#pragma unroll
+        for (int t = 0; t < 2; ++t) x1par[c][t] = *reinterpret_cast<const uint4*>(xr + (c & 1) * XA_X1B + t * 1024);
+    };
+    {
+        const __amdgpu_buffer_rsrc_t rs_r = __builtin_amdgcn_make_buffer_rsrc(const_cast<uint16_t*>(p.res), 0, 0x80000000u, 0x00020000);
+        const int res_shift = p.res_rows > 0 ? (m0 / p.res_rows) * p.res_rows : 0;
+        const uint32_t r0off = (uint32_t)(m - res_shift) * (uint32_t)(p.res_ld * 2) + (uint32_t)(chh * 64 + hi * 16);
+        const float* b1_s = reinterpret_cast<const float*>(smem + XA_OFF_X + XA_OFF_B1);
+        char* xw = smem + XA_OFF_X + wave * 2048 + lane * 16;
+        uint4 r0raw[2][2];
+        auto load_res0 = [&](int c) {
+#pragma unroll
+            for (int t = 0; t < 2; ++t) r0raw[c & 1][t] = buf_load16(rs_r, r0off + (uint32_t)(c * 128 + t * 32));
+        };
+        auto emit0 = [&](int c, const f32x16& acc) {
+            uint2 rres[4];
+#pragma unroll
+            for (int t = 0; t < 2; ++t) {
+                const uint4 r = wide_to_quads(r0raw[c & 1][t]);
+                rres[2 * t] = make_uint2(r.x, r.y); rres[2 * t + 1] = make_uint2(r.z, r.w);
+            }
+            v2u pk[4];
+#pragma unroll
+            for (int j = 0; j < 4; ++j) {
+                const float4 bb = *reinterpret_cast<const float4*>(b1_s + c * 64 + chh * 32 + 8 * j + 4 * hi);
+                const float v0 = acc[4 * j] + bb.x + E::lo(rres[j].x), v1 = acc[4 * j + 1] + bb.y + E::hi(rres[j].x);
+                const float v2 = acc[4 * j + 2] + bb.z + E::lo(rres[j].y), v3 = acc[4 * j + 3] + bb.w + E::hi(rres[j].y);
+                pk[j] = v2u{E::pack2(v0, v1), E::pack2(v2, v3)};
+            }
+#pragma unroll
+            for (int t = 0; t < 2; ++t) {
+                const v4u w = quads_to_wide(pk[2 * t], pk[2 * t + 1]);
+                x1own[c][t] = make_uint4(w[0], w[1], w[2], w[3]);
+                *reinterpret_cast<uint4*>(xw + (c & 1) * XA_X1B + t * 1024) = x1own[c][t];
+            }
+        };
+        load_res0(0);
+#pragma unroll
+        for (int c = 0; c < XA_NO1; ++c) {
+            if (c == 0) dma_wait(); else dma_wait_keep_n<XA_PIECES + 2>();
+            __syncthreads();
+            if (c > 0) take_x1(c - 1);
+            if (c + 2 < XA_NO1) stage0(c + 2); else stage(c + 2 - XA_NO1);
+            if (c + 1 < XA_NO1) load_res0(c + 1);
+            const char* Ws = wlane + (c % XA_RING) * XA_CHUNK;
+            f32x16 acc = zero16;
+#pragma unroll
+            for (int s = 0; s < XA_STEPS; ++s) {
+                const uint4 wf = *reinterpret_cast<const uint4*>(Ws + ((uint32_t)(s * 32) ^ a16));
+                acc = E::mfma(wf, af[s], acc);
+            }
+            emit0(c, acc);
+        }
+    }
+
+    uint4 qf[2 * XA_NQ];
+#pragma unroll
+    for (int c = 0; c < XA_NQ; ++c) {
+        dma_wait_keep_n<XA_PIECES>();
+        __syncthreads();
+        stage(c + 2);
+        {
+            if (c == 0) {
+                take_x1(XA_NO1 - 1);
+#pragma unroll
+                for (int k = 0; k < XA_NO1; ++k)
+#pragma unroll
+                    for (int t = 0; t < 2; ++t) {
+                        const uint4 a = x1own[k][t], b = x1par[k][t];
+                        xf[4 * k + t] = chh == 0 ? a : b;
+                        xf[4 * k + 2 + t] = chh == 0 ? b : a;
+                    }
+                ln_rows_inplace<F16, XA_C>(xf, p.ln_eps);
+            }
+        }
+        const char* Ws = wlane + ((C0 + c) % XA_RING) * XA_CHUNK;
+        f32x16 acc = zero16;
+#pragma unroll
+        for (int s = 0; s < XA_STEPS; ++s) {
+            const uint4 wf = *reinterpret_cast<const uint4*>(Ws + ((uint32_t)(s * 32) ^ a16));
+            acc = E::mfma(wf, xf[s], acc);
+        }
+        v2u pk[4];
+#pragma unroll
+        for (int j = 0; j < 4; ++j) {
+            const float4 bb = *reinterpret_cast<const float4*>(bq_s + c * 64 + chh * 32 + 8 * j + 4 * hi);
+            pk[j] = v2u{E::pack2((acc[4 * j] + bb.x) * p.q_scale, (acc[4 * j + 1] + bb.y) * p.q_scale),
+                        E::pack2((acc[4 * j + 2] + bb.z) * p.q_scale, (acc[4 * j + 3] + bb.w) * p.q_scale)};
+        }
+#pragma unroll
+        for (int t = 0; t < 2; ++t) {
+            const v4u w = quads_to_wide(pk[2 * t], pk[2 * t + 1]);
+            qf[2 * c + t] = make_uint4(w[0], w[1], w[2], w[3]);
+        }
+    }
+    {
+        const uint32_t one = (uint32_t)E::fromf(1.0f);
+#pragma unroll
+        for (int hl = 0; hl < 4; ++hl)
+            if (hi == 1) qf[3 * hl + 2].x = (qf[3 * hl + 2].x & 0xffff0000u) | one;
+    }
+
+    uint2 og[4][5], pg[4][5];
+    const int krot = 3 * ((col >> 3) & 1);
+    const char* xown = smem + XA_OFF_X + wave * (5 * 512) + lane * 8;
+    const char* xpar = smem + XA_OFF_X + (wave ^ 4) * (5 * 512) + lane * 8;
+#pragma unroll
+    for (int hl = 0; hl < XA_NKV; ++hl) {
+        const int c = XA_NQ + hl;
+        dma_wait_keep_n<XA_PIECES>();
+        __syncthreads();
+        stage(c + 2);
+        if (hl > 0) {
+#pragma unroll
+            for (int j = 0; j < 5; ++j) pg[hl - 1][j] = *reinterpret_cast<const uint2*>(xpar + ((hl - 1) & 1) * XA_XB + j * 512);
+        }
+        const char* Ks = smem + ((C0 + c) % XA_RING) * XA_CHUNK + chh * XA_HEADB;
+        const char* Vs = Ks + XA_KBYTES;
+        f32x16 sc[3];
+#pragma unroll
+        for (int kb = 0; kb < 3; ++kb) {
+            sc[kb] = zero16;
+#pragma unroll
+            for (int t = 0; t < 3; ++t) {
+                const uint4 kf = *reinterpret_cast<const uint4*>(Ks + (kb * 32 + col) * XA_KROW + ((2 * t + hi + krot) % 6) * 16);
+                sc[kb] = E::mfma(kf, qf[3 * hl + t], sc[kb]);
+            }
+        }
+        float mx = sc[0][0];
+#pragma unroll
+        for (int kb = 0; kb < 3; ++kb)
+#pragma unroll
+            for (int r = 0; r < 16; ++r) mx = fmaxf(mx, sc[kb][r]);
+        mx = fmaxf(mx, __shfl_xor(mx, 32));
+        f32x16 o0 = zero16, o1 = zero16;
+#pragma unroll
+        for (int kb = 0; kb < 3; ++kb)
+#pragma unroll
+            for (int g = 0; g < 2; ++g) {
+                uint4 pf;
+                pf.x = E::pack2(__builtin_amdgcn_exp2f(sc[kb][8 * g + 0] - mx), __builtin_amdgcn_exp2f(sc[kb][8 * g + 1] - mx));
+                pf.y = E::pack2(__builtin_amdgcn_exp2f(sc[kb][8 * g + 2] - mx), __builtin_amdgcn_exp2f(sc[kb][8 * g + 3] - mx));
+                pf.z = E::pack2(__builtin_amdgcn_exp2f(sc[kb][8 * g + 4] - mx), __builtin_amdgcn_exp2f(sc[kb][8 * g + 5] - mx));
+                pf.w = E::pack2(__builtin_amdgcn_exp2f(sc[kb][8 * g + 6] - mx), __builtin_amdgcn_exp2f(sc[kb][8 * g + 7] - mx));
+                const int pc = (2 * (2 * kb + g) + hi) * 16;
+                const uint4 v0 = *reinterpret_cast<const uint4*>(Vs + col * XA_VROW + pc);
+                const uint4 v1 = *reinterpret_cast<const uint4*>(Vs + (32 + (col & 15)) * XA_VROW + pc);
+                o0 = E::mfma(v0, pf, o0);
+                o1 = E::mfma(v1, pf, o1);
+            }
+        const float inv = 1.0f / __shfl(o1[4], col);
+#pragma unroll
+        for (int j = 0; j < 4; ++j)
+            og[hl][j] = make_uint2(E::pack2(o0[4 * j] * inv, o0[4 * j + 1] * inv), E::pack2(o0[4 * j + 2] * inv, o0[4 * j + 3] * inv));
+        og[hl][4] = make_uint2(E::pack2(o1[0] * inv, o1[1] * inv), E::pack2(o1[2] * inv, o1[3] * inv));
+#pragma unroll
+        for (int j = 0; j < 5; ++j) *reinterpret_cast<uint2*>(const_cast<char*>(xown) + (hl & 1) * XA_XB + j * 512) = og[hl][j];
+    }
+
+    const __amdgpu_buffer_rsrc_t rs_o = __builtin_amdgcn_make_buffer_rsrc(p.out, 0, 0x80000000u, 0x00020000);
+    const uint32_t obase = m < p.M ? (uint32_t)m * (uint32_t)(p.out_ld * 2) : OOB;
+    f32x16 acc[XA_NO];
+    auto emit = [&](int c) {
+        uint2 rres[4];
+#pragma unroll
+        for (int t = 0; t < 2; ++t) {
+            const uint4 r = wide_to_quads(x1own[c][t]);
+            rres[2 * t] = make_uint2(r.x, r.y); rres[2 * t + 1] = make_uint2(r.z, r.w);
+        }
+        v2u pk[4];
+#pragma unroll
+        for (int j = 0; j < 4; ++j) {
+            const float4 bb = *reinterpret_cast<const float4*>(bias_s + c * 64 + chh * 32 + 8 * j + 4 * hi);
+            const float v0 = acc[c][4 * j] + bb.x + E::lo(rres[j].x), v1 = acc[c][4 * j + 1] + bb.y + E::hi(rres[j].x);
+            const float v2 = acc[c][4 * j + 2] + bb.z + E::lo(rres[j].y), v3 = acc[c][4 * j + 3] + bb.w + E::hi(rres[j].y);
+            pk[j] = v2u{E::pack2(v0, v1), E::pack2(v2, v3)};
+        }
+#pragma unroll
+        for (int t = 0; t < 2; ++t) {
+            const v4u w = quads_to_wide(pk[2 * t], pk[2 * t + 1]);
+            const uint32_t off = (uint32_t)((c * 64 + chh * 32 + 16 * t + 8 * hi) * 2);
+            __builtin_amdgcn_raw_buffer_store_b128(w, rs_o, (int)(obase == OOB ? OOB : obase + off), 0, 0);
+        }
+    };
+    uint4 of[XA_STEPS];
+#pragma unroll
+    for (int co = 0; co < XA_NO; ++co) {
+        const int c = XA_NQ + XA_NKV + co;
+        dma_wait();
+        __syncthreads();
+        if (co == 0) {
+#pragma unroll
+            for (int j = 0; j < 5; ++j) pg[3][j] = *reinterpret_cast<const uint2*>(xpar + XA_XB + j * 512);
+            if (tid < XA_C) bias_s[tid] = bo_v;
+#pragma unroll
+            for (int s = 0; s < XA_STEPS; ++s) {
+                uint2 g2[2];
+#pragma unroll
+                for (int e = 0; e < 2; ++e) {
+                    const int G = 2 * s + e, h = G / 5, j = G % 5;
+                    const uint2 mine = og[h & 3][j], theirs = pg[h & 3][j];
+                    const bool own = (h >> 2) == chh;
+                    g2[e] = make_uint2(own ? mine.x : theirs.x, own ? mine.y : theirs.y);
+                }
+                of[s] = make_uint4(g2[0].x, g2[0].y, g2[1].x, g2[1].y);
+            }
+        }
+        if (co > 0) emit(co - 1);
+        if (c + 2 < XA_NCHUNK) stage(c + 2);
+        const char* Ws = wlane + ((C0 + c) % XA_RING) * XA_CHUNK;
+        acc[co] = zero16;
+#pragma unroll
+        for (int s = 0; s < XA_STEPS; ++s) {
+            const uint4 wf = *reinterpret_cast<const uint4*>(Ws + ((uint32_t)(s * 32) ^ a16));
+            acc[co] = E::mfma(wf, of[s], acc[co]);
+        }
+    }
+    emit(XA_NO - 1);
+}
+
 }
 
 bool imd_text_xattn320_supported_of(const imd_xattn_params& p) {
@@ -253,3 +534,31 @@
     else hipLaunchKernelGGL(text_xattn320_kernel<false>, grid, dim3(512), XA_LDS, s, p);
     return imd_check_launch("text_xattn320");
 }
+bool imd_attn_out_text_xattn320_supported_of(const imd_attn_out_xattn_params& p) {
+    imd_xattn_params q{};
+    q.M = p.M; q.C = p.C; q.heads = p.heads; q.L = p.L; q.rows_per_image = p.rows_per_image; q.kv_bdiv = p.kv_bdiv; q.text_rows = p.text_rows;
+    q.x_ld = p.out_ld; q.out_ld = p.out_ld; q.dtype = p.dtype;
+    return imd_text_xattn320_supported_of(q) && p.o_ld >= XA_C && (p.o_ld % 8) == 0 && p.res_ld >= XA_C && (p.res_ld % 8) == 0 &&
+           (p.res_rows == 0 || (p.res_rows > 0 && (p.res_rows % XA_BM) == 0 && (p.M % p.res_rows) == 0));
+}
+
+int imd_launch_attn_out_text_xattn320(const imd_attn_out_xattn_params& p, hipStream_t s) {
+    if (!imd_attn_out_text_xattn320_supported_of(p))
+        return imd_set_error("attn_out_text_xattn320: needs the geometry of text_xattn320 (C = 320, 8 heads, 1..96 text keys, rows per image a multiple of 128, "
+                             "M / rows_per_image == text_rows * kv_bdiv), leading dimensions >= 320 in steps of 8 and res_rows = 0 or a multiple of 128 that divides M "
+                             "(got C=%d heads=%d L=%d M=%d rows_per_image=%d text_rows=%d kv_bdiv=%d o_ld=%d res_ld=%d res_rows=%d out_ld=%d dtype=%d)",
+                             p.C, p.heads, p.L, p.M, p.rows_per_image, p.text_rows, p.kv_bdiv, p.o_ld, p.res_ld, p.res_rows, p.out_ld, p.dtype);
+    const int rrows = p.res_rows > 0 ? p.res_rows : p.M;
+    if (((size_t)(p.M - 1) * p.o_ld + XA_C) * 2 >= 0x80000000ull || ((size_t)(p.M - 1) * p.out_ld + XA_C) * 2 >= 0x80000000ull ||
+        ((size_t)(rrows - 1) * p.res_ld + XA_C) * 2 >= 0x80000000ull)
+        return imd_set_error("attn_out_text_xattn320: operand larger than 2 GiB");
+    if (p.res_rows > 0 && p.res == p.out) return imd_set_error("attn_out_text_xattn320: out may alias res only without res_rows");
+    if (!(p.ln_eps > 0.f)) return imd_set_error("attn_out_text_xattn320: LayerNorm needs eps > 0");
+    const bool h = p.dtype == IMD_DTYPE_F16;
+    const void* kern = h ? reinterpret_cast<const void*>(attn_out_text_xattn320_kernel<true>) : reinterpret_cast<const void*>(attn_out_text_xattn320_kernel<false>);
+    if (int rc_attr = imd_lds_attr(kern, XA_LDS, "attn_out_text_xattn320")) return rc_attr;
+    const dim3 grid((unsigned)(p.M / XA_BM));
+    if (h) hipLaunchKernelGGL((attn_out_text_xattn320_kernel<true>), grid, dim3(512), XA_LDS, s, p);
+    else hipLaunchKernelGGL((attn_out_text_xattn320_kernel<false>), grid, dim3(512), XA_LDS, s, p);
+    return imd_check_launch("attn_out_text_xattn320");
+}
diff --git a/imagdressing_amd/ops.py b/imagdressing_amd/ops.py
--- a/imagdressing_amd/ops.py
+++ b/imagdressing_amd/ops.py
@@ -611,6 +611,62 @@
     return out
 
 
+FUSED_ROWCHAIN = _os.environ.get("IMD_FUSED_ROWCHAIN", "1") != "0"
+_ATTN_OUT_W: Dict[Tuple, tuple] = {}
+_clear_hooks.append(_ATTN_OUT_W.clear)
+
+
+class DeferredOutProj:
+    __slots__ = ("o", "wo", "bo", "res")
+
+    def __init__(self, o, wo, bo, res):
+        self.o, self.wo, self.bo, self.res = o, wo, bo, res
+
+    def materialize(self) -> torch.Tensor:
+        Cc = self.o.shape[-1]
+        return linear(self.o.view(-1, Cc), self.wo, self.bo, res=self.res.reshape(-1, Cc)).view(self.o.shape)
+
+
+def pack_attn_out(wo1: torch.Tensor, bo1: Optional[torch.Tensor]):
+    if tuple(wo1.shape) != (XATTN_C, XATTN_C):
+        raise L.ImdError(f"pack_attn_out: expected a [320, 320] matrix, got {tuple(wo1.shape)}")
+    srcs = (wo1, bo1)
+    key = tuple(None if t is None else (t.data_ptr(), t._version, t.dtype, str(t.device)) for t in srcs)
+    ent = _ATTN_OUT_W.get(key)
+    if ent is None:
+        if len(_ATTN_OUT_W) > 64:
+            _ATTN_OUT_W.clear()
+        b = torch.zeros(XATTN_C, dtype=torch.float32, device=wo1.device) if bo1 is None else bo1.float().contiguous()
+        ent = _ATTN_OUT_W[key] = (srcs, dict(w=xattn_swizzle_rows(wo1.contiguous()), b=b))
+    return ent[1]
+
+
+def attn_out_text_xattn(o: torch.Tensor, res: torch.Tensor, packed_o1: dict, packed: dict, kv_img: torch.Tensor, *, Lk: int, kv_bdiv: int = 1,
+                        ln_eps: float = 1e-5, q_scale: Optional[float] = None, out: Optional[torch.Tensor] = None) -> torch.Tensor:
+    ensure_device(o.device)
+    B, N, C_ = o.shape
+    dt = o.dtype
+    if out is None:
+        out = torch.empty((B, N, C_), dtype=dt, device=o.device)
+    if kv_img.dim() != 3 or tuple(kv_img.shape[1:]) != (4, XATTN_CHUNK):
+        raise L.ImdError(f"attn_out_text_xattn: kv_img must be [Bt, 4, {XATTN_CHUNK}], got {tuple(kv_img.shape)}")
+    res2 = res.reshape(-1, C_)
+    p = L.AttnOutXattnParams()
+    p.o, p.res, p.out = _dev(o, dt, "o"), _dev(res2, dt, "res"), _dev(out, dt, "out")
+    p.w_o1, p.b_o1 = _dev(packed_o1["w"], dt, "w_o1"), _dev(packed_o1["b"], torch.float32, "b_o1")
+    p.w, p.bq, p.bo, p.kv = _dev(packed["w"], dt, "w"), _dev(packed["bq"], torch.float32, "bq"), _dev(packed["bo"], torch.float32, "bo"), _dev(kv_img, dt, "kv_img")
+    p.M, p.C, p.heads, p.L = B * N, C_, XATTN_HEADS, int(Lk)
+    p.rows_per_image, p.kv_bdiv, p.text_rows = N, int(kv_bdiv), kv_img.shape[0]
+    p.o_ld = p.res_ld = p.out_ld = C_
+    p.res_rows = 0 if res2.shape[0] == B * N else res2.shape[0]
+    p.q_scale = float(XATTN_D ** -0.5 * 1.4426950408889634 if q_scale is None else q_scale)
+    p.ln_eps, p.dtype = float(ln_eps), _code(o, "o")
+    _count("gemm_conv", 3 * 2.0 * B * N * C_ * C_)
+    _count("attention", 4.0 * XATTN_HEADS * N * XATTN_D * B * Lk)
+    L.check(L.load().imd_attn_out_text_xattn320(C.byref(p), _stream()))
+    return out
+
+
 def conv2d_nhwc(x: torch.Tensor, w: torch.Tensor, bias=None, *, taps=9, stride=1, ups=False, rowvec=None,
                 rowvec_stride=0, rowvec_off=0, res=None, out_scale=1.0, act=ACT_NONE, out_f32=False, cfg=-1, split_k=0, gn=None,
                 pad_br_only=False, gn_stats_groups=0, gn_out=None, gn_in=None) -> torch.Tensor:
diff --git a/imagdressing_amd/unet.py b/imagdressing_amd/unet.py
--- a/imagdressing_amd/unet.py
+++ b/imagdressing_amd/unet.py
@@ -211,8 +211,17 @@
     def set_processor(self, p):
         self.processor = p
 
-    def __call__(self, hidden_states, encoder_hidden_states=None, residual=None, layernorm=None, **cross_attention_kwargs):
+    def __call__(self, hidden_states, encoder_hidden_states=None, residual=None, layernorm=None, defer_out=False, **cross_attention_kwargs):
         proc = self.processor
+        chain = getattr(proc, "fused_rowchain", False) and getattr(proc, "fused_residual", False)
+        if isinstance(hidden_states, ops.DeferredOutProj):
+            if (chain and getattr(proc, "fused_layernorm", False) and ops.FUSED_LN and layernorm is not None and encoder_hidden_states is not None):
+                cross_attention_kwargs = dict(cross_attention_kwargs, imd_attn_out=hidden_states)
+                hidden_states, residual = hidden_states.o, None
+            else:
+                hidden_states = residual = hidden_states.materialize()
+        if defer_out and chain and residual is not None:
+            cross_attention_kwargs = dict(cross_attention_kwargs, imd_defer_out=True)
         if layernorm is not None:
             nrm, eps = layernorm
             if (getattr(proc, "fused_layernorm", False) and getattr(proc, "fused_residual", False) and ops.FUSED_LN
@@ -249,8 +258,16 @@
                                               sd[f"{p}.ff.net.2.bias"].to(device), self.norm3.weight, self.norm3.bias, dtype=dtype)
 
     def __call__(self, h, ehs, cak):
-        h = self.attn1(h, encoder_hidden_states=None, residual=h, layernorm=(self.norm1, 1e-5), **cak)
+        h = self.attn1(h, encoder_hidden_states=None, residual=h, layernorm=(self.norm1, 1e-5), defer_out=self.rowchain_ok(h, ehs), **cak)
         return self.after_attn1(h, ehs, cak)
+
+    def rowchain_ok(self, h, ehs) -> bool:
+        p1, p2 = self.attn1.processor, self.attn2.processor
+        return bool(ops.FUSED_ROWCHAIN and ops.FUSED_XATTN and ops.FUSED_LN and not ops.ATTN_FP8 and not ops.FUSED_OUT_PROJ
+                    and ehs is not None and ehs.dim() == 3
+                    and all(getattr(p, "fused_rowchain", False) and getattr(p, "fused_residual", False) for p in (p1, p2))
+                    and getattr(p2, "fused_layernorm", False)
+                    and ops.text_xattn_supported(h.shape[-1], self.attn2.heads, h.shape[1], ehs.shape[1]))
 
     def after_attn1(self, h, ehs, cak):
         h = self.attn2(h, encoder_hidden_states=ehs, residual=h, layernorm=(self.norm2, 1e-5), **cak)
@@ -292,7 +309,7 @@
         blk = self.transformer_blocks[0]
         h = self.proj_in(x_half, gn_in=(self.norm.weight, self.norm.bias, 1e-6, False, self.groups)).view(Bh, H * W, Cc)
         r = h
-        h = blk.attn1(h, encoder_hidden_states=None, residual=r, layernorm=(blk.norm1, 1e-5), imd_pair_half=True, **cak)
+        h = blk.attn1(h, encoder_hidden_states=None, residual=r, layernorm=(blk.norm1, 1e-5), imd_pair_half=True, defer_out=blk.rowchain_ok(h, ehs), **cak)
         h = blk.after_attn1(h, ehs, cak)
         return self.proj_out(h.view(2 * Bh, H, W, Cc), res=x_half)
 
diff --git a/include/imagdressing_hip.h b/include/imagdressing_hip.h
--- a/include/imagdressing_hip.h
+++ b/include/imagdressing_hip.h
@@ -129,6 +129,26 @@
     int dtype;
 } imd_xattn_params;
 
+typedef struct imd_attn_out_xattn_params {
+    uint32_t struct_bytes;
+    const uint16_t* o;
+    const uint16_t* w_o1;
+    const float* b_o1;
+    const uint16_t* res;
+    const uint16_t* w;
+    const float* bq;
+    const float* bo;
+    const uint16_t* kv;
+    uint16_t* out;
+    int M, C, heads, L;
+    int rows_per_image;
+    int kv_bdiv, text_rows;
+    int o_ld, res_ld, res_rows, out_ld;
+    float q_scale;
+    float ln_eps;
+    int dtype;
+} imd_attn_out_xattn_params;
+
 typedef struct imd_groupnorm_params {
     uint32_t struct_bytes;
     const uint16_t* x; uint16_t* y; const float* gamma; const float* beta;
@@ -286,6 +306,9 @@
 int imd_text_xattn320(const imd_xattn_params* p, void* stream);
 int imd_text_xattn320_supported(const imd_xattn_params* p);
 
+int imd_attn_out_text_xattn320(const imd_attn_out_xattn_params* p, void* stream);
+int imd_attn_out_text_xattn320_supported(const imd_attn_out_xattn_params* p);
+
 int imd_conv_ups_phase(const imd_conv_gemm_params* p, void* stream);
 int imd_conv_ups_phase_supported(const imd_conv_gemm_params* p);
 
```
